# mosure/burn_depth

Measured on AMD Instinct MI355X. Metric: frames/sec Depth Pro @1536^2 bf16, higher is better.
Workload: dtype bf16; 1 GPU; DepthPro::infer [8,3,1536,1536] per GPU, default DepthProConfig; batch_per_gpu=8, streams_per_gpu=1, global_batch=8, parallelism=dp1, attention_form=attn577_gfx950.s (assembly-owned, one persistent workgroup per CU), scatter_inputs_from_rank0=False, gather_depth_to_rank0=False, ranks_seen=1

## Files before the change

### burn_depth_amd/_lib.py

```python
from __future__ import annotations

import ctypes as C
import os

_HERE = os.path.dirname(os.path.abspath(__file__))
LIB_PATH = os.path.join(_HERE, "libmi_depth.so")

MD_OK = 0
MD_ERR_INVALID_ARG, MD_ERR_SHAPE, MD_ERR_IO, MD_ERR_FORMAT, MD_ERR_HIP = -1, -2, -3, -4, -5
MD_ERR_UNSUPPORTED, MD_ERR_NO_FOV, MD_ERR_OOM, MD_ERR_LEVELS = -6, -7, -8, -9
MD_MEM_HOST, MD_MEM_DEVICE = 0, 1
MD_COMM_ID_BYTES = 128
MD_FRAME_U8_GRAY, MD_FRAME_RGBA_F32 = 0, 1
VIT_GEMM_RESID, VIT_GEMM_QKV, VIT_GEMM_FC1, VIT_GEMM_PATCH_EMBED = 0, 1, 2, 3
DECODER_GEMM_CONV3, DECODER_GEMM_CONV3_S2, DECODER_GEMM_PIXSHUF, DECODER_GEMM_HEAD, DECODER_GEMM_HEAD_UP2 = 0, 1, 2, 3, 4
TILE_256x256, TILE_128x128, TILE_256x32, TILE_128x64, TILE_64x64, TILE_AUTO = 0, 1, 2, 3, 4, 99


class MdError(RuntimeError):

    def __init__(self, code: int, message: str):
        super().__init__(f"mi_depth error {code}: {message}")
        self.code = code
        self.message = message
# ... 252 lines not shown
    "md_debug_gemm_direct_store": (_I, [_I]),
    "md_debug_gemm_persistent": (_I, [_I]),
    "md_debug_gemm_stagger": (_I, [_I, _I]),
    "md_debug_gemm_stagger_ticks": (_I, [_I]),
    "md_da3_infer_raw": (_I, [_P, _P, _I, _I, _I, _I, _P, _I, _P]),
    "md_da3_infer_from_tokens": (_I, [_P, C.POINTER(C.c_void_p), _I, _I, _I, _I, _I, _P, _I, _P]),
    "md_da3_param_inventory": (_I, [C.POINTER(MdDa3Cfg), _I, _I, C.POINTER(C.c_char_p), C.POINTER(C.c_size_t), _F, _F]),
    "md_model_query": (_I, [_P, C.c_char_p, C.POINTER(C.c_int64)]),
    "md_model_set_option": (_I, [_P, C.c_char_p, C.c_int64]),
    "md_model_enable_taps": (_I, [_P, _I]),
    "md_model_read_tap": (_I, [_P, C.c_char_p, _P, C.c_size_t, C.POINTER(C.c_int64 * 4)]),
    "md_model_enable_timing": (_I, [_P, _I]),
    "md_model_set_timing_filter": (_I, [_P, C.c_char_p]),
    "md_model_read_timing": (_I, [_P, C.POINTER(C.c_char_p), _F, C.POINTER(_I), _I, C.POINTER(_I)]),
    "md_model_read_launch_order": (_I, [_P, C.POINTER(C.c_char_p), _I, C.POINTER(_I)]),
    "md_op_rgb_to_input": (_I, [_P, _P, C.c_size_t, _I, _I, _P, _P]),
    "md_catmull_rom_taps": (_I, [_I, _I, _I, C.POINTER(_I), C.POINTER(_I), _F]),
    "md_op_resize_catmull_rom": (_I, [_P, _P, _I, _I, _I, _I, _I, _I, _I, _I, _I, _P, _P, _P]),
    "md_op_depth_display": (_I, [_P, _P, _I, _I, _I, _I, _I, _I, _I, _I, _I, _I, _I, _P, _P, _P]),
    "md_op_resize_bilinear": (_I, [_P, _P, _I, _I, _I, _I, _P, _I, _I, _I, _P]),
    "md_op_pyramid_patchify": (_I, [_P, _P, _I, _I, _I, _I, _I, _I, _I, _P, C.POINTER(_I), C.POINTER(_I), _P]),
    "md_op_resize_nhwc": (_I, [_P, _P, _I, _I, _I, _I, _P, _I, _I, _I, _I, _P]),
    "md_op_resize_output_size": (_I, [_I, _I, C.c_float, C.c_float, C.POINTER(_I), C.POINTER(_I)]),
    "md_op_split": (_I, [_P, _P, _I, _I, _I, _I, C.c_float, _P, C.POINTER(_I), _P]),
    "md_op_merge": (_I, [_P, _P, _I, _I, _I, _I, _I, _I, _P, C.POINTER(_I), C.POINTER(_I), _P]),
    "md_op_layernorm": (_I, [_P, _P, _P, _P, _I, _I, C.c_float, _P, _P]),
    "md_op_linear": (_I, [_P, _P, _P, _P, _I, _I, _I, _I, _I, _P, _P]),
    "md_op_linear_tile": (_I, [_P, _P, _P, _P, _I, _I, _I, _I, _I, _I, _P, _P]),
    "md_op_attention": (_I, [_P, _P, _I, _I, _I, _I, _P, _P]),
    "md_op_attention_views": (_I, [_P, _P, _I, _I, _I, _I, _I, _P, _P]),
    "md_op_attention_ex": (_I, [_P, C.POINTER(MdAttentionOp), _P]),
    "md_debug_attention_last_form": (_I, [C.POINTER(_I * 4)]),
    "md_op_conv3x3": (_I, [_P, _P, _P, _P, _I, _I, _I, _I, _I, _I, _I, _P, _P]),
    "md_op_deconv2x2": (_I, [_P, _P, _P, _P, _I, _I, _I, _I, _I, _I, _P, _P]),
    "md_op_conv2d_direct": (_I, [_P, _P, _P, _P, _I, _I, _I, _I, _I, _I, _I, _I, _I, _P, _P]),
    "md_op_qkv_norm_rope": (_I, [_P, _P, _P, _P, _P, _P, _P, _P, _I, _I, _I, _I, _I, _I, _I, C.c_float, C.c_float, _I, _I, _I, _P, _P, _P]),
    "md_op_qk_norm_rope": (_I, [_P, _P, _P, _P, _P, _P, _I, _I, _I, _I, _I, _I, C.c_float, C.c_float, _I, _P, _P]),
    "md_op_hook_cat_ln": (_I, [_P, _P, _P, _I, _I, _I, _I, _P, _P, C.c_float, _P, _P, C.c_float, _I, _P, _P, _P]),
    "md_op_patchify": (_I, [_P, _P, _I, _I, _I, _I, _I, _I, _P, _P, _I, _I, _I, _P, _P, _P]),
    "md_op_set_token0": (_I, [_P, _P, _I, _I, _I, _P, _I, _P]),
    "md_op_border_bias_fix": (_I, [_P, _P, _I, _I, _I, _I, _I, _P, _I, _P]),
    "md_op_layernorm_ex": (_I, [_P, _P, _I, _I, _I, _I, C.POINTER(_I), C.POINTER(_I), C.POINTER(_P), C.POINTER(_P), C.c_float, _I, _I,
                                C.c_float, _P, _I, _P, _P]),
    "md_op_store_rows": (_I, [_P, _P, C.c_int64, _I, _I, _P, _P]),
    "md_op_load_rows": (_I, [_P, _P, C.c_int64, _I, _I, _P, _P]),
    "md_op_f32_to_fp8": (_I, [_P, _P, C.c_int64, C.c_float, _P, _P]),
    "md_op_pack_fp8_rows": (_I, [_P, _P, _I, _I, _I, _P, _P, _P]),
    "md_op_nchw_to_nhwc": (_I, [_P, _P, _I, _I, _I, _I, _I, _I, _I, _P, _P]),
    "md_op_nhwc_to_nchw": (_I, [_P, _P, _I, _I, _I, _I, _I, _I, _I, _P, _P]),
    "md_op_ln_fold_vectors": (_I, [_P, _P, _P, _P, _P, _I, _I, _I, _P, _P, _P]),
    "md_op_ln_finish": (_I, [_P, _P, C.c_int64, C.c_float, C.c_float, _P, _P]),
    "md_op_vit_gemm": (_I, [_P, C.POINTER(MdVitGemm), _P]),
    "md_debug_gemm_last_form": (_I, [C.POINTER(_I * 8)]),
    "md_debug_gemm_last_launch": (_I, [C.POINTER(_I * 4)]),
    "md_op_decoder_gemm": (_I, [_P, C.POINTER(MdDecoderGemm), _P]),
    "md_op_camera_encode": (_I, [_P, C.POINTER(MdCameraEncode), _P]),
    "md_op_camera_decode": (_I, [_P, C.POINTER(MdCameraDecode), _P]),
    "md_op_pose_to_camera": (_I, [_P, _P, _I, _I, _I, _P, _P, _P]),
    "md_op_conv2d_direct_ex": (_I, [_P, _P, _P, _P, _P, _I, _I, _I, _I, _I, _I, _I, _I, _I, _I, _I, _P, _P]),
    "md_op_fov_to_focal": (_I, [C.c_float, _I, _I, _F, _F]),
    "md_op_focal_to_fov": (_I, [C.c_float, _I, _I, _F, _F]),
    "md_bench_gemm": (_I, [_P, _I, _I, _I, _I, _I, _I, _I, _I, _I, _F]),
    "md_gemm_pick_tile": (_I, [_I, _I, _I, _I]),
    "md_bench_attention": (_I, [_P, _I, _I, _I, _I, _F]),
    "md_bench_attention_ex": (_I, [_P, _I, _I, _I, _I, C.c_float, _I, _F]),
    "md_debug_attention_asm": (_I, [_I]),
    "md_debug_attention_asm_launches": (C.c_long, []),
    "md_debug_attention_redo_units": (C.c_long, [_P, _I]),
    "md_bench_attention_qkv": (_I, [_P, _P, _I, _I, _I, _I, _I, _F, C.POINTER(C.c_long)]),
    "md_comm_unique_id": (_I, [_P]),
    "md_comm_init_rank": (_I, [_P, _P, _I, _I, C.POINTER(_P)]),
    "md_comm_rank": (_I, [_P, C.POINTER(_I), C.POINTER(_I)]),
    "md_comm_count": (_I, [_P, C.POINTER(_I)]),
    "md_comm_destroy": (_I, [_P]),
    "md_comm_broadcast_weights": (_I, [_P, _P, _I]),
    "md_comm_scatter_images": (_I, [_P, _P, _P, C.c_size_t, _I, _P]),
    "md_comm_gather_depth": (_I, [_P, _P, _P, C.c_size_t, _I, _P]),
    "md_depth_pro_infer_tiles_loopback": (_I, [C.POINTER(_P), _I, _I, _P, _I, _I, _I, _I, _P, _P, _P, _P, _I, _P]),
    "md_comm_depth_pro_infer_tiles": (_I, [_P, _P, _P, _I, _I, _I, _I, _P, _P, _P, _P, _I, _I, _P]),
    "md_param_inventory": (_I, [C.POINTER(MdDepthProCfg), _I, _I, C.POINTER(C.c_char_p), C.POINTER(C.c_size_t), _F, _F]),
    "md_uniform_stream": (_I, [C.c_char_p, C.c_uint64, C.c_size_t, C.c_float, C.c_float, _P]),
    "md_split_geometry": (_I, [_I, _I, C.c_float, C.POINTER(_I), C.POINTER(_I)]),
    "md_feature_padding": (_I, [_I, _I, _I]),
}


def _infer_points(*parts):
    return _I, [_P, _P, _I, _I, _I, _I, _P, C.POINTER(MdPointsCameras), *(C.POINTER(p) for p in parts), _I, _P]


_POINTS_HEAD = [MdViewFilterOpts, MdPointsOpts, MdPointsOutputs]
_POINTS_PARTS = [("normals", MdPointsNormals), ("voxel", MdPointsVoxel), ("render", MdPointsRender), ("mesh", MdPointsMesh),
                 ("raster", MdPointsRaster), ("outlier", MdPointsOutlier), ("decimate", MdPointsDecimate), ("components", MdPointsComponents),
                 ("smooth", MdPointsSmooth), ("planes", MdPointsPlanes), ("clusters", MdPointsClusters)]
SYMBOLS["md_infer_points"] = _infer_points(*_POINTS_HEAD[1:])
SYMBOLS["md_infer_points_filtered"] = _infer_points(*_POINTS_HEAD)
SYMBOLS.update({f"md_infer_points_{name}": _infer_points(*_POINTS_HEAD, *(p for _, p in _POINTS_PARTS[:i + 1]))
                for i, (name, _) in enumerate(_POINTS_PARTS)})

_lib = None


def load() -> C.CDLL:
    global _lib
    if _lib is not None:
        return _lib
    if not os.path.exists(LIB_PATH):
        raise ImportError(
            f"{LIB_PATH} is missing: build the HIP extension first (python -c 'import __graft_entry__ as g; g.build()'). "
            "burn_depth_amd has no CPU fallback.")
    lib = C.CDLL(LIB_PATH)
    for name, (res, args) in SYMBOLS.items():
        fn = getattr(lib, name)
        fn.restype = res
        fn.argtypes = args
    _lib = lib
    return lib


def check(code: int) -> None:
    if code != MD_OK:
        msg = load().md_last_error()
        raise MdError(code, msg.decode("utf-8", "replace") if msg else "")
```

### burn_depth_amd/csrc/kernels/ops.h

```cpp
#pragma once

#include "../md_common.h"

namespace md {

int launch_rgb_to_input(const uint8_t* rgb, int w, int h, float* out, hipStream_t s);

struct CrAxis {
  const int2* win;
  const float* w;
  int maxc;
};
void catmull_rom_window(int in_len, int out_len, int o, int* left, int* count, float* weights);
int catmull_rom_max_taps(int in_len, int out_len);
void catmull_rom_span(const int* left, const int* count, int cx, int tw, int* xb0, int* nq);
int launch_resize_catmull_rom(const uint8_t* rgb, int B, int h, int w, const CrAxis& ax_v, int cy, int th, const CrAxis& ax_h, int cx,
                              int tw, int xb0, int nq, float* tmp, uint8_t* out_u8, float* out_nchw, hipStream_t s);
struct DisplayGeom {
  int B, h, w, cx, cy, cw, ch, ow, oh, resize;
  float sx, sy;
};
int display_parts(const DisplayGeom& g);
int launch_depth_display(const float* depth, const DisplayGeom& g, int normalize, int format, void* out, float* range, float2* parts,
                         hipStream_t s);
// ... 233 lines not shown
};
constexpr int kRenderMaxRadius = 16;
size_t render_scratch_bytes(int T, int H, int W);
int launch_render_points(const RenderParams& p, void* scratch, hipStream_t s);

struct MeshParams {
  const float* depth = nullptr;
  const int32_t* pixel_index = nullptr;
  int B = 0, H = 0, W = 0, stride = 1;
  long limit = 0;
  float max_rtol = 0.f;
  int32_t* faces = nullptr;
  int32_t* face_count = nullptr;
  long face_capacity = 0;
};
size_t mesh_scratch_bytes(int B, int H, int W, int stride);
int launch_mesh_index(int B, int H, int W, const void* points_scratch, int32_t* pixel_index, hipStream_t s);
int launch_mesh_grid(const MeshParams& p, void* scratch, hipStream_t s);

struct RasterParams {
  const float* xyz = nullptr;
  const uint8_t* rgb = nullptr;
  const int32_t* faces = nullptr;
  const int32_t* count = nullptr;
  int n = 0, nf = 0;
  int T = 0, H = 0, W = 0;
  const float *K = nullptr, *E = nullptr, *focal = nullptr;
  float off = 0.f, znear = 0.f, zfar = 0.f;
  int cull = 0, max_extent = 64;
  float* depth = nullptr;
  int32_t* face = nullptr;
  uint8_t* rgb_out = nullptr;
  int32_t* filled = nullptr;
  int32_t* skipped = nullptr;
};
constexpr int kRasterMaxExtent = 1024;
constexpr int kRasterDefaultExtent = 64;
int raster_inline_pixels();
int raster_queue_capacity(int capacity);
int raster_queue_entries();
size_t raster_scratch_bytes(int T, int H, int W, int queue_entries);
int launch_render_mesh(const RasterParams& p, void* scratch, int queue_entries, hipStream_t s);

int launch_resize_bilinear(const float* in, int planes, int H, int W, float* out, int OH, int OW, int method,
                           int post, hipStream_t s);

struct PyramidGeom {
  int B, S, win, ps;
  int steps0, stride0;
  int steps1, stride1;
  int method;
};
int launch_pyramid_patchify(const float* x, const PyramidGeom& g, void* patches, int prec, hipStream_t s, bool force_generic = false);

int launch_patchify(const float* x, int B, int H, int W, int ps, int Kp, void* out, int prec, hipStream_t s, float* cls_x = nullptr,
                    int S = 0, int n_tokens = 0, int D = 0, const float* cls = nullptr, const float* pos0 = nullptr);

int launch_resize_nhwc(const void* in, int B, int H, int W, int C, long ld_in, void* out, int OH, int OW, long ld_out,
                       int method, const float* addend, int prec, hipStream_t s);

int launch_border_bias_fix(void* map, int B, int H, int W, int C, long ld, const float* bias9, int prec, hipStream_t s);

int launch_split(const float* x, int B, int C, int S, int win, int stride, int steps, float* out, hipStream_t s);
int launch_merge(const float* tiles, int B, int C, int h, int w, int steps, int pad, float* out, int OH, int OW,
                 hipStream_t s);

struct SeqGroups {
  int ngroups;
  int seq0[4];
  int nseq[4];
  const float* a[4];
  const float* b[4];
};
int launch_cls_init(float* x, int nseq_total, int S, int n_tokens, int D, const SeqGroups& g, hipStream_t s);

int launch_layernorm(const float* x, void* out, long rows, int D, float eps, int S, const SeqGroups& g, int prec,
                     int out_f32, hipStream_t s, float fp8_inv_scale = 1.f, const float* tok0 = nullptr, int tok0_stride = 0,
                     float* x_rw = nullptr);
int launch_ln_fold_vectors(const float* W, const float* gamma, const float* beta, const float* bias, int N, int K, int prec, float* c,
                           float* d, hipStream_t s);
int launch_fill_pairs(float* ab, long rows, float a, float b, hipStream_t s);
int launch_ln_finish(const float* parts, float* ab, long rows, float inv_n, float eps, hipStream_t s);
int launch_convert_rows(const float* x, void* out, long count, int prec, hipStream_t s, int width = 0);

int launch_nchw_to_nhwc(const float* in, int B, int C, int H, int W, void* out, int prec, int relu, hipStream_t s, long ld = 0);
int launch_head_tail_debug(const void* relu_map, long ld, long pixels, int C, const float* w, const float* bias, float* pre_out,
                           float* canonical, int prec, hipStream_t s);
int launch_nhwc_to_nchw(const void* in, int B, int C, int H, int W, long ld, int coff, float* out, int prec,
                        hipStream_t s);
int launch_rows_to_f32(const void* in, long count, float* out, int prec, hipStream_t s, int width = 0);
int launch_f32_to_rows(const float* in, long count, void* out, int prec, hipStream_t s, int width = 0);

int launch_conv_direct(const void* in, int in_prec, const float* add, int B, int H, int W, int Cin, const float* w,
                       const float* bias, int Cout, int k, int stride, int pad, int relu, float* out, hipStream_t s, int out_ld = 0);

int launch_f32_to_fp8(const float* in, long n, float inv_scale, void* out, hipStream_t s);
int launch_pack_fp8_rows(const float* w, int N, int K, int Kp, void* out, float* scale, hipStream_t s);

int launch_qk_norm_rope(void* qk, long rows, int S, int n_tokens, int D, int heads, int pw, const float* q_gamma,
                        const float* q_beta, const float* k_gamma, const float* k_beta, float eps, const float* rope_cos,
                        const float* rope_sin, int global_pos, float q_scale, int prec, hipStream_t s);
int launch_set_token0(float* x, int nseq, int S, int D, const float* src, hipStream_t s, int src_stride = 0);

#define MD_CAM_MAX_VIEWS 16
struct CamEncW {
  static constexpr int kMaxDepth = 8;
  const float *fc1_w, *fc1_b, *fc2_w, *fc2_b;
  const float *tn_g, *tn_b, *on_g, *on_b;
  struct Blk {
    const float *n1g, *n1b, *n2g, *n2b, *qkv_w, *qkv_b, *proj_w, *proj_b, *ls1, *fc1_w, *fc1_b, *fc2_w, *fc2_b, *ls2;
  } blk[kMaxDepth];
  int depth;
};
struct CamDecW {
  const float *w1, *b1, *w2, *b2, *wt, *bt, *wq, *bq, *wf, *bf;
};
int launch_camera_decoder(const float* cam, int B, int din, const CamDecW& w, int H, int W, float* h1, float* h2, float* pose, float* extr,
                          float* intr, hipStream_t s);
size_t camera_encoder_scratch_floats(int B, int V, int D);
int launch_camera_encoder(const float* extr, const float* intr, int B, int V, int D, int heads, int H, int W, float eps_tok, float eps_blk,
                          const CamEncW& w, float* scratch, float* out, hipStream_t s);
int launch_hook_cat_ln(const float* x_local, const float* x, long rows, int S, int n_tokens, int D, const float* norm_g,
                       const float* norm_b, float eps_final, const float* head_g, const float* head_b, float eps_head,
                       void* out, float* cam_out, int prec, hipStream_t s);
int launch_pose_to_camera(const float* pose, int B, int H, int W, float* extrinsics, float* intrinsics, hipStream_t s);

int launch_fov_post(const float* fov_deg, int B, int H, int W, float* focal_px, float* fovy_rad, float* ratio,
                    hipStream_t s);
int launch_focal_post(const float* f_px, int B, int H, int W, float* focal_px, float* fovx_deg, float* fovy_rad, float* ratio,
                      hipStream_t s);
int launch_depth_post(const float* canonical, const float* ratio, int B, long hw, float* out, int post, hipStream_t s);

int launch_softmax_rows(float* s, long rows, int n_valid, int ld, float scale, hipStream_t st);

int launch_qkv_split(const float* qkv, int T, int N, int heads, int SS, int kpad, void* qk, void* vT, float q_scale, int prec,
                     hipStream_t s);
int launch_unpad_rows(const void* in, int T, int N, int SS, int D, float* out, int prec, hipStream_t s);

constexpr float kAttnQScale = 0.125f * 1.4426950408889634f;
inline float attn_qscale(int prec) { return prec == MD_PREC_F32 ? 1.0f : kAttnQScale; }

int launch_attention(const void* qk, const void* vT, void* out, int nseq, int S, int n_tokens, int heads, int D,
                     int kpad, int prec, hipStream_t s, float out_fp8_inv = 0.f, long v_plane = 0, int* redo = nullptr,
                     int redo_units = 0);
int attention_asm_prepare();
int launch_attention_views(const void* qk, const void* vT, void* out, int nseq, int views, int S, int n_tokens, int heads, int D,
                           int kpad, int prec, hipStream_t s, long v_plane = 0, int* redo = nullptr, int redo_units = 0);
int attention_allow_asm(int on);
long attention_asm_launches();
int attention_redo_ints(int nunits);
long attention_asm_redo_units(int reset);
int attention_allow_small(int on);
struct AttnSmallScope {
  explicit AttnSmallScope(int on) : prev_(attention_allow_small(on)) {}
  ~AttnSmallScope() { attention_allow_small(prev_); }
  AttnSmallScope(const AttnSmallScope&) = delete;
  AttnSmallScope& operator=(const AttnSmallScope&) = delete;

 private:
  int prev_;
};
enum { ATTN_FORM_NONE = -1, ATTN_FORM_PLAIN = 0, ATTN_FORM_KEYSPLIT = 1, ATTN_FORM_ASM = 2, ATTN_FORM_VIEWS = 3, ATTN_FORM_FP8OUT = 4, ATTN_FORM_F32 = 5 };
struct AttnForm {
  int form = ATTN_FORM_NONE;
  int grid = 0, qw = 0, ks = 0;
};
// ... 5 lines not shown
```

### burn_depth_amd/csrc/kernels/ops.hip

```cpp
#include "ops.h"
#include "camera_math.h"
#include "elem.h"

namespace md {

static inline int grid_for(long work_items, int block = 256, int cap = 256 * 8) {
  long g = (work_items + block - 1) / block;
  if (g < 1) g = 1;
  if (g > cap) g = cap;
  return (int)g;
}

__global__ void rgb_to_input_kernel(const uint8_t* __restrict__ rgb, long hw, float* __restrict__ out) {
#pragma clang fp contract(off)
  const float mean[3] = {0.485f, 0.456f, 0.406f};
  const float sd[3] = {0.229f, 0.224f, 0.225f};
  for (long i = blockIdx.x * (long)blockDim.x + threadIdx.x; i < hw; i += (long)gridDim.x * blockDim.x) {
#pragma unroll
    for (int c = 0; c < 3; ++c) {
      float v = (float)rgb[i * 3 + c] / 255.0f;
      out[c * hw + i] = (v - mean[c]) / sd[c];
    }
  }
}
// ... 685 lines not shown
  }
}

int launch_f32_to_rows(const float* in, long count, void* out, int prec, hipStream_t s, int width) {
  if (prec == MD_PREC_F16X2 && (width <= 0 || count % width != 0)) MD_FAIL(MD_ERR_INVALID_ARG, "f32_to_rows: split-half rows need the row width");
  MD_BY_PREC(prec, hipLaunchKernelGGL(f32_to_rows_kernel<T>, dim3(grid_for(count)), dim3(256), 0, s, in, count, (T*)out, width));
  MD_HIP(hipGetLastError());
  return MD_OK;
}
__global__ __launch_bounds__(256) void ln_finish_kernel(const float* __restrict__ parts, float* __restrict__ ab, long rows, float inv_n, float eps) {
  const long r = (long)blockIdx.x * 256 + threadIdx.x;
  if (r >= rows) return;
  const f32x4_t p0 = *(const f32x4_t*)(parts + r * 8), p1 = *(const f32x4_t*)(parts + r * 8 + 4);
  const float mu = ((p0[0] + p0[2]) + (p1[0] + p1[2])) * 0.25f;
  const float d0 = p0[0] - mu, d1 = p0[2] - mu, d2 = p1[0] - mu, d3 = p1[2] - mu;
  const float m2 = ((p0[1] + p0[3]) + (p1[1] + p1[3])) + 256.0f * ((d0 * d0 + d1 * d1) + (d2 * d2 + d3 * d3));
  const float rstd = 1.0f / sqrtf(m2 * inv_n + eps);
  ab[r * 2] = rstd;
  ab[r * 2 + 1] = -mu * rstd;
}

__global__ __launch_bounds__(256) void fill_pairs_kernel(float* __restrict__ ab, long rows, float a, float b) {
  const long r = (long)blockIdx.x * 256 + threadIdx.x;
  if (r < rows) { ab[2 * r] = a; ab[2 * r + 1] = b; }
}
int launch_fill_pairs(float* ab, long rows, float a, float b, hipStream_t s) {
  if (!ab || rows <= 0) MD_FAIL(MD_ERR_INVALID_ARG, "fill_pairs: invalid argument");
  hipLaunchKernelGGL(fill_pairs_kernel, dim3((unsigned)((rows + 255) / 256)), dim3(256), 0, s, ab, rows, a, b);
  MD_HIP(hipGetLastError());
  return MD_OK;
}

int launch_ln_finish(const float* parts, float* ab, long rows, float inv_n, float eps, hipStream_t s) {
  if (!parts || !ab || rows <= 0) MD_FAIL(MD_ERR_INVALID_ARG, "ln_finish: invalid argument");
  hipLaunchKernelGGL(ln_finish_kernel, dim3((unsigned)((rows + 255) / 256)), dim3(256), 0, s, parts, ab, rows, inv_n, eps);
  MD_HIP(hipGetLastError());
  return MD_OK;
}

template <typename T>
__global__ __launch_bounds__(256) void ln_fold_vectors_kernel(const float* __restrict__ W, const float* __restrict__ gamma,
                                                              const float* __restrict__ beta, const float* __restrict__ bias, int N, int K,
                                                              float* __restrict__ c, float* __restrict__ d) {
  const int n = blockIdx.x * 4 + (threadIdx.x >> 6), lane = threadIdx.x & 63;
  if (n >= N) return;
  const float* w = W + (long)n * K;
  double sc = 0.0, sd = 0.0;
  for (int k = lane; k < K; k += 64) {
    float wr;
    if constexpr (sizeof(T) == 4) {
      wr = w[k];
    } else {
      const float hi = (float)cvt_elem<T>(w[k]);
      wr = is_split<T>::value ? hi + (float)cvt_elem<T>(w[k] - hi) : hi;
    }
    sc += (double)gamma[k] * (double)wr;
    sd += (double)beta[k] * (double)wr;
  }
#pragma unroll
  for (int o = 32; o > 0; o >>= 1) {
    sc += __shfl_xor(sc, o);
    sd += __shfl_xor(sd, o);
  }
  if (lane == 0) {
    c[n] = (float)sc;
    d[n] = (float)(sd + (bias ? (double)bias[n] : 0.0));
  }
}

int launch_ln_fold_vectors(const float* W, const float* gamma, const float* beta, const float* bias, int N, int K, int prec, float* c,
                           float* d, hipStream_t s) {
  if (!W || !gamma || !beta || !c || !d || N <= 0 || K <= 0) MD_FAIL(MD_ERR_INVALID_ARG, "ln_fold_vectors: invalid argument");
  MD_BY_PREC(prec, hipLaunchKernelGGL(ln_fold_vectors_kernel<T>, dim3((unsigned)((N + 3) / 4)), dim3(256), 0, s, W, gamma, beta, bias, N, K, c, d));
  MD_HIP(hipGetLastError());
  return MD_OK;
}

int launch_convert_rows(const float* x, void* out, long count, int prec, hipStream_t s, int width) {
  return launch_f32_to_rows(x, count, out, prec, s, width);
}
int launch_rows_to_f32(const void* in, long count, float* out, int prec, hipStream_t s, int width) {
  if (prec == MD_PREC_F16X2 && (width <= 0 || count % width != 0)) MD_FAIL(MD_ERR_INVALID_ARG, "rows_to_f32: split-half rows need the row width");
  MD_BY_PREC(prec, hipLaunchKernelGGL(rows_to_f32_kernel<T>, dim3(grid_for(count)), dim3(256), 0, s, (const T*)in, count, out, width));
  MD_HIP(hipGetLastError());
  return MD_OK;
}

template <typename T>
__global__ void nchw_to_nhwc_kernel(const float* __restrict__ in, int B, int C, int H, int W, T* __restrict__ out,
                                    int relu, long ld) {
  const long total = (long)B * C * H * W;
  for (long e = blockIdx.x * (long)blockDim.x + threadIdx.x; e < total; e += (long)gridDim.x * blockDim.x) {
    const int c = (int)(e % C);
    long t = e / C;
    const int xw = (int)(t % W);
    t /= W;
    const int y = (int)(t % H);
    const int b = (int)(t / H);
    float v = in[(((long)b * C + c) * H + y) * W + xw];
    if (relu) v = fmaxf(v, 0.f);
    st1p<T>(out + (e / C) * (ld * kPlanes<T>) + c, ld, v);
  }
}
template <typename T>
__global__ void nhwc_to_nchw_kernel(const T* __restrict__ in, int B, int C, int H, int W, long ld, int coff,
                                    float* __restrict__ out) {
  const long total = (long)B * C * H * W;
  for (long e = blockIdx.x * (long)blockDim.x + threadIdx.x; e < total; e += (long)gridDim.x * blockDim.x) {
    const int xw = (int)(e % W);
    long t = e / W;
    const int y = (int)(t % H);
    t /= H;
    const int c = (int)(t % C);
    const int b = (int)(t / C);
    const long src = (((long)b * H + y) * W + xw) * (ld * kPlanes<T>) + coff + c;
    out[e] = ld1p<T>(in + src, ld);
  }
}

int launch_nchw_to_nhwc(const float* in, int B, int C, int H, int W, void* out, int prec, int relu, hipStream_t s, long ld) {
  const long total = (long)B * C * H * W;
  if (ld != 0 && ld < C) MD_FAIL(MD_ERR_INVALID_ARG, "nchw_to_nhwc: pixel stride %ld below C %d", ld, C);
  MD_BY_PREC(prec, hipLaunchKernelGGL(nchw_to_nhwc_kernel<T>, dim3(grid_for(total)), dim3(256), 0, s, in, B, C, H, W, (T*)out, relu, ld ? ld : (long)C));
  MD_HIP(hipGetLastError());
  return MD_OK;
}

template <typename T>
__global__ void head_tail_debug_kernel(const T* __restrict__ relu_map, long ld, long pixels, int C, const float* __restrict__ w,
                                       const float* __restrict__ bias, float* __restrict__ pre_out, float* __restrict__ canonical) {
  for (long e = blockIdx.x * (long)blockDim.x + threadIdx.x; e < pixels; e += (long)gridDim.x * blockDim.x) {
    const T* px = relu_map + e * (ld * kPlanes<T>);
    float acc = 0.f;
    for (int c = 0; c < C; ++c) acc = fmaf(ld1p<T>(px + c, ld), w[c], acc);
    acc += bias ? bias[0] : 0.f;
    if (pre_out) pre_out[e] = acc;
    if (canonical) canonical[e] = fmaxf(acc, 0.f);
  }
}
int launch_head_tail_debug(const void* relu_map, long ld, long pixels, int C, const float* w, const float* bias, float* pre_out,
                           float* canonical, int prec, hipStream_t s) {
  MD_BY_PREC(prec, hipLaunchKernelGGL(head_tail_debug_kernel<T>, dim3(grid_for(pixels)), dim3(256), 0, s, (const T*)relu_map, ld, pixels, C, w,
                                      bias, pre_out, canonical));
  MD_HIP(hipGetLastError());
  return MD_OK;
}
int launch_nhwc_to_nchw(const void* in, int B, int C, int H, int W, long ld, int coff, float* out, int prec,
                        hipStream_t s) {
  const long total = (long)B * C * H * W;
  MD_BY_PREC(prec, hipLaunchKernelGGL(nhwc_to_nchw_kernel<T>, dim3(grid_for(total)), dim3(256), 0, s, (const T*)in, B, C, H, W, ld, coff, out));
  MD_HIP(hipGetLastError());
  return MD_OK;
}

template <typename TI>
__device__ inline void load4v(const TI* in, long src, long plane, float v[4]) {
  const f32x4_t t = load4p<TI>(in + src, plane);
  v[0] = t[0], v[1] = t[1], v[2] = t[2], v[3] = t[3];
}

template <typename TI, int CO, int VEC>
__global__ __launch_bounds__(256) void conv_direct_kernel(const TI* __restrict__ in, const float* __restrict__ add,
                                                          int B, int H, int W, int Cin, const float* __restrict__ w,
                                                          const float* __restrict__ bias, int Cout, int k, int stride,
                                                          int pad, int relu, float* __restrict__ out, int OH, int OW, int out_ld) {
  const int lane = threadIdx.x & 63;
// ... 466 lines not shown
```

### burn_depth_amd/csrc/md_api.cpp

```cpp
#include <algorithm>
#include <cmath>
#include <cstdio>
#include <cstring>
#include <optional>
#include <vector>

#include "md_engine.h"
#include "md_engine_util.h"

using namespace md;

namespace {
struct DevBuf {
  void* p = nullptr;
  ~DevBuf() {
    if (p) (void)hipFree(p);
  }
  int alloc(size_t bytes, bool raw = false) {
    if (hipMalloc(&p, bytes + 4096) != hipSuccess) {
      set_error("hipMalloc(%zu) failed", bytes);
      return MD_ERR_OOM;
    }
    return raw || hipMemset(p, 0, bytes + 4096) == hipSuccess ? MD_OK : MD_ERR_HIP;
  }
// ... 289 lines not shown
}

int md_depth_pro_decoder_from_features(md_model_t m, const md_nchw_view* features, int levels, int B, int in_kind,
                                       float* out_features, float* out_lowres, float* const* out_fusions, int out_kind,
                                       void* stream) {
  return model_decoder_from_features(m, features, levels, B, in_kind, out_features, out_lowres, out_fusions, out_kind, (hipStream_t)stream);
}

int md_depth_pro_head_debug(md_model_t m, const md_nchw_view* feature, int B, int in_kind, const md_head_debug* out, int out_kind,
                            void* stream) {
  return model_head_debug(m, feature, B, in_kind, out, out_kind, (hipStream_t)stream);
}

int md_depth_pro_infer_windows(md_model_t m, const float* nchw, int B, int H, int W, int in_kind, float* depth,
                               float* focallength_px, float* fovx_deg, float* fovy_rad, int out_kind, int parts,
                               float* window_ms, float* tail_ms, void* stream) {
  if (!nchw) MD_FAIL(MD_ERR_INVALID_ARG, "input pointer is null");
  if (m && m->kind != 0) MD_FAIL(MD_ERR_INVALID_ARG, "not a Depth Pro model");
  if (parts < 1 || parts > 64) MD_FAIL(MD_ERR_INVALID_ARG, "parts = %d (1 .. 64)", parts);
  ShardPlan sp;
  sp.parts = parts;
  sp.part = -1;
  sp.window_ms = window_ms;
  sp.tail_ms = tail_ms;
  return model_infer_sharded(m, nchw, B, H, W, in_kind, depth, focallength_px, fovx_deg, fovy_rad, out_kind, (hipStream_t)stream, sp);
}

int md_infer_from_rgb(md_model_t m, const uint8_t* rgb, size_t rgb_len, int w, int h, int in_kind, float* depth,
                      float* focallength_px, float* fovy_rad, int out_kind, void* stream) {
  if (!rgb) MD_FAIL(MD_ERR_INVALID_ARG, "rgb pointer is null");
  if (w <= 0 || h <= 0) MD_FAIL(MD_ERR_SHAPE, "invalid image size %dx%d", w, h);
  const size_t expected = (size_t)w * (size_t)h * 3;
  if (rgb_len != expected) MD_FAIL(MD_ERR_SHAPE, "expected %zu RGB bytes for %dx%d, got %zu", expected, w, h, rgb_len);
  if (m && m->kind != 0) MD_FAIL(MD_ERR_INVALID_ARG, "not a Depth Pro model");
  return model_infer(m, nullptr, 1, h, w, in_kind, depth, focallength_px, nullptr, fovy_rad, out_kind, (hipStream_t)stream,
                     rgb, rgb_len);
}

int md_infer_from_rgb_with_focal(md_model_t m, const uint8_t* rgb, size_t rgb_len, int w, int h, int in_kind, float f_px,
                                 float* depth, float* focallength_px, float* fovy_rad, int out_kind, void* stream) {
  if (!rgb) MD_FAIL(MD_ERR_INVALID_ARG, "rgb pointer is null");
  if (w <= 0 || h <= 0) MD_FAIL(MD_ERR_SHAPE, "invalid image size %dx%d", w, h);
  const size_t expected = (size_t)w * (size_t)h * 3;
  if (rgb_len != expected) MD_FAIL(MD_ERR_SHAPE, "expected %zu RGB bytes for %dx%d, got %zu", expected, w, h, rgb_len);
  if (m && m->kind != 0) MD_FAIL(MD_ERR_INVALID_ARG, "not a Depth Pro model");
  return model_infer(m, nullptr, 1, h, w, in_kind, depth, focallength_px, nullptr, fovy_rad, out_kind, (hipStream_t)stream,
                     rgb, rgb_len, &f_px, MD_MEM_HOST);
}

int md_model_enable_graph(md_model_t m, int enable) {
  if (!m) MD_FAIL(MD_ERR_INVALID_ARG, "model is null");
  m->graph_enabled = enable != 0;
  return MD_OK;
}

int md_model_query(md_model_t m, const char* key, int64_t* out) {
  if (!m || !key || !out) MD_FAIL(MD_ERR_INVALID_ARG, "null argument");
  const std::string k = key;
  if (k == "img_size") *out = m->S;
  else if (k == "patch_window") *out = m->win;
  else if (k == "interpolation") *out = m->cfg.interpolation;
  else if (k == "precision") *out = m->prec;
  else if (k == "max_batch") *out = m->cfg.max_batch;
  else if (k == "num_params") {
    int64_t n = 0;
    for (auto& p : m->params) n += (int64_t)p.count();
    *out = n;
  } else if (k == "workspace_bytes") *out = (int64_t)m->ws.cap;
  else if (k == "weight_bytes") *out = m->parent ? 0 : (int64_t)(m->w32_bytes + m->wpk_bytes);
  else if (k == "tiles_per_image") *out = m->steps0 * m->steps0 + m->steps1 * m->steps1 + 1;
  else if (k == "seq_stride") *out = m->SS;
  else if (k == "is_fork") *out = m->parent ? 1 : 0;
  else if (k == "forks") *out = m->forks.load();
  else if (k == "weight_terms") *out = model_root(m)->wterms;
  else if (k == "allocs") *out = m->alloc_count;
  else if (k == "voxel_overflow") return points_voxel_overflow(m, out);
  else if (k == "outlier_overflow") return points_outlier_overflow(m, out);
  else if (k == "clusters_overflow") return points_clusters_overflow(m, out);
  else if (k == "decimate_overflow") return points_decimate_overflow(m, out);
  else if (k == "da3_shape_builds") *out = da3_shape_builds(m);
  else if (k == "batch_invariant") *out = m->batch_invariant ? 1 : 0;
  else if (k == "ln_fold") *out = m->ln_fold_opt;
  else if (k == "ln_fold_active") *out = m->ln_fold_on() ? 1 : 0;
  else if (model_decoder_query(m, k, out)) {}
  else MD_FAIL(MD_ERR_INVALID_ARG, "unknown query key `%s`", key);
  return MD_OK;
}

int md_model_set_option(md_model_t m, const char* key, int64_t value) {
  if (!m || !key) MD_FAIL(MD_ERR_INVALID_ARG, "null argument");
  const std::string k = key;
  if (k == "batch_invariant") {
    if (value != 0 && value != 1) MD_FAIL(MD_ERR_INVALID_ARG, "batch_invariant takes 0 or 1");
    if (m->batch_invariant != (value != 0)) {
      m->batch_invariant = value != 0;
      MD_HIP(hipSetDevice(m->dev->ordinal));
      MD_HIP(hipDeviceSynchronize());
      m->graphs.clear();
    }
    return MD_OK;
  }
  if (k == "ln_fold") {
    if (value < 0 || value > 4) MD_FAIL(MD_ERR_INVALID_ARG, "ln_fold takes 0 (off), 1 (automatic), 2 (on whenever the model can), 3 / 4 (bench diagnostics: unfolded schedule through the fold-form consumer kernels on neutral statistics / the fold with the ln_finish launch)");
    if (value >= 2 && !m->ln_fold_can) MD_FAIL(MD_ERR_UNSUPPORTED, "ln_fold: this model cannot fold its LayerNorms (16-bit Depth Pro models of width %% 256 == 0 can)");
    if (m->ln_fold_opt != (int)value) {
      m->ln_fold_opt = (int)value;
      MD_HIP(hipSetDevice(m->dev->ordinal));
      MD_HIP(hipDeviceSynchronize());
      m->graphs.clear();
    }
    return MD_OK;
  }
  MD_FAIL(MD_ERR_INVALID_ARG, "unknown option `%s`", key);
}

int md_model_enable_taps(md_model_t m, int enable) {
  if (!m) MD_FAIL(MD_ERR_INVALID_ARG, "model is null");
  m->taps_enabled = enable != 0;
  return MD_OK;
}

int md_model_read_tap(md_model_t m, const char* name, float* host_data, size_t capacity, int64_t dims[4]) {
  if (!m || !name) MD_FAIL(MD_ERR_INVALID_ARG, "null argument");
  auto it = m->taps.find(name);
  if (it == m->taps.end() || !it->second.dev) MD_FAIL(MD_ERR_INVALID_ARG, "tap `%s` was not captured", name);
  if (dims) memcpy(dims, it->second.dims, sizeof(int64_t) * 4);
  if (!host_data) return MD_OK;
  if (capacity < it->second.count) MD_FAIL(MD_ERR_SHAPE, "tap `%s` needs %zu floats, capacity %zu", name, it->second.count, capacity);
  MD_HIP(hipSetDevice(m->dev->ordinal));
  MD_HIP(hipDeviceSynchronize());
  MD_HIP(hipMemcpy(host_data, it->second.dev, it->second.count * 4, hipMemcpyDeviceToHost));
  return MD_OK;
}

int md_model_enable_timing(md_model_t m, int enable) {
  if (!m) MD_FAIL(MD_ERR_INVALID_ARG, "model is null");
  m->timing_enabled = enable != 0;
  return MD_OK;
}

int md_model_set_timing_filter(md_model_t m, const char* family) {
  if (!m) MD_FAIL(MD_ERR_INVALID_ARG, "model is null");
  m->timing_filter = family ? family : "";
  return MD_OK;
}

int md_model_read_timing(md_model_t m, const char** names, float* ms, int* calls, int cap, int* n) {
  if (!m || !n) MD_FAIL(MD_ERR_INVALID_ARG, "null argument");
  MD_HIP(hipSetDevice(m->dev->ordinal));
  MD_HIP(hipDeviceSynchronize());
  m->timing_names_out.clear();
  std::vector<float> tot;
  std::vector<int> cnt;
  for (auto& t : m->timing) {
    float e = 0.f;
    if (hipEventElapsedTime(&e, t.a, t.b) != hipSuccess) continue;
    size_t i = 0;
    for (; i < m->timing_names_out.size(); ++i)
      if (m->timing_names_out[i] == t.name) break;
    if (i == m->timing_names_out.size()) {
      m->timing_names_out.push_back(t.name);
      tot.push_back(0.f);
      cnt.push_back(0);
    }
    tot[i] += e;
    cnt[i] += 1;
  }
  for (auto& t : m->timing) {
    (void)hipEventDestroy(t.a);
    (void)hipEventDestroy(t.b);
  }
  m->timing.clear();
  *n = (int)m->timing_names_out.size();
  for (int i = 0; i < *n && i < cap; ++i) {
    if (names) names[i] = m->timing_names_out[i].c_str();
    if (ms) ms[i] = tot[i];
    if (calls) calls[i] = cnt[i];
  }
  return MD_OK;
}

int md_model_read_launch_order(md_model_t m, const char** names, int cap, int* n) {
  if (!m || !n) MD_FAIL(MD_ERR_INVALID_ARG, "null argument");
  *n = (int)m->timing.size();
  for (int i = 0; i < *n && i < cap; ++i)
    if (names) names[i] = m->timing[i].name.c_str();
  return MD_OK;
}

// ... 742 lines not shown
  if ((long)next * S < rows) MD_FAIL(MD_ERR_SHAPE, "layernorm_ex: %d sequences of %d rows do not cover %d rows", next, S, rows);
  OpStage s;
  MD_TRY(s.open(dev, stream));
  MD_TRY(launch_layernorm(x, out, rows, D, eps, S, g, precision, out_f32, s.st, fp8_inv_scale, tok0, tok0_stride, tok0 ? x : nullptr));
  return s.finish();
}

int md_op_store_rows(md_device_t dev, const float* in, int64_t count, int width, int precision, void* out, void* stream) {
  if (!dev || !in || !out) MD_FAIL(MD_ERR_INVALID_ARG, "null argument");
  if (!token_op_prec(precision)) MD_FAIL(MD_ERR_INVALID_ARG, "unknown precision %d", precision);
  if (count <= 0 || width < 0) MD_FAIL(MD_ERR_SHAPE, "store_rows: count=%lld width=%d", (long long)count, width);
  OpStage s;
  MD_TRY(s.open(dev, stream));
  MD_TRY(launch_f32_to_rows(in, (long)count, out, precision, s.st, width));
  return s.finish();
}

int md_op_load_rows(md_device_t dev, const void* in, int64_t count, int width, int precision, float* out, void* stream) {
  if (!dev || !in || !out) MD_FAIL(MD_ERR_INVALID_ARG, "null argument");
  if (!token_op_prec(precision)) MD_FAIL(MD_ERR_INVALID_ARG, "unknown precision %d", precision);
  if (count <= 0 || width < 0) MD_FAIL(MD_ERR_SHAPE, "load_rows: count=%lld width=%d", (long long)count, width);
  OpStage s;
  MD_TRY(s.open(dev, stream));
  MD_TRY(launch_rows_to_f32(in, (long)count, out, precision, s.st, width));
  return s.finish();
}

int md_op_f32_to_fp8(md_device_t dev, const float* in, int64_t count, float inv_scale, void* out, void* stream) {
  if (!dev || !in || !out) MD_FAIL(MD_ERR_INVALID_ARG, "null argument");
  if (count <= 0) MD_FAIL(MD_ERR_SHAPE, "f32_to_fp8: count=%lld", (long long)count);
  OpStage s;
  MD_TRY(s.open(dev, stream));
  MD_TRY(launch_f32_to_fp8(in, (long)count, inv_scale, out, s.st));
  return s.finish();
}

int md_op_pack_fp8_rows(md_device_t dev, const float* w, int N, int K, int Kp, void* out, float* scale, void* stream) {
  if (!dev || !w || !out || !scale) MD_FAIL(MD_ERR_INVALID_ARG, "null argument");
  if (N <= 0 || K <= 0) MD_FAIL(MD_ERR_SHAPE, "pack_fp8_rows: N=%d K=%d", N, K);
  OpStage s;
  MD_TRY(s.open(dev, stream));
  MD_TRY(launch_pack_fp8_rows(w, N, K, Kp, out, scale, s.st));
  return s.finish();
}

int md_op_nchw_to_nhwc(md_device_t dev, const float* in, int B, int C, int H, int W, int precision, int relu, int ld, void* out,
                       void* stream) {
  if (!dev || !in || !out) MD_FAIL(MD_ERR_INVALID_ARG, "null argument");
  if (!token_op_prec(precision)) MD_FAIL(MD_ERR_INVALID_ARG, "unknown precision %d", precision);
  if (B <= 0 || C <= 0 || H <= 0 || W <= 0 || ld < 0) MD_FAIL(MD_ERR_SHAPE, "nchw_to_nhwc: [%d,%d,%d,%d] ld=%d", B, C, H, W, ld);
  OpStage s;
  MD_TRY(s.open(dev, stream));
  MD_TRY(launch_nchw_to_nhwc(in, B, C, H, W, out, precision, relu ? 1 : 0, s.st, ld));
  return s.finish();
}

int md_op_nhwc_to_nchw(md_device_t dev, const void* in, int B, int C, int H, int W, int ld, int coff, int precision, float* out,
                       void* stream) {
  if (!dev || !in || !out) MD_FAIL(MD_ERR_INVALID_ARG, "null argument");
  if (!token_op_prec(precision)) MD_FAIL(MD_ERR_INVALID_ARG, "unknown precision %d", precision);
  if (B <= 0 || C <= 0 || H <= 0 || W <= 0) MD_FAIL(MD_ERR_SHAPE, "nhwc_to_nchw: [%d,%d,%d,%d]", B, C, H, W);
  if (coff < 0 || ld < coff + C) MD_FAIL(MD_ERR_INVALID_ARG, "nhwc_to_nchw: channels [%d, %d) outside a pixel of %d", coff, coff + C, ld);
  OpStage s;
  MD_TRY(s.open(dev, stream));
  MD_TRY(launch_nhwc_to_nchw(in, B, C, H, W, ld, coff, out, precision, s.st));
  return s.finish();
}

int md_op_ln_fold_vectors(md_device_t dev, const float* w, const float* gamma, const float* beta, const float* bias, int N, int K,
                          int precision, float* c, float* d, void* stream) {
  if (!dev) MD_FAIL(MD_ERR_INVALID_ARG, "null argument");
  if (!token_op_prec(precision)) MD_FAIL(MD_ERR_INVALID_ARG, "unknown precision %d", precision);
  OpStage s;
  MD_TRY(s.open(dev, stream));
  MD_TRY(launch_ln_fold_vectors(w, gamma, beta, bias, N, K, precision, c, d, s.st));
  return s.finish();
}

int md_op_ln_finish(md_device_t dev, const float* parts, int64_t rows, float inv_n, float eps, float* ab, void* stream) {
  if (!dev) MD_FAIL(MD_ERR_INVALID_ARG, "null argument");
  OpStage s;
  MD_TRY(s.open(dev, stream));
  MD_TRY(launch_ln_finish(parts, ab, (long)rows, inv_n, eps, s.st));
  return s.finish();
}

int md_op_vit_gemm(md_device_t dev, const md_vit_gemm* d, void* stream) {
  if (!dev || !d || !d->a) MD_FAIL(MD_ERR_INVALID_ARG, "null argument");
  const int prec = d->precision, kind = d->kind, N = d->N, K = d->K, G = d->ngroups;
  if (!token_op_prec(prec) && !(prec == MD_PREC_FP8 && kind == MD_VIT_GEMM_RESID)) MD_FAIL(MD_ERR_INVALID_ARG, "vit_gemm: kind %d has no precision %d", kind, prec);
  if (kind < MD_VIT_GEMM_RESID || kind > MD_VIT_GEMM_PATCH_EMBED) MD_FAIL(MD_ERR_INVALID_ARG, "vit_gemm: kind %d", kind);
  if (G < 1 || G > kMaxGroups) MD_FAIL(MD_ERR_INVALID_ARG, "vit_gemm: %d groups (1..%d)", G, kMaxGroups);
  if (N <= 0 || N % 4 != 0 || K <= 0 || K % ke_of(prec) != 0) MD_FAIL(MD_ERR_UNSUPPORTED, "vit_gemm: N=%d (x4), K=%d (x%d)", N, K, ke_of(prec));
  if (d->a_rows <= 0 || d->out_rows <= 0) MD_FAIL(MD_ERR_SHAPE, "vit_gemm: a_rows=%d out_rows=%d", d->a_rows, d->out_rows);
  const bool patch = kind == MD_VIT_GEMM_PATCH_EMBED, resid = kind == MD_VIT_GEMM_RESID, qkv = kind == MD_VIT_GEMM_QKV;
  const bool producer = resid && d->g[0].gamma_next, consumer = (qkv || kind == MD_VIT_GEMM_FC1) && d->g[0].c;
  long row_space = d->out_rows;
  if (patch) {
    if (d->P <= 0 || d->S < 1 + d->P || d->out_rows % d->S != 0 || !d->x) MD_FAIL(MD_ERR_SHAPE, "vit_gemm: patch embed P=%d S=%d rows=%d", d->P, d->S, d->out_rows);
    row_space = (long)(d->out_rows / d->S) * d->P;
  }
  const int row_mult = (consumer || qkv) ? 4 : 1;
  for (int g = 0; g < G; ++g) {
    const md_vit_gemm_group& q = d->g[g];
    if (!q.w || !q.bias) MD_FAIL(MD_ERR_INVALID_ARG, "vit_gemm: group %d has no weight / bias", g);
    if (q.rows <= 0 || q.row0 < 0 || (long)q.row0 + q.rows > row_space || q.arow0 < 0 || (long)q.arow0 + q.rows > d->a_rows)
      MD_FAIL(MD_ERR_SHAPE, "vit_gemm: group %d = rows [%d, +%d) from A row %d outside %ld output / %d A rows", g, q.row0, q.rows, q.arow0, row_space, d->a_rows);
    if (q.rows % row_mult != 0 || q.row0 % row_mult != 0) MD_FAIL(MD_ERR_UNSUPPORTED, "vit_gemm: group %d: rows [%d, +%d) must be multiples of %d here", g, q.row0, q.rows, row_mult);
    if (resid && !q.scale) MD_FAIL(MD_ERR_INVALID_ARG, "vit_gemm: group %d has no LayerScale", g);
    if (patch && !q.pos) MD_FAIL(MD_ERR_INVALID_ARG, "vit_gemm: group %d has no position table", g);
    if ((resid && !q.gamma_next != !producer) || (!resid && !patch && !q.c != !consumer)) MD_FAIL(MD_ERR_INVALID_ARG, "vit_gemm: the LayerNorm fold is for every group or for none");
  }
  if (producer || consumer) {
    if (d->tile != TILE_256x256 || N % 256 != 0 || prec == MD_PREC_F32 || prec == MD_PREC_FP8) MD_FAIL(MD_ERR_UNSUPPORTED, "vit_gemm: the LayerNorm fold runs on the 256 x 256 kernel, 16-bit operands, N %% 256 == 0");
    if (producer && (!d->ln_out || !d->ln_stats_out)) MD_FAIL(MD_ERR_INVALID_ARG, "vit_gemm: fold producer outputs missing");
    if (consumer && (!d->ln_stats || (d->ln_raw && K != 1024))) MD_FAIL(MD_ERR_INVALID_ARG, "vit_gemm: fold consumer statistics missing (raw partials: four per row, K = 1024)");
  }
  const int D = d->D, S = d->S, heads = D / 64, kpad = (S + 63) / 64 * 64;
  size_t vt_elems = 0;
  if (resid && !d->x) MD_FAIL(MD_ERR_INVALID_ARG, "vit_gemm: x missing");
  if (kind == MD_VIT_GEMM_FC1 && !d->out) MD_FAIL(MD_ERR_INVALID_ARG, "vit_gemm: out missing");
  if (qkv) {
    if (!d->qk || !d->vT) MD_FAIL(MD_ERR_INVALID_ARG, "vit_gemm: qk / vT missing");
    if (D <= 0 || D % 64 != 0 || N != 3 * D || S <= 0 || S % 4 != 0 || d->out_rows % S != 0) MD_FAIL(MD_ERR_SHAPE, "vit_gemm: qkv N=%d D=%d S=%d rows=%d", N, D, S, d->out_rows);
    vt_elems = (size_t)(d->out_rows / S) * heads * 64 * kpad;
    if (vt_elems >= ((size_t)1 << 31) || (long)d->out_rows * 2 * D >= (1L << 31)) MD_FAIL(MD_ERR_UNSUPPORTED, "vit_gemm: tensors of this size are not a test");
  }
  const KsplitScope ksplit(1);
  OpStage s;
  MD_TRY(s.open(dev, stream, prec));
  hipStream_t st = s.st;
  const bool split = s.split;
  const int xm = s.geom.xm;

  DevBuf xa, wa[kMaxGroups], ws[kMaxGroups];
  GemmParams p;
  for (int g = 0; g < G; ++g) MD_TRY(s.terms_of(d->g[g].w, (long)N * K));
  MD_TRY(s.dense_a(d->a, d->a_rows, K, xa, &p.ascale));
  for (int g = 0; g < G; ++g) {
    const md_vit_gemm_group& q = d->g[g];
    MD_TRY(wa[g].alloc((size_t)N * K * esz_of(prec) * split_terms(s.geom, 0)));
    MD_TRY(s.dense_w(q.w, N, K, wa[g], ws[g]));
    p.g_row0[g] = q.row0; p.g_rows[g] = q.rows; p.g_arow0[g] = q.arow0;
    p.W[g] = wa[g].p; p.wscale[g] = (const float*)ws[g].p; p.bias[g] = q.bias; p.scale[g] = q.scale; p.pos[g] = q.pos;
    if (producer) p.ln_gamma[g] = q.gamma_next;
    if (consumer) p.ln_c[g] = q.c;
  }
  p.N = N; p.ngroups = G; p.A = xa.p;
  split_dense_a(s.geom, p, K, K, 0);
  if (consumer) {
    p.ln_stats = d->ln_stats; p.ln_raw = d->ln_raw ? 1 : 0; p.ln_parts = K / 256; p.ln_inv_n = d->ln_inv_n; p.ln_eps = d->ln_eps;
  }

  StorageOut o1, o2;
  const long rows = d->out_rows;
  if (resid) {
    p.epi = EPI_RESID_LS;
    split_out(s.geom, p, N, false);
    p.out = d->x_out ? d->x_out : d->x;
    p.resid_src = d->x_out ? d->x : nullptr;
    if (producer) {
      MD_TRY(o1.open(d->ln_out, rows * N, N, prec, st));
      p.ln_out = o1.buf.p; p.ln_ldo = (long)N * xm; p.ln_plane = split ? N : 0;
      p.ln_stats_out = d->ln_stats_out; p.ln_parts = N / 256;
    }
  } else if (qkv) {
// ... 545 lines not shown
  Da3Outputs o;
  o.depth = out->depth; o.depth_confidence = out->depth_confidence; o.aux = out->aux; o.aux_confidence = out->aux_confidence;
  o.pose_encoding = out->pose_encoding; o.extrinsics = out->extrinsics; o.intrinsics = out->intrinsics;
  o.views = V;
  return da3_infer_ex(m, nchw, B * V, H, W, in_kind, o, out_kind, (hipStream_t)stream);
}

int md_da3_infer_with_camera(md_model_t m, const float* nchw, int B, int H, int W, int in_kind, const float* extrinsics,
                             const float* intrinsics, int views, const md_da3_outputs* out, int out_kind, void* stream) {
  if (!out) MD_FAIL(MD_ERR_INVALID_ARG, "outputs struct is null");
  if (!extrinsics || !intrinsics) MD_FAIL(MD_ERR_INVALID_ARG, "extrinsics/intrinsics is null (md_da3_infer_ex is the call without camera inputs)");
  if (views < 1) MD_FAIL(MD_ERR_SHAPE, "camera inputs need at least one view, got %d", views);
  Da3Outputs o;
  o.depth = out->depth; o.depth_confidence = out->depth_confidence; o.aux = out->aux; o.aux_confidence = out->aux_confidence;
  o.pose_encoding = out->pose_encoding; o.extrinsics = out->extrinsics; o.intrinsics = out->intrinsics;
  o.cam_extrinsics = extrinsics; o.cam_intrinsics = intrinsics; o.cam_views = views;
  return da3_infer_ex(m, nchw, B, H, W, in_kind, o, out_kind, (hipStream_t)stream);
}

int md_da3_infer_raw(md_model_t m, const float* nchw, int B, int H, int W, int in_kind, float* logits, int out_kind, void* stream) {
  if (!logits) MD_FAIL(MD_ERR_INVALID_ARG, "logits is null");
  Da3Outputs o;
  o.raw_logits = logits;
  return da3_infer_ex(m, nchw, B, H, W, in_kind, o, out_kind, (hipStream_t)stream);
}

int md_da3_infer_from_tokens(md_model_t m, const float* const* tokens, int tokens_per_image, int B, int H, int W, int in_kind,
                             const md_da3_outputs* out, int out_kind, void* stream) {
  if (!out) MD_FAIL(MD_ERR_INVALID_ARG, "outputs struct is null");
  if (!tokens) MD_FAIL(MD_ERR_INVALID_ARG, "tokens is null");
  Da3Outputs o;
  o.depth = out->depth; o.depth_confidence = out->depth_confidence; o.aux = out->aux; o.aux_confidence = out->aux_confidence;
  o.pose_encoding = out->pose_encoding; o.extrinsics = out->extrinsics; o.intrinsics = out->intrinsics;
  for (int i = 0; i < 4; ++i) o.tokens[i] = tokens[i];
  if (!o.tokens[0]) MD_FAIL(MD_ERR_LEVELS, "Backbone returned fewer hooks (0) than requested (4)");
  o.tokens_per_image = tokens_per_image;
  return da3_infer_ex(m, nullptr, B, H, W, in_kind, o, out_kind, (hipStream_t)stream);
}

int md_da3_param_inventory(const md_da3_cfg* cfg, int init_scheme, int index, const char** name, size_t* count, float* lo,
                           float* hi) {
  Da3Cfg dc;
  MD_TRY(parse_da3_cfg(cfg, &dc));
  static thread_local std::vector<ParamSpec> specs;
  specs = da3_param_specs(dc, init_scheme);
  if (index >= 0 && index < (int)specs.size()) {
    if (name) *name = specs[index].name.c_str();
    if (count) *count = specs[index].count();
    if (lo) *lo = specs[index].lo;
    if (hi) *hi = specs[index].hi;
  }
  return (int)specs.size();
}

int md_param_inventory(const md_depth_pro_cfg* cfg, int init_scheme, int index, const char** name, size_t* count, float* lo,
                       float* hi) {
  ModelCfg mc;
  MD_TRY(parse_cfg(cfg, &mc));
  static thread_local std::vector<ParamSpec> specs;
  specs = depth_pro_param_specs(mc, init_scheme);
  if (index >= 0 && index < (int)specs.size()) {
    if (name) *name = specs[index].name.c_str();
    if (count) *count = specs[index].count();
    if (lo) *lo = specs[index].lo;
    if (hi) *hi = specs[index].hi;
  }
  return (int)specs.size();
}

int md_uniform_stream(const char* name, uint64_t seed, size_t count, float lo, float hi, float* out_host) {
  if (!name || !out_host) MD_FAIL(MD_ERR_INVALID_ARG, "null argument");
  uniform_stream(name, seed, count, lo, hi, out_host);
  return MD_OK;
}

int md_split_geometry(int image_size, int window, float overlap, int* stride, int* steps) {
  if (!stride || !steps || image_size <= 0 || window <= 0) MD_FAIL(MD_ERR_INVALID_ARG, "invalid argument");
  split_geometry(image_size, window, overlap, stride, steps);
  return MD_OK;
}

int md_feature_padding(int window, int stride, int feature_size) { return feature_padding(window, stride, feature_size); }

}
```

### burn_depth_amd/csrc/md_engine.h

```cpp
#pragma once

#include <atomic>
#include <cstdint>
#include <map>
#include <string>
#include <unordered_map>
#include <vector>

#include "kernels/gemm.h"
#include "kernels/ops.h"
#include "md_common.h"
#include "md_weights.h"

struct md_device_s {
  int ordinal = 0;
  hipStream_t stream = nullptr;
};

namespace md {

struct Arena {
  char* base = nullptr;
  size_t cap = 0, off = 0;
  void* take(size_t bytes) {
    size_t o = align_up(off, 256);
    if (o + bytes > cap) return nullptr;
    off = o + bytes;
    return base + o;
  }
};

void split_geometry(int image_size, int patch_size, float overlap, int* stride, int* steps);
int feature_padding(int patch_size, int stride, int feature_patch_size);
void merge_source(int Y, int X, int h, int w, int steps, int pad, int* j, int* i, int* ty, int* tx);
int merged_extent(int h, int steps, int pad);

enum PackKind : int { PACK_NK = 0, PACK_CONV3 = 1, PACK_DECONV = 2, PACK_DIRECT = 3, PACK_HEAD_W = 4, PACK_HEAD_B = 5, PACK_C1C3_W = 6, PACK_C1C3_B = 7 };

struct PackEntry {
  int param = -1;
  int param2 = -1;
  int param3 = -1, param4 = -1;
  int kind = PACK_NK;
  int d0 = 0, d1 = 0, k = 1;
  int kp = 0;
  int terms = 1;
  int f32 = 0;
  void* dst = nullptr;
  size_t bytes = 0;
};

struct VitBlockW {
  const float *n1g, *n1b, *n2g, *n2b, *qkv_b, *proj_b, *ls1, *fc1_b, *fc2_b, *ls2;
  const void *qkv_w, *proj_w, *fc1_w, *fc2_w;
  const float* w32[4] = {nullptr, nullptr, nullptr, nullptr};
  const float *qkv_c = nullptr, *qkv_d = nullptr, *fc1_c = nullptr, *fc1_d = nullptr;
  const float *qkn_g[2] = {nullptr, nullptr}, *qkn_b[2] = {nullptr, nullptr};
  void* w8[4] = {nullptr, nullptr, nullptr, nullptr};
  float* s8[4] = {nullptr, nullptr, nullptr, nullptr};
  bool global = false;
};
struct VitW {
  const void* pe_w;
  const float *pe_b, *cls, *pos, *norm_g, *norm_b;
  std::vector<VitBlockW> blk;
};
struct ConvW { const void* w = nullptr; const float* b = nullptr; };
struct ResUnitW { ConvW c1, c2; };
struct DepthProW {
  const void *enc_proj[5] = {}, *enc_up[5] = {}, *latent0_1x2 = nullptr;
  ConvW lowres, fuse;
  const void* convs[5] = {};
  ResUnitW res[5][2];
  ConvW out[5];
  ConvW conv0, outconv_conv0, deconv, deconv_conv1, conv1, conv_out;
  ConvW down, fov_proj, head[4];
  const void* down_gemm = nullptr;
};

struct Tap {
  float* dev = nullptr;
  int64_t dims[4] = {0, 0, 0, 0};
  size_t count = 0;
};

struct TimingEntry {
  std::string name;
  hipEvent_t a, b;
};

struct GraphCache {
  GraphCache() = default;
  GraphCache(const GraphCache&) = delete;
  GraphCache& operator=(const GraphCache&) = delete;
  ~GraphCache() { clear(); }
  void clear() {
    for (auto& kv : entries)
      if (kv.second.exec) (void)hipGraphExecDestroy(kv.second.exec);
    entries.clear();
  }
  void track_generation(unsigned root_gen) {
    if (gen == root_gen) return;
    clear();
    gen = root_gen;
  }
  template <typename F>
  int run(hipStream_t st, const std::vector<uintptr_t>& key, F&& body) {
    {
      Entry& e = entries[key];
      if (e.exec) {
        MD_HIP(hipGraphLaunch(e.exec, st));
        return MD_OK;
      }
      if (e.seen++ == 0) return body();
    }
    MD_HIP(hipStreamBeginCapture(st, hipStreamCaptureModeRelaxed));
    const int s = body();
    hipGraph_t g = nullptr;
    const hipError_t ce = hipStreamEndCapture(st, &g);
    if (s != MD_OK || ce != hipSuccess || !g) {
      if (g) (void)hipGraphDestroy(g);
      entries.erase(key);
      if (s != MD_OK) return s;
      MD_FAIL(MD_ERR_HIP, "stream capture failed: %s", hipGetErrorString(ce));
    }
    hipGraphExec_t ex = nullptr;
    const hipError_t ie = hipGraphInstantiate(&ex, g, nullptr, nullptr, 0);
    (void)hipGraphDestroy(g);
    if (ie != hipSuccess || !ex) {
      entries.erase(key);
      MD_FAIL(MD_ERR_HIP, "hipGraphInstantiate failed: %s", hipGetErrorString(ie));
    }
    entries[key].exec = ex;
    MD_HIP(hipGraphLaunch(ex, st));
    return MD_OK;
  }

 private:
  struct Entry {
    int seen = 0;
    hipGraphExec_t exec = nullptr;
  };
  std::map<std::vector<uintptr_t>, Entry> entries;
  unsigned gen = 0;
};

template <typename T, bool Pinned = false>
struct GrowBuf {
  T* p = nullptr;
  size_t cap = 0;
  GrowBuf() = default;
  GrowBuf(const GrowBuf&) = delete;
  GrowBuf& operator=(const GrowBuf&) = delete;
  ~GrowBuf() { release(); }
  void release() {
    if (p) (void)(Pinned ? hipHostFree((void*)p) : hipFree((void*)p));
    p = nullptr;
    cap = 0;
  }
};
using PinnedBuf = GrowBuf<void, true>;

}

struct md_model_s {
  md_device_t dev = nullptr;
  md::ModelCfg cfg;
  int prec = MD_PREC_BF16;
  int esz = 2;
  int ke = 64;
  int xm = 1;
  int wterms = 1;
  size_t vt_plane = 0;

  std::vector<md::ParamSpec> params;
  std::unordered_map<std::string, int> pindex;
  std::vector<float*> w32;
  char* w32_base = nullptr;
  size_t w32_bytes = 0;
  std::vector<md::PackEntry> packs;
  std::unordered_map<std::string, int> pack_index;
  char* wpk_base = nullptr;
  size_t wpk_bytes = 0;
  bool committed = false;
  unsigned commit_gen = 0;
  int ngroups = 2;
  md::VitW vit[3];
  md::DepthProW dp;
  float head_b_host = 0.f;

  md::Arena ws;
  struct Buffers;
  Buffers* buf = nullptr;
  void* zero_page = nullptr;
  long alloc_count = 0;
  std::map<int, int*> index_tables;
  struct IndexSet {
    int *hi = nullptr, *mid = nullptr, *x2 = nullptr, *img = nullptr, *fov = nullptr;
  };
  std::map<int, IndexSet> index_sets;

  bool taps_enabled = false;
  std::map<std::string, md::Tap> taps;
  bool timing_enabled = false;
  std::string timing_filter;
  std::vector<md::TimingEntry> timing;
  std::vector<std::string> timing_names_out;

  bool graph_enabled = false;
  bool batch_invariant = false;
  int ln_fold_opt = 1;
  bool ln_fold_can = false;
  float* lnfold_base = nullptr;
  bool ln_fold_on() const { return ln_fold_can && (ln_fold_opt == 2 || ln_fold_opt == 4 || (ln_fold_opt == 1 && NT >= 256)); }
  md::GraphCache graphs;

  md_model_s* parent = nullptr;
  std::atomic<int> forks{0};
  hipStream_t own_stream = nullptr;

  int kind = 0;
  struct Da3State;
  Da3State* da3 = nullptr;
  struct FrameState;
  FrameState* frame = nullptr;
  struct PointsState;
  PointsState* points = nullptr;
  int S = 0, win = 0, g = 0, P = 0, NT = 0, SS = 0, kpad = 0;
  int steps0 = 0, stride0 = 0, steps1 = 0, stride1 = 0, pad_hi = 0, pad_mid = 0;
  int mh_hi = 0, mh_mid = 0;
};

namespace md {

int model_create(md_device_t dev, const ModelCfg& cfg, md_model_t* out);
int model_init_seeded(md_model_t m, uint64_t seed, int scheme);
int model_load_container(md_model_t m, const char* path);
int model_commit(md_model_t m);
int model_round_weights_f16(md_model_t m);
int model_destroy(md_model_t m);
int model_fork(md_model_t src, md_model_t* out);
inline md_model_s* model_root(md_model_s* m) { return m->parent ? m->parent : m; }
inline hipStream_t model_stream(const md_model_s* m, hipStream_t stream) { return stream ? stream : (m->own_stream ? m->own_stream : m->dev->stream); }
template <typename T, bool Pinned>
int grow(md_model_s* m, hipStream_t st, GrowBuf<T, Pinned>& b, size_t bytes, bool* grown = nullptr) {
  if (grown) *grown = false;
  if (b.cap >= bytes) return MD_OK;
  MD_HIP(hipStreamSynchronize(st));
  m->graphs.clear();
  b.release();
  void* p = nullptr;
  const hipError_t e = Pinned ? hipHostMalloc(&p, bytes, hipHostMallocDefault) : hipMalloc(&p, bytes);
  if (e != hipSuccess) MD_FAIL(MD_ERR_OOM, "%s(%zu) of a staging buffer failed: %s", Pinned ? "hipHostMalloc" : "hipMalloc", bytes, hipGetErrorString(e));
  b.p = (T*)p;
  b.cap = bytes;
  m->alloc_count += 1;
  if (grown) *grown = true;
  return MD_OK;
}
int model_infer(md_model_t m, const float* nchw, int B, int H, int W, int in_kind, float* depth, float* focal,
                float* fovx, float* fovy, int out_kind, hipStream_t stream, const uint8_t* rgb, size_t rgb_len,
                const float* f_px = nullptr, int f_kind = 0);
int model_decoder_from_features(md_model_t m, const md_nchw_view* features, int levels, int B, int in_kind, float* out_features,
                                float* out_lowres, float* const* out_fusions, int out_kind, hipStream_t stream);
int model_head_debug(md_model_t m, const md_nchw_view* feature, int B, int in_kind, const md_head_debug* out, int out_kind,
                     hipStream_t stream);
bool model_decoder_query(md_model_t m, const std::string& key, int64_t* out);
struct ShardSegment {
  void* ptr;
  size_t bytes;
};
struct ShardPlan {
  int parts = 1;
  int part = 0;
  int root = 0;
  int (*exchange)(void* ctx, int parts, const ShardSegment (*seg)[3], hipStream_t st) = nullptr;
  void* ctx = nullptr;
  float* window_ms = nullptr;
  float* tail_ms = nullptr;
};
int model_infer_sharded(md_model_t m, const float* nchw, int B, int H, int W, int in_kind, float* depth, float* focal,
                        float* fovx, float* fovy, int out_kind, hipStream_t stream, const ShardPlan& sp);
int model_stage_input(md_model_t m, const float* nchw, size_t elems, int in_kind, hipStream_t stream, float** dev);
// ... 124 lines not shown
```

### burn_depth_amd/csrc/md_engine.hip

```cpp
#include "md_engine.h"
#include "md_engine_util.h"
#include "kernels/elem.h"

#include <algorithm>
#include <cmath>
#include <cstring>

namespace md {

void split_geometry(int image_size, int patch_size, float overlap, int* stride, int* steps) {
  int st = (int)std::floor((float)patch_size * (1.0f - overlap));
  st = std::max(st, 1);
  st = std::min(st, patch_size);
  *stride = st;
  *steps = patch_size >= image_size ? 1 : 1 + (image_size - patch_size + st - 1) / st;
}

int feature_padding(int patch_size, int stride, int fps) {
  if (fps == 0 || patch_size == 0) return 0;
  const int denom = std::max(patch_size, 1);
  const int fstride = (stride * fps + denom / 2) / denom;
  return std::max(fps - fstride, 0) / 2;
}

// ... 515 lines not shown
  md_model_s* m = new md_model_s();
  m->dev = dev;
  m->cfg = cfg;
  m->prec = cfg.precision;
  m->esz = cfg.precision == MD_PREC_F32 ? 4 : 2;
  m->ke = 128 / m->esz;
  m->xm = cfg.precision == MD_PREC_F16X2 ? 2 : 1;
  m->wterms = m->xm == 2 ? 3 : 1;
  m->ngroups = 2 + ((cfg.use_fov_head && cfg.has_fov_vit) ? 1 : 0);
  m->ln_fold_can = (m->prec == MD_PREC_BF16 || m->prec == MD_PREC_F16 || m->prec == MD_PREC_F16X2) && cfg.pv.D == 1024;
  m->S = cfg.img_size();
  m->win = cfg.pv.img;
  m->g = cfg.pv.grid();
  m->P = m->g * m->g;
  m->NT = m->P + 1;
  m->SS = round_up(m->NT, 4);
  m->kpad = round_up(m->NT, 64);
  split_geometry(m->S, m->win, 0.25f, &m->stride0, &m->steps0);
  split_geometry(m->S / 2, m->win, 0.5f, &m->stride1, &m->steps1);
  m->pad_hi = feature_padding(m->win, m->stride0, m->g);
  m->pad_mid = feature_padding(m->win, m->stride1, m->g);
  m->mh_hi = merged_extent(m->g, m->steps0, m->pad_hi);
  m->mh_mid = merged_extent(m->g, m->steps1, m->pad_mid);
  auto fail = [&](int code) {
    model_destroy(m);
    return code;
  };
  if ((m->steps0 - 1) * m->stride0 + m->win != m->S || (m->steps1 - 1) * m->stride1 + m->win != m->S / 2 ||
      m->stride0 % 4 != 0 || m->stride1 % 4 != 0 || m->g - 2 * m->pad_hi <= 0 || m->g - 2 * m->pad_mid <= 0) {
    set_error("split geometry of window %d at image %d is not tile-exact", m->win, m->S);
    return fail(MD_ERR_UNSUPPORTED);
  }
  if (m->mh_mid * 2 != m->mh_hi || m->g * 4 != m->mh_hi) {
    set_error("merged feature maps %d / %d / %d do not nest by 2", m->mh_hi, m->mh_mid, m->g);
    return fail(MD_ERR_UNSUPPORTED);
  }

  int st = alloc_param_arena(m, depth_pro_param_specs(cfg, MD_INIT_REFERENCE));
  if (st != MD_OK) return fail(st);
  const int D = cfg.pv.D;
  const char* vnames[3] = {"encoder.patch_encoder", "encoder.image_encoder", "fov.encoder"};
  for (int gi = 0; gi < m->ngroups; ++gi) vit_add_packs(m, vnames[gi], cfg.pv);
  dp_add_packs(m);
  if ((st = place_packs(m)) != MD_OK) return fail(st);
  for (int gi = 0; gi < m->ngroups; ++gi) vit_bind(m, vnames[gi], cfg.pv.depth, m->vit[gi]);
  if ((st = dp_bind(m)) != MD_OK) return fail(st);
  if (m->ln_fold_can) {
    const size_t per_blk = (size_t)14 * D;
    if (hipMalloc((void**)&m->lnfold_base, ((size_t)m->ngroups * cfg.pv.depth * per_blk + 4 * D) * 4) != hipSuccess ||
        hipMemset(m->lnfold_base + (size_t)m->ngroups * cfg.pv.depth * per_blk, 0, (size_t)4 * D * 4) != hipSuccess) {
      set_error("hipMalloc of the LayerNorm-fold vectors failed");
      return fail(MD_ERR_OOM);
    }
    for (int gi = 0; gi < m->ngroups; ++gi)
      for (int i = 0; i < cfg.pv.depth; ++i) {
        float* q = m->lnfold_base + ((size_t)gi * cfg.pv.depth + i) * per_blk;
        VitBlockW& k = m->vit[gi].blk[i];
        k.qkv_c = q; k.qkv_d = q + 3 * D; k.fc1_c = q + 6 * D; k.fc1_d = q + 10 * D;
      }
  }

  if ((st = alloc_workspace(m)) != MD_OK) return fail(st);
  *out = m;
  return MD_OK;
}

int model_destroy(md_model_t m) {
  if (!m) return MD_OK;
  if (m->forks.load() > 0) MD_FAIL(MD_ERR_INVALID_ARG, "model has %d live fork(s) sharing its weights: destroy them first", m->forks.load());
  if (m->dev) (void)hipSetDevice(m->dev->ordinal);
  (void)hipDeviceSynchronize();
  if (m->parent) {
    m->parent->forks.fetch_sub(1);
    m->w32_base = nullptr;
    m->wpk_base = nullptr;
  }
  if (m->own_stream) (void)hipStreamDestroy(m->own_stream);
  if (m->w32_base) (void)hipFree(m->w32_base);
  if (m->wpk_base) (void)hipFree(m->wpk_base);
  if (m->lnfold_base && !m->parent) (void)hipFree(m->lnfold_base);
  if (m->ws.base) (void)hipFree(m->ws.base);
  if (m->zero_page) (void)hipFree(m->zero_page);
  for (auto& kv : m->index_tables) (void)hipFree(kv.second);
  m->graphs.clear();
  for (auto& kv : m->taps) (void)hipFree(kv.second.dev);
  for (auto& t : m->timing) {
    (void)hipEventDestroy(t.a);
    (void)hipEventDestroy(t.b);
  }
  if (m->da3) da3_destroy_state(m);
  if (m->frame) frame_destroy_state(m);
  if (m->points) points_destroy_state(m);
  delete m->buf;
  delete m;
  return MD_OK;
}

int model_fork(md_model_t src, md_model_t* out) {
  if (!src || !out) MD_FAIL(MD_ERR_INVALID_ARG, "model/out is null");
  if (src->kind != 0)
    MD_FAIL(MD_ERR_UNSUPPORTED, "md_model_fork: Depth-Anything-v3 models keep per-shape tables beside their workspace "
                                "(the reference's CachedDepthAnything3 is not Sync either, depth_anything3/mod.rs:44,67-70)");
  md_model_s* root = model_root(src);
  if (!root->committed) MD_FAIL(MD_ERR_INVALID_ARG, "weights were modified; call md_model_commit_weights before forking");
  MD_HIP(hipSetDevice(root->dev->ordinal));
  md_model_s* m = new md_model_s();
  m->dev = root->dev;
  m->cfg = root->cfg;
  m->prec = root->prec; m->esz = root->esz; m->ke = root->ke; m->xm = root->xm; m->wterms = root->wterms;
  m->params = root->params; m->pindex = root->pindex; m->w32 = root->w32;
  m->w32_base = root->w32_base; m->w32_bytes = root->w32_bytes;
  m->packs = root->packs; m->pack_index = root->pack_index;
  m->wpk_base = root->wpk_base; m->wpk_bytes = root->wpk_bytes;
  m->committed = true;
  m->ngroups = root->ngroups;
  m->ln_fold_can = root->ln_fold_can; m->ln_fold_opt = root->ln_fold_opt; m->lnfold_base = root->lnfold_base;
  for (int g = 0; g < 3; ++g) m->vit[g] = root->vit[g];
  m->dp = root->dp;
  m->head_b_host = root->head_b_host;
  m->S = root->S; m->win = root->win; m->g = root->g; m->P = root->P; m->NT = root->NT; m->SS = root->SS; m->kpad = root->kpad;
  m->steps0 = root->steps0; m->stride0 = root->stride0; m->steps1 = root->steps1; m->stride1 = root->stride1;
  m->pad_hi = root->pad_hi; m->pad_mid = root->pad_mid; m->mh_hi = root->mh_hi; m->mh_mid = root->mh_mid;
  m->parent = root;
  root->forks.fetch_add(1);
  auto fail = [&](int code) {
    model_destroy(m);
    return code;
  };
  if (hipStreamCreateWithFlags(&m->own_stream, hipStreamDefault) != hipSuccess) {
    set_error("hipStreamCreate failed");
    return fail(MD_ERR_HIP);
  }
  const int st = alloc_workspace(m);
  if (st != MD_OK) return fail(st);
  *out = m;
  return MD_OK;
}

int model_init_seeded(md_model_t m, uint64_t seed, int scheme) {
  if (scheme != MD_INIT_REFERENCE && scheme != MD_INIT_PARITY) MD_FAIL(MD_ERR_INVALID_ARG, "unknown init scheme %d", scheme);
  MD_HIP(hipSetDevice(m->dev->ordinal));
  std::vector<ParamSpec> specs = m->kind == 1 ? da3_param_specs(da3_cfg(m), scheme) : depth_pro_param_specs(m->cfg, scheme);
  if (specs.size() != m->params.size()) MD_FAIL(MD_ERR_FORMAT, "internal: inventory mismatch");
  std::vector<float> tmp;
  for (size_t i = 0; i < specs.size(); ++i) {
    const size_t n = specs[i].count();
    tmp.resize(n);
    uniform_stream(specs[i].name, seed, n, specs[i].lo, specs[i].hi, tmp.data());
    MD_HIP(hipMemcpy(m->w32[i], tmp.data(), n * 4, hipMemcpyHostToDevice));
  }
  return model_commit(m);
}

int model_load_params_from_container(md_model_t m, const char* path) {
  Container c;
  MD_TRY(read_container(path, &c));
  MD_HIP(hipSetDevice(m->dev->ordinal));
  std::vector<float> tmp;
  for (size_t i = 0; i < m->params.size(); ++i) {
    const ParamSpec& s = m->params[i];
    auto it = c.tensors.find(s.name);
    if (it == c.tensors.end()) MD_FAIL(MD_ERR_FORMAT, "checkpoint `%s` has no tensor `%s`", path, s.name.c_str());
    size_t n = 1;
    for (auto d : it->second.shape) n *= (size_t)d;
    if (n != s.count()) {
      MD_FAIL(MD_ERR_FORMAT, "tensor `%s` has %zu elements, the model expects %zu", s.name.c_str(), n, s.count());
    }
    bool linear_t = false;
    if (c.burn_record && s.shape.size() == 2 && it->second.shape.size() == 2) {
      if (it->second.shape[0] != s.shape[1] || it->second.shape[1] != s.shape[0])
        MD_FAIL(MD_ERR_FORMAT, "Burn record: linear weight `%s` has shape [%lld, %lld], expected [d_input = %lld, d_output = %lld]", s.name.c_str(),
                (long long)it->second.shape[0], (long long)it->second.shape[1], (long long)s.shape[1], (long long)s.shape[0]);
      linear_t = true;
    }
    bool swap = false;
    if (s.shape.size() == 4 && it->second.shape.size() == 4 && s.shape[2] == 2 && s.shape[3] == 2 &&
        s.shape[0] != s.shape[1] && it->second.shape[0] == s.shape[1] && it->second.shape[1] == s.shape[0])
      swap = true;
    tmp.resize(n);
    MD_TRY(container_tensor_to_f32(c, it->second, tmp.data(), n));
    if (linear_t) {
      std::vector<float> t2(n);
      const size_t no = (size_t)s.shape[0], ni = (size_t)s.shape[1];
      for (size_t ii = 0; ii < ni; ++ii)
        for (size_t o = 0; o < no; ++o) t2[o * ni + ii] = tmp[ii * no + o];
      tmp.swap(t2);
    }
    if (swap) {
      std::vector<float> t2(n);
      const size_t a = (size_t)s.shape[0], b2 = (size_t)s.shape[1];
      for (size_t o = 0; o < b2; ++o)
        for (size_t ii = 0; ii < a; ++ii)
          for (int q = 0; q < 4; ++q) t2[(ii * b2 + o) * 4 + q] = tmp[(o * a + ii) * 4 + q];
      tmp.swap(t2);
    }
    MD_HIP(hipMemcpy(m->w32[i], tmp.data(), n * 4, hipMemcpyHostToDevice));
  }
  return MD_OK;
}
// ... 10 lines not shown
  float* composed = nullptr;
  size_t composed_elems = 0;
  for (auto& e : m->packs) {
    if (e.kind == PACK_HEAD_W) composed_elems = std::max(composed_elems, (size_t)4 * e.d0 * e.d1 * 9);
    else if (e.kind == PACK_C1C3_W) composed_elems = std::max(composed_elems, (size_t)e.d0 * e.d1 * 9);
    else if (e.kind == PACK_HEAD_B || e.kind == PACK_C1C3_B) continue;
    else if (e.param2 >= 0) composed_elems = std::max(composed_elems, (size_t)e.d0 * e.d1 * e.k * e.k);
  }
  if (composed_elems) MD_HIP(hipMalloc((void**)&composed, composed_elems * sizeof(float)));
  if (m->xm == 2) {
    unsigned* d_cnt = nullptr;
    unsigned h_cnt = 0;
    MD_HIP(hipMalloc((void**)&d_cnt, 4));
    MD_HIP(hipMemsetAsync(d_cnt, 0, 4, s));
    for (auto& e : m->packs) {
      if (e.f32 || e.param2 >= 0 || (e.kind != PACK_NK && e.kind != PACK_CONV3 && e.kind != PACK_DECONV)) continue;
      const long n = (long)m->params[e.param].count();
      hipLaunchKernelGGL(count_inexact_f16_kernel, dim3((int)std::min<long>((n + 255) / 256, 2048)), dim3(256), 0, s, m->w32[e.param], n, d_cnt);
    }
    MD_HIP(hipMemcpyAsync(&h_cnt, d_cnt, 4, hipMemcpyDeviceToHost, s));
    MD_HIP(hipStreamSynchronize(s));
    MD_HIP(hipFree(d_cnt));
    m->wterms = h_cnt == 0 ? 2 : 3;
    for (auto& e : m->packs) e.terms = e.f32 ? 1 : ((e.param2 >= 0 || e.kind == PACK_HEAD_W || e.kind == PACK_C1C3_W) ? 3 : m->wterms);
  }
  for (auto& e : m->packs) {
    if (e.kind == PACK_HEAD_W) {
      MD_TRY(compose_head(m->w32[e.param], m->w32[e.param2], e.d1, e.k, e.d0, composed, s));
      PackEntry c3 = e;
      c3.kind = PACK_CONV3; c3.d0 = 4 * e.d0; c3.k = 3;
      MD_TRY(pack_weight(composed, c3, m->prec, s));
    } else if (e.kind == PACK_HEAD_B || e.kind == PACK_C1C3_B) {
      MD_TRY(compose_head_bias(m->w32[e.param2], m->w32[e.param3], m->w32[e.param4], e.k, e.d0, (float*)e.dst, s));
    } else if (e.kind == PACK_C1C3_W) {
      MD_TRY(compose_c1c3(m->w32[e.param], m->w32[e.param2], e.d1, e.k, e.d0, composed, s));
      PackEntry c3 = e;
      c3.kind = PACK_CONV3; c3.k = 3;
      MD_TRY(pack_weight(composed, c3, m->prec, s));
    } else if (e.param2 < 0) {
      MD_TRY(pack_weight(m->w32[e.param], e, m->prec, s));
    } else if (e.k == 4) {
      MD_TRY(compose_deconv_pair(m->w32[e.param], m->w32[e.param2], e.d0, e.param3, e.d1, composed, s));
      MD_TRY(pack_weight(composed, e, m->prec, s));
    } else {
      MD_TRY(compose_deconv_conv(m->w32[e.param], m->w32[e.param2], e.d0, e.d1, e.d1, composed, s));
      MD_TRY(pack_weight(composed, e, m->prec, s));
    }
  }
  if (m->kind == 0 && m->ln_fold_can && m->lnfold_base) {
    const int D = m->cfg.pv.D;
    for (int gi = 0; gi < m->ngroups; ++gi)
      for (const VitBlockW& k : m->vit[gi].blk) {
        MD_TRY(launch_ln_fold_vectors(k.w32[0], k.n1g, k.n1b, k.qkv_b, 3 * D, D, m->prec, (float*)k.qkv_c, (float*)k.qkv_d, s));
        MD_TRY(launch_ln_fold_vectors(k.w32[2], k.n2g, k.n2b, k.fc1_b, 4 * D, D, m->prec, (float*)k.fc1_c, (float*)k.fc1_d, s));
      }
  }
  auto it = m->pindex.find(m->kind == 1 ? "head_mono.scratch.output_conv2.conv2.bias" : "head.conv_out.bias");
  if (it != m->pindex.end()) MD_HIP(hipMemcpyAsync(&m->head_b_host, m->w32[it->second], 4, hipMemcpyDeviceToHost, s));
  MD_HIP(hipStreamSynchronize(s));
  if (composed) MD_HIP(hipFree(composed));
  if (m->kind == 1) MD_TRY(da3_on_commit(m));
  m->graphs.clear();
  m->commit_gen += 1;
  m->committed = true;
  return MD_OK;
}

int model_round_weights_f16(md_model_t m) {
  if (!m) MD_FAIL(MD_ERR_INVALID_ARG, "model is null");
  if (m->parent) MD_FAIL(MD_ERR_INVALID_ARG, "a fork shares its root's weights: round them on the root model");
  if (m->forks.load() > 0) MD_FAIL(MD_ERR_INVALID_ARG, "model has %d live fork(s) sharing its weights", m->forks.load());
  MD_HIP(hipSetDevice(m->dev->ordinal));
  hipStream_t s = m->dev->stream;
  for (size_t i = 0; i < m->params.size(); ++i) {
    const long n = (long)m->params[i].count();
    hipLaunchKernelGGL(round_f16_kernel, dim3((int)std::min<long>((n + 255) / 256, 2048)), dim3(256), 0, s, m->w32[i], n);
  }
  MD_HIP(hipGetLastError());
  MD_HIP(hipStreamSynchronize(s));
  m->committed = false;
  return model_commit(m);
}

static int get_index_set(md_model_s* m, int B, md_model_s::IndexSet* out) {
  auto it = m->index_sets.find(B);
  if (it != m->index_sets.end()) {
    *out = it->second;
    return MD_OK;
  }
  const int g = m->g, SS = m->SS, P = m->P;
  const int n0 = m->steps0 * m->steps0 * B, n1 = m->steps1 * m->steps1 * B;
  const int nseq_p = n0 + n1 + B;
  const size_t nhi = (size_t)B * m->mh_hi * m->mh_hi, nmid = (size_t)B * m->mh_mid * m->mh_mid, nlo = (size_t)B * P;
  std::vector<int> h(nhi + nmid + 3 * nlo);
  size_t o = 0;
  for (int b = 0; b < B; ++b)
    for (int Y = 0; Y < m->mh_hi; ++Y)
      for (int X = 0; X < m->mh_hi; ++X) {
        int j, i, ty, tx;
        merge_source(Y, X, g, g, m->steps0, m->pad_hi, &j, &i, &ty, &tx);
        h[o++] = ((j * m->steps0 + i) * B + b) * SS + 1 + ty * g + tx;
      }
  for (int b = 0; b < B; ++b)
    for (int Y = 0; Y < m->mh_mid; ++Y)
      for (int X = 0; X < m->mh_mid; ++X) {
        int j, i, ty, tx;
        merge_source(Y, X, g, g, m->steps1, m->pad_mid, &j, &i, &ty, &tx);
        h[o++] = (n0 + (j * m->steps1 + i) * B + b) * SS + 1 + ty * g + tx;
      }
  for (int which = 0; which < 3; ++which)
    for (int b = 0; b < B; ++b)
      for (int p = 0; p < P; ++p) {
        const int seq = which == 0 ? n0 + n1 + b : which == 1 ? nseq_p + b : nseq_p + B + b;
        h[o++] = seq * SS + 1 + p;
      }
  int* d = nullptr;
  MD_HIP(hipMalloc((void**)&d, h.size() * 4));
  m->alloc_count += 1;
  MD_HIP(hipMemcpy(d, h.data(), h.size() * 4, hipMemcpyHostToDevice));
  m->index_tables[B] = d;
  md_model_s::IndexSet s;
  s.hi = d;
  s.mid = d + nhi;
  s.x2 = s.mid + nmid;
  s.img = s.x2 + nlo;
  s.fov = s.img + nlo;
  m->index_sets[B] = s;
  *out = s;
  return MD_OK;
}

int attention_f32(Run* r, hipStream_t st, const void* qk, const void* vT, void* out, float* scores, int nseq, int S, int n_tokens,
                  int heads, int kpad) {
  const int D = heads * 64;
  GemmParams p;
  p.N = S; p.K = 64; p.ngroups = 1; p.g_rows[0] = n_tokens;
  p.batch = nseq * heads; p.batch_inner = heads;
  p.A = qk; p.lda = 2 * D; p.a_bs[0] = (long)S * 2 * D; p.a_bs[1] = 64;
  p.W[0] = (const float*)qk + D; p.ldw = 2 * D; p.w_bs[0] = (long)S * 2 * D; p.w_bs[1] = 64;
  p.epi = EPI_STORE; p.out_f32 = 1; p.out = scores; p.ldo = kpad;
  p.o_bs[0] = (long)heads * S * kpad; p.o_bs[1] = (long)S * kpad;
  if (r) r->begin("attn_scores_f32");
  MD_TRY(launch_gemm(p, A_DENSE, MD_PREC_F32, TILE_128x128, st));
  if (r) r->end();
  if (r) r->begin("attn_softmax_f32");
  MD_TRY(launch_softmax_rows(scores, (long)nseq * heads * S, n_tokens, kpad, 0.125f, st));
  if (r) r->end();
  GemmParams q;
  q.N = 64; q.K = kpad; q.ngroups = 1; q.g_rows[0] = n_tokens;
  q.batch = nseq * heads; q.batch_inner = heads;
  q.A = scores; q.lda = kpad; q.a_bs[0] = (long)heads * S * kpad; q.a_bs[1] = (long)S * kpad;
  q.W[0] = vT; q.ldw = kpad; q.w_bs[0] = (long)heads * 64 * kpad; q.w_bs[1] = 64L * kpad;
  q.epi = EPI_STORE; q.out = out; q.ldo = D; q.o_bs[0] = (long)S * D; q.o_bs[1] = 64;
  if (r) r->begin("attn_pv_f32");
  MD_TRY(launch_gemm(q, A_DENSE, MD_PREC_F32, TILE_128x128, st));
  if (r) r->end();
  attention_note_form(ATTN_FORM_F32, (long)nseq * heads, 0, 0);
  return MD_OK;
}

void vit_add_packs(md_model_s* m, const std::string& prefix, const ViTDims& v) {
  const int D = v.D;
  add_pack(m, prefix + ".patch_embed.proj.weight", PACK_NK, D, 3 * v.ps * v.ps, 1);
  for (int i = 0; i < v.depth; ++i) {
    const std::string b = prefix + ".blocks." + std::to_string(i);
    add_pack(m, b + ".attn.qkv.weight", PACK_NK, 3 * D, D, 1);
    add_pack(m, b + ".attn.proj.weight", PACK_NK, D, D, 1);
    add_pack(m, b + ".mlp.fc1.weight", PACK_NK, 4 * D, D, 1);
    add_pack(m, b + ".mlp.fc2.weight", PACK_NK, D, 4 * D, 1);
  }
}

void vit_bind(md_model_s* m, const std::string& prefix, int depth, VitW& w) {
  w.pe_w = PK(m, prefix + ".patch_embed.proj.weight");
  w.pe_b = P32(m, prefix + ".patch_embed.proj.bias");
  w.cls = P32(m, prefix + ".cls_token");
  w.pos = P32(m, prefix + ".pos_embed");
  w.norm_g = P32(m, prefix + ".norm.gamma");
  w.norm_b = P32(m, prefix + ".norm.beta");
  for (int i = 0; i < depth; ++i) {
    const std::string b = prefix + ".blocks." + std::to_string(i);
    VitBlockW k;
    k.n1g = P32(m, b + ".norm1.gamma"); k.n1b = P32(m, b + ".norm1.beta");
    k.n2g = P32(m, b + ".norm2.gamma"); k.n2b = P32(m, b + ".norm2.beta");
    k.qkv_w = PK(m, b + ".attn.qkv.weight"); k.qkv_b = P32(m, b + ".attn.qkv.bias");
    k.proj_w = PK(m, b + ".attn.proj.weight"); k.proj_b = P32(m, b + ".attn.proj.bias");
    k.ls1 = P32(m, b + ".ls1.gamma"); k.ls2 = P32(m, b + ".ls2.gamma");
    k.fc1_w = PK(m, b + ".mlp.fc1.weight"); k.fc1_b = P32(m, b + ".mlp.fc1.bias");
    k.fc2_w = PK(m, b + ".mlp.fc2.weight"); k.fc2_b = P32(m, b + ".mlp.fc2.bias");
    k.w32[0] = P32(m, b + ".attn.qkv.weight"); k.w32[1] = P32(m, b + ".attn.proj.weight");
    k.w32[2] = P32(m, b + ".mlp.fc1.weight"); k.w32[3] = P32(m, b + ".mlp.fc2.weight");
    k.qkn_g[0] = P32(m, b + ".attn.q_norm.gamma"); k.qkn_b[0] = P32(m, b + ".attn.q_norm.beta");
    k.qkn_g[1] = P32(m, b + ".attn.k_norm.gamma"); k.qkn_b[1] = P32(m, b + ".attn.k_norm.beta");
    w.blk.push_back(k);
  }
}

int run_vit_block(Run& r, VitPlan& v, int i) {
  md_model_s* m = r.m;
  const int G = v.G, D = v.D, heads = v.heads, SS = v.SS, NT = v.NT;
  const size_t esz = (size_t)m->esz * m->xm;
  auto trow = [&](void* base, int width) { return (void*)((char*)base + (size_t)v.s_lo * SS * width * esz); };
  const long rows = (long)v.WS * SS;
  const VitBlockW& k0 = v.vit[0]->blk[i];
  const int depth = (int)v.vit[0]->blk.size();
  const bool f8 = v.lin_prec == MD_PREC_FP8;
  const float a_inv = f8 ? 1.0f / v.a_scale : 1.f;
  auto dense_a = [&](GemmParams& p, int K) {
    if (f8) { p.K = K; p.lda = K; } else split_dense_a(m, p, K, K, 0);
  };
  auto group_rows = [&](GemmParams& p) {
    p.ngroups = G;
    for (int g = 0; g < G; ++g) {
      p.g_row0[g] = v.glo[g] * SS;
      p.g_arow0[g] = v.glo[g] * SS;
      p.g_rows[g] = v.gcnt[g] * SS;
    }
  };
  SeqGroups sg;
  memset(&sg, 0, sizeof(sg));
  sg.ngroups = G;
  for (int g = 0; g < G; ++g) { sg.seq0[g] = v.glo[g] - v.s_lo; sg.nseq[g] = v.gcnt[g]; }
  auto layernorm = [&](bool norm2, const float* tok0) -> int {
    for (int g = 0; g < G; ++g) {
      const VitBlockW& k = v.vit[g]->blk[i];
      sg.a[g] = norm2 ? k.n2g : k.n1g; sg.b[g] = norm2 ? k.n2b : k.n1b;
    }
    float* x = v.x + (size_t)v.s_lo * SS * D;
    r.begin("layernorm");
    const int st_ = launch_layernorm(x, trow(v.xn, D), rows, D, v.ln_eps, SS, sg, v.lin_prec, 0, r.st, a_inv, tok0,
                                     tok0 ? v.tok0_stride : 0, tok0 ? x : nullptr);
    r.end();
    return st_;
  };
  const bool fold = v.fold, neutral = v.neutral;
  const bool fold1 = fold && i > 0;
  auto fold_producer = [&](GemmParams& p, int blk, bool norm2) {
    p.ln_out = v.xn; p.ln_ldo = (long)D * m->xm; p.ln_plane = m->xm == 2 ? D : 0;
    p.ln_stats_out = v.ln_stats; p.ln_parts = D / 256;
    for (int g = 0; g < G; ++g) p.ln_gamma[g] = norm2 ? v.vit[g]->blk[blk].n2g : v.vit[g]->blk[blk].n1g;
  };
  auto fold_consumer = [&](GemmParams& p) {
    p.ln_stats = v.finish_launch ? v.ln_ab : v.ln_stats; p.ln_raw = v.finish_launch ? 0 : 1;
    p.ln_parts = D / 256; p.ln_inv_n = 1.0f / (float)D; p.ln_eps = v.ln_eps;
  };
  auto fold_finish = [&]() -> int {
    if (!v.finish_launch) return MD_OK;
    r.begin("ln_finish");
    const int st_ = launch_ln_finish(v.ln_stats + (size_t)v.s_lo * SS * (D / 256) * 2, v.ln_ab + (size_t)v.s_lo * SS * 2, rows,
                                     1.0f / (float)D, v.ln_eps, r.st);
    r.end();
    return st_;
  };

  if (!fold1) MD_TRY(layernorm(false, i == v.tok0_block ? v.tok0 : nullptr));
  {
    GemmParams p;
    p.N = 3 * D; group_rows(p);
    for (int g = 0; g < G; ++g) {
      const VitBlockW& k = v.vit[g]->blk[i];
      p.W[g] = f8 ? k.w8[0] : k.qkv_w;
      p.wscale[g] = k.s8[0];
      p.bias[g] = fold1 ? k.qkv_d : k.qkv_b;
      if (fold1) p.ln_c[g] = k.qkv_c;
      if (neutral) p.ln_c[g] = v.zero_c;
    }
    if (fold1 || neutral) fold_consumer(p);
    p.A = v.xn;
    dense_a(p, D);
    p.v_plane = (long)m->vt_plane;
    p.epi = EPI_QKV; p.out = v.qk; p.vT = v.vT; p.seq_stride = SS; p.embed = D; p.heads = heads; p.kpad = v.kpad; p.qscale = attn_qscale(m->prec);
    if (f8) p.ascale = v.a_scale;
    if (k0.qkn_g[0] && !f8) {
      p.qkn_g[0] = k0.qkn_g[0]; p.qkn_b[0] = k0.qkn_b[0]; p.qkn_g[1] = k0.qkn_g[1]; p.qkn_b[1] = k0.qkn_b[1];
      p.qkn_eps = v.qk_norm_eps; p.rope_cos = v.rope_cos; p.rope_sin = v.rope_sin;
      p.rope_pw = v.rope_pw; p.rope_global = k0.global ? 1 : 0; p.rope_ntok = NT;
    }
    r.begin("qkv_gemm");
    MD_TRY(launch_gemm(p, A_DENSE, v.lin_prec, (fold1 || neutral) ? TILE_256x256 : TILE_AUTO, r.st));
    r.end();
  }
  if (k0.qkn_g[0] && f8) {
    r.begin("qk_norm_rope");
    MD_TRY(launch_qk_norm_rope(trow(v.qk, 2 * D), rows, SS, NT, D, heads, v.rope_pw, k0.qkn_g[0], k0.qkn_b[0], k0.qkn_g[1], k0.qkn_b[1],
                               v.qk_norm_eps, v.rope_cos, v.rope_sin, k0.global ? 1 : 0, attn_qscale(m->prec), m->prec, r.st));
    r.end();
  }
  void* vT_w = (char*)v.vT + (size_t)v.s_lo * heads * 64 * v.kpad * m->esz;
  if (v.views > 1 && k0.global) {
    if (m->prec == MD_PREC_F32 || f8) MD_FAIL(MD_ERR_UNSUPPORTED, "cross-view attention runs in the bf16, f16 and f16x2 modes");
    r.begin("attention_views");
    MD_TRY(launch_attention_views(trow(v.qk, 2 * D), vT_w, trow(v.ao, D), v.WS, v.views, SS, NT, heads, D, v.kpad, m->prec, r.st, (long)m->vt_plane));
    r.end();
  } else if (m->prec != MD_PREC_F32) {
    r.begin("attention");
    MD_TRY(launch_attention(trow(v.qk, 2 * D), vT_w, trow(v.ao, D), v.WS, SS, NT, heads, D, v.kpad, m->prec, r.st, f8 ? a_inv : 0.f,
                            (long)m->vt_plane, v.redo, v.redo_units));
    r.end();
  } else {
    MD_TRY(attention_f32(&r, r.st, trow(v.qk, 2 * D), vT_w, trow(v.ao, D), v.scores, v.WS, SS, NT, heads, v.kpad));
  }
  {
    GemmParams p;
    p.N = D; group_rows(p);
    for (int g = 0; g < G; ++g) {
      const VitBlockW& k = v.vit[g]->blk[i];
      p.W[g] = f8 ? k.w8[1] : k.proj_w; p.wscale[g] = k.s8[1]; p.bias[g] = k.proj_b; p.scale[g] = k.ls1;
    }
    p.A = v.ao;
    dense_a(p, D);
    p.epi = EPI_RESID_LS; p.out = v.x; p.ldo = D;
    if (k0.global) {
      p.resid_src = v.x; p.out = v.xalt;
      std::swap(v.x, v.xalt);
    }
    if (f8) p.ascale = v.a_scale;
    if (fold) fold_producer(p, i, true);
    r.begin("proj_gemm");
    MD_TRY(launch_gemm(p, A_DENSE, v.lin_prec, fold ? TILE_256x256 : TILE_AUTO, r.st));
    r.end();
    if (fold) MD_TRY(fold_finish());
  }
  if (!fold) MD_TRY(layernorm(true, nullptr));
  {
    GemmParams p;
    p.N = 4 * D; group_rows(p);
    for (int g = 0; g < G; ++g) {
      const VitBlockW& k = v.vit[g]->blk[i];
      p.W[g] = f8 ? k.w8[2] : k.fc1_w;
      p.wscale[g] = k.s8[2];
      p.bias[g] = fold ? k.fc1_d : k.fc1_b;
      if (fold) p.ln_c[g] = k.fc1_c;
      if (neutral) p.ln_c[g] = v.zero_c;
    }
    if (fold || neutral) fold_consumer(p);
    p.A = v.xn;
    dense_a(p, D);
    p.epi = EPI_STORE; p.act = ACT_GELU; p.out = v.hbuf;
    split_out(m, p, 4 * D, true);
    if (f8) { p.ascale = v.a_scale; p.out_fp8 = 1; p.out_inv_scale = 1.0f / v.h_scale; }
    r.begin("fc1_gemm");
    MD_TRY(launch_gemm(p, A_DENSE, v.lin_prec, (fold || neutral || f8) ? TILE_256x256 : TILE_AUTO, r.st));
    r.end();
  }
  {
    const bool fold_next = fold && i + 1 < depth;
    GemmParams p;
    p.N = D; group_rows(p);
    for (int g = 0; g < G; ++g) {
      const VitBlockW& k = v.vit[g]->blk[i];
      p.W[g] = f8 ? k.w8[3] : k.fc2_w; p.wscale[g] = k.s8[3]; p.bias[g] = k.fc2_b; p.scale[g] = k.ls2;
    }
    p.A = v.hbuf;
    dense_a(p, 4 * D);
    p.epi = EPI_RESID_LS; p.out = v.x; p.ldo = D;
    if (f8) p.ascale = v.h_scale;
    if (fold_next) fold_producer(p, i + 1, false);
    r.begin("fc2_gemm");
    MD_TRY(launch_gemm(p, A_DENSE, v.lin_prec, fold ? TILE_256x256 : TILE_AUTO, r.st));
    r.end();
    if (fold_next) MD_TRY(fold_finish());
  }
  return MD_OK;
}

static int run_vit(Run& r, int nseq_p, int nseq, int s_lo, int s_hi) {
  md_model_s* m = r.m;
  md_model_s::Buffers* b = m->buf;
  const ModelCfg& c = m->cfg;
  const int B = r.B, D = c.pv.D, P = m->P, SS = m->SS, NT = m->NT, heads = c.pv.heads;
  const int n0 = m->steps0 * m->steps0 * B, n1 = m->steps1 * m->steps1 * B;
  const int Kpe = 3 * c.pv.ps * c.pv.ps;
  const int gseq0[3] = {0, nseq_p, nseq_p + B};
  const int gnseq[3] = {nseq_p, B, B};
  if (s_lo < 0 || s_hi > nseq || s_lo > s_hi) MD_FAIL(MD_ERR_INVALID_ARG, "sequence window [%d, %d) of %d", s_lo, s_hi, nseq);
  const int WS = s_hi - s_lo;
  if (WS == 0) return MD_OK;
  int G = 0, gi[3], glo[3], gcnt[3];
  for (int g = 0; g < m->ngroups; ++g) {
    const int lo = std::max(gseq0[g], s_lo), hi = std::min(gseq0[g] + gnseq[g], s_hi);
    if (hi > lo) { gi[G] = g; glo[G] = lo; gcnt[G] = hi - lo; ++G; }
  }
  const size_t esz = (size_t)m->esz * m->xm;
  auto trow = [&](void* base, int width) { return (void*)((char*)base + (size_t)s_lo * SS * width * esz); };
  float* xres_w = b->xres + (size_t)s_lo * SS * D;

  SeqGroups sg;
  sg.ngroups = G;
  for (int g = 0; g < 4; ++g) { sg.seq0[g] = 0; sg.nseq[g] = 0; sg.a[g] = nullptr; sg.b[g] = nullptr; }
  for (int g = 0; g < G; ++g) { sg.seq0[g] = glo[g] - s_lo; sg.nseq[g] = gcnt[g]; }

  for (int g = 0; g < G; ++g) { sg.a[g] = m->vit[gi[g]].cls; sg.b[g] = m->vit[gi[g]].pos; }
  r.begin("cls_init");
  MD_TRY(launch_cls_init(xres_w, WS, SS, NT, D, sg, r.st));
  r.end();

  {
    GemmParams p;
    p.N = D; p.K = Kpe; p.ngroups = G;
    for (int g = 0; g < G; ++g) {
      p.g_row0[g] = glo[g] * P;
      p.g_rows[g] = gcnt[g] * P;
      p.g_arow0[g] = gi[g] == 0 ? glo[g] * P : (n0 + n1 + (glo[g] - gseq0[gi[g]])) * P;
      p.W[g] = m->vit[gi[g]].pe_w;
      p.bias[g] = m->vit[gi[g]].pe_b;
      p.pos[g] = m->vit[gi[g]].pos;
    }
    p.A = b->patches;
    split_dense_a(m, p, Kpe, Kpe, 0);
    p.epi = EPI_PATCH_EMBED; p.out = b->xres; p.ldo = D; p.seq_stride = SS; p.seq_patches = P; p.embed = D;
    r.begin("patch_embed");
    MD_TRY(launch_gemm(p, A_DENSE, m->prec, TILE_AUTO, r.st));
    r.end();
  }
  const long rows = (long)WS * SS;
  VitPlan v;
  v.G = G;
  for (int g = 0; g < G; ++g) { v.vit[g] = &m->vit[gi[g]]; v.glo[g] = glo[g]; v.gcnt[g] = gcnt[g]; }
  v.s_lo = s_lo; v.WS = WS;
  v.D = D; v.heads = heads; v.SS = SS; v.NT = NT; v.kpad = m->kpad; v.ln_eps = c.ln_eps;
  v.x = b->xres; v.xn = b->xn; v.qk = b->qk; v.vT = b->vT; v.ao = b->ao; v.hbuf = b->hbuf; v.scores = b->scores;
  v.redo = b->attn_redo; v.redo_units = b->attn_redo_units;
  v.lin_prec = m->prec;
  v.fold = m->ln_fold_on();
  v.neutral = !v.fold && m->ln_fold_can && m->ln_fold_opt == 3;
  v.finish_launch = v.neutral || m->ln_fold_opt == 4;
  v.ln_stats = b->ln_stats; v.ln_ab = b->ln_ab;
  v.zero_c = m->lnfold_base ? m->lnfold_base + (size_t)m->ngroups * c.pv.depth * 14 * D : nullptr;
  if (v.neutral) MD_TRY(launch_fill_pairs(b->ln_ab + (size_t)s_lo * SS * 2, rows, 1.0f, 0.0f, r.st));
  for (int i = 0; i < c.pv.depth; ++i) {
    MD_TRY(run_vit_block(r, v, i));
    for (int hk = 0; hk < 2; ++hk)
      if (c.pv.hook_ids[hk] == i) {
        const int h_lo = std::min(s_lo, n0), h_hi = std::min(s_hi, n0);
        if (h_hi > h_lo) {
          r.begin("hook_copy");
          MD_TRY(launch_convert_rows(b->xres + (size_t)h_lo * SS * D, (char*)b->hook[hk] + (size_t)h_lo * SS * D * esz,
                                     (long)(h_hi - h_lo) * SS * D, m->prec, r.st, D));
          r.end();
        }
      }
  }
  for (int g = 0; g < G; ++g) { sg.a[g] = m->vit[gi[g]].norm_g; sg.b[g] = m->vit[gi[g]].norm_b; }
  r.begin("layernorm");
  MD_TRY(launch_layernorm(xres_w, trow(b->tok, D), rows, D, c.ln_eps, SS, sg, m->prec, 0, r.st));
  r.end();
  return MD_OK;
}

static int run_encoder_tail(Run& r, const md_model_s::IndexSet& ix) {
  md_model_s* m = r.m;
  md_model_s::Buffers* b = m->buf;
  const ModelCfg& c = m->cfg;
  const int B = r.B, D = c.pv.D, F = c.F, g = m->g;
  const int* dims = c.pv.feat_dims;
  const int hi = m->mh_hi, mid = m->mh_mid;
  const long Mhi = (long)B * hi * hi, Mmid = (long)B * mid * mid, Mlo = (long)B * g * g;
  const DepthProW& w = m->dp;
  MD_TRY(gemm_rows(r, "enc_proj", b->hook[0], D, ix.hi, Mhi, w.enc_proj[0], dims[0], D,
                   nullptr, b->l0p, cpad(m, dims[0])));
  MD_TRY(deconv2(r, "enc_deconv", b->l0p, cpad(m, dims[0]), nullptr, hi, hi, w.enc_up[0],
                 cpad(m, dims[0]), F, nullptr, b->l0a, cpad(m, F), 0));
  MD_TRY(deconv2(r, "enc_deconv", b->l0a, cpad(m, F), nullptr, 2 * hi, 2 * hi, w.latent0_1x2,
                 cpad(m, F), F, nullptr, b->enc0, cpad(m, F), 0, b->enc0r, 4, 3));
  MD_TRY(gemm_rows(r, "enc_proj", b->hook[1], D, ix.hi, Mhi, w.enc_proj[1], dims[0], D,
                   nullptr, b->l1p, cpad(m, dims[0])));
  MD_TRY(deconv2(r, "enc_deconv", b->l1p, cpad(m, dims[0]), nullptr, hi, hi, w.enc_up[1],
                 cpad(m, dims[0]), dims[0], nullptr, b->enc1, cpad(m, dims[0]), 0, nullptr, 4, 3));
  MD_TRY(gemm_rows(r, "enc_proj", b->tok, D, ix.hi, Mhi, w.enc_proj[2], dims[1], D, nullptr,
                   b->x0p, cpad(m, dims[1])));
  MD_TRY(deconv2(r, "enc_deconv", b->x0p, cpad(m, dims[1]), nullptr, hi, hi, w.enc_up[2],
                 cpad(m, dims[1]), dims[1], nullptr, b->enc2, cpad(m, dims[1]), 0));
  MD_TRY(gemm_rows(r, "enc_proj", b->tok, D, ix.mid, Mmid, w.enc_proj[3], dims[2], D, nullptr,
                   b->x1p, cpad(m, dims[2])));
  MD_TRY(deconv2(r, "enc_deconv", b->x1p, cpad(m, dims[2]), nullptr, mid, mid, w.enc_up[3],
                 cpad(m, dims[2]), dims[2], nullptr, b->enc3, cpad(m, dims[2]), 0));
  const int catld = 2 * cpad(m, dims[3]);
  MD_TRY(gemm_rows(r, "enc_proj", b->tok, D, ix.x2, Mlo, w.enc_proj[4], dims[3], D, nullptr,
                   b->x2p, cpad(m, dims[3])));
  MD_TRY(deconv2(r, "enc_deconv", b->x2p, cpad(m, dims[3]), nullptr, g, g, w.enc_up[4],
                 cpad(m, dims[3]), dims[3], nullptr, b->cat, catld, 0));
  MD_TRY(deconv2(r, "enc_deconv", b->tok, D, ix.img, g, g, w.lowres.w, D, dims[3], w.lowres.b, b->cat, catld, cpad(m, dims[3])));
  MD_TRY(gemm_rows(r, "enc_fuse", b->cat, catld, nullptr, Mlo * 4, w.fuse.w, dims[3], catld, w.fuse.b, b->enc4, cpad(m, dims[3])));
  if (m->taps_enabled) {
    MD_TRY(r.tap_nhwc("encoder_feature_0", b->enc0, F, 8 * hi, 8 * hi, cpad(m, F)));
    MD_TRY(r.tap_nhwc("encoder_feature_1", b->enc1, dims[0], 4 * hi, 4 * hi, cpad(m, dims[0])));
    MD_TRY(r.tap_nhwc("encoder_feature_2", b->enc2, dims[1], 2 * hi, 2 * hi, cpad(m, dims[1])));
    MD_TRY(r.tap_nhwc("encoder_feature_3", b->enc3, dims[2], 2 * mid, 2 * mid, cpad(m, dims[2])));
    MD_TRY(r.tap_nhwc("encoder_feature_4", b->enc4, dims[3], 2 * g, 2 * g, cpad(m, dims[3])));
  }
  return MD_OK;
}

static int run_decoder_head(Run& r, bool decoder_only = false) {
  md_model_s* m = r.m;
  md_model_s::Buffers* b = m->buf;
  const ModelCfg& c = m->cfg;
  const int F = c.F, Fp = cpad(m, F);
  const int* dims = c.pv.feat_dims;
  int hw[5];
  level_sizes(m, hw);
  const int ddims[5] = {F, dims[0], dims[1], dims[2], dims[3]};
  const void* enc[5] = {b->enc0, b->enc1, b->enc2, b->enc3, b->enc4};
  const DepthProW& w = m->dp;
  const bool fused_c0 = w.outconv_conv0.w != nullptr && hw[0] >= 2;
  const void* feats = nullptr;
  for (int l = 4; l >= 0; --l) {
    const void *pj, *pjr;
    if (l == 0) {
      pj = b->enc0;
      pjr = b->enc0r;
    } else {
      const ConvW cv{w.convs[l], nullptr};
      MD_TRY(conv3(r, "dec_conv3x3", enc[l], hw[l], hw[l], cpad(m, ddims[l]), &cv, F, b->proj[l], Fp, ACT_NONE, nullptr, nullptr, b->projr[l]));
      pj = b->proj[l];
      pjr = b->projr[l];
    }
    const void *x, *xr;
    if (l == 4) {
      if (m->taps_enabled) MD_TRY(r.tap_nhwc("decoder_lowres_feature", pj, F, hw[4], hw[4], Fp));
      x = pj;
      xr = pjr;
    } else {
      MD_TRY(residual_unit(r, "dec_conv3x3", &w.res[l][0], 1, hw[l], hw[l], Fp, F, pj, pjr, false, feats, b->dt[l], b->dx[l], b->dxr[l]));
      x = b->dx[l];
      xr = b->dxr[l];
    }
    MD_TRY(residual_unit(r, "dec_conv3x3", &w.res[l][1], 1, hw[l], hw[l], Fp, F, x, xr, false, nullptr, b->dt[l], b->dy[l], nullptr));
    int ohw = hw[l];
    if (l != 0) {
      MD_TRY(deconv2(r, "dec_deconv_out", b->dy[l], Fp, nullptr, hw[l], hw[l], w.out[l].w, Fp, F, w.out[l].b, b->df[l], Fp, 0, nullptr, 2, 3));
      ohw = 2 * hw[l];
    } else if (!fused_c0 || m->taps_enabled) {
      MD_TRY(gemm_rows(r, "dec_out_conv", b->dy[l], Fp, nullptr, (long)r.B * ohw * ohw, w.out[l].w, F, Fp, w.out[l].b, b->df[l],
                       Fp));
    }
    feats = b->df[l];
    if (m->taps_enabled) {
      const std::string tn = "decoder_fusion_" + std::to_string(l);
      MD_TRY(r.tap_nhwc(tn.c_str(), feats, F, ohw, ohw, Fp));
    }
  }
  if (m->taps_enabled) MD_TRY(r.tap_nhwc("decoder_feature", feats, F, hw[0], hw[0], Fp));
  if (decoder_only) return MD_OK;
  const int F2 = F / 2, F2p = cpad(m, F2);
  if (fused_c0) {
    const float* bias9 = w.outconv_conv0.b;
    const ConvW c0{w.outconv_conv0.w, bias9 + 4 * F2};
    MD_TRY(conv3(r, "head_conv0", b->dy[0], hw[0], hw[0], Fp, &c0, F2, b->h0, F2p, ACT_NONE, nullptr, nullptr, nullptr, 3));
    r.begin("head_conv0");
    MD_TRY(launch_border_bias_fix(b->h0, r.B, hw[0], hw[0], F2, F2p, bias9, m->prec, r.st));
    r.end();
  } else {
    MD_TRY(conv3(r, "head_conv0", feats, hw[0], hw[0], Fp, &w.conv0, F2, b->h0, F2p, ACT_NONE, nullptr, nullptr, nullptr));
  }
  if (m->taps_enabled) {
    MD_TRY(deconv2(r, "head_deconv_tap", b->h0, F2p, nullptr, hw[0], hw[0], w.deconv.w, F2p, F2, w.deconv.b, b->h1, F2p, 0));
    MD_TRY(r.tap_nhwc("head_conv0", b->h0, F2, hw[0], hw[0], F2p));
    MD_TRY(r.tap_nhwc("head_deconv", b->h1, F2, 2 * hw[0], 2 * hw[0], F2p));
  }
  {
    GemmParams p;
    p.N = 4 * 32; p.ngroups = 1; p.g_rows[0] = r.B * hw[0] * hw[0]; p.W[0] = w.deconv_conv1.w;
    p.A = b->h0; p.cH = hw[0]; p.cW = hw[0]; p.zero_page = m->zero_page;
    split_conv_a(m, p, F2p, 3);
// ... 351 lines not shown
  return model_infer_eager(m, nchw, B, H, W, in_kind, depth, focal, fovx, fovy, out_kind, stream, nullptr, 0, nullptr, 0, &sp);
}

static int model_infer_eager(md_model_t m, const float* nchw, int B, int H, int W, int in_kind, float* depth, float* focal,
                             float* fovx, float* fovy, int out_kind, hipStream_t stream, const uint8_t* rgb, size_t rgb_len,
                             const float* f_px, int f_kind, const ShardPlan* sp) {
  if (!m) MD_FAIL(MD_ERR_INVALID_ARG, "model is null");
  if (!model_root(m)->committed) MD_FAIL(MD_ERR_INVALID_ARG, "weights were modified; call md_model_commit_weights first");
  if (!nchw && !rgb) MD_FAIL(MD_ERR_INVALID_ARG, "input pointer is null");
  if (B <= 0 || H <= 0 || W <= 0) MD_FAIL(MD_ERR_SHAPE, "invalid input shape [%d,3,%d,%d]", B, H, W);
  if (B > m->cfg.max_batch) MD_FAIL(MD_ERR_SHAPE, "batch %d exceeds max_batch %d", B, m->cfg.max_batch);
  const bool known_focal = f_px != nullptr;
  if (known_focal && sp) MD_FAIL(MD_ERR_INVALID_ARG, "the tile-parallel mode takes no focal length");
  if (!known_focal && !m->cfg.use_fov_head) MD_FAIL(MD_ERR_NO_FOV, "FOV head required for focal length");
  if (known_focal && f_kind == MD_MEM_HOST)
    for (int i = 0; i < B; ++i)
      if (!std::isfinite(f_px[i]) || !(f_px[i] > 0.f)) MD_FAIL(MD_ERR_INVALID_ARG, "f_px[%d] = %g: a focal length must be finite and > 0", i, (double)f_px[i]);
  MD_HIP(hipSetDevice(m->dev->ordinal));
  hipStream_t st = model_stream(m, stream);
  md_model_s::Buffers* b = m->buf;
  Run r{m, st, B};
  const float* fpx_dev = f_px;
  if (known_focal && f_kind == MD_MEM_HOST) {
    MD_TRY(grow(m, st, b->fpx, (size_t)B * 4));
    MD_TRY(stage_host_to_device(m, b->fpx.p, f_px, (size_t)B * 4, st, &b->pin_fpx));
    fpx_dev = b->fpx.p;
  }
  const int S = m->S;
  const size_t in_elems = (size_t)B * 3 * H * W;
  const bool resize_needed = H != S || W != S;
  const float* x_dev = nullptr;
  if (rgb) {
    if (rgb_len != (size_t)W * H * 3) MD_FAIL(MD_ERR_SHAPE, "expected %zu RGB bytes for %dx%d, got %zu", (size_t)W * H * 3, W, H, rgb_len);
    const uint8_t* rgb_dev = rgb;
    if (in_kind == MD_MEM_HOST) {
      MD_TRY(grow(m, st, b->rgb, rgb_len));
      MD_TRY(stage_host_to_device(m, b->rgb.p, rgb, rgb_len, st));
      rgb_dev = b->rgb.p;
    }
    float* dst = b->xin;
    if (resize_needed) {
      MD_TRY(grow(m, st, b->xraw, in_elems * 4));
      dst = b->xraw.p;
    }
    r.begin("rgb_to_input");
    MD_TRY(launch_rgb_to_input(rgb_dev, W, H, dst, st));
    r.end();
    x_dev = dst;
  } else if (in_kind == MD_MEM_HOST) {
    float* dst = b->xin;
    if (resize_needed) {
      MD_TRY(grow(m, st, b->xraw, in_elems * 4));
      dst = b->xraw.p;
    }
    MD_TRY(stage_host_to_device(m, dst, nchw, in_elems * 4, st));
    x_dev = dst;
  } else {
    x_dev = nchw;
  }
  if (resize_needed) {
    r.begin("resize_in");
    MD_TRY(launch_resize_bilinear(x_dev, B * 3, H, W, b->xin, S, S, m->cfg.interpolation, 0, st));
    r.end();
    x_dev = b->xin;
  }
  const int n0 = m->steps0 * m->steps0 * B, n1 = m->steps1 * m->steps1 * B;
  const int nseq_p = n0 + n1 + B;
  const int nseq = nseq_p + B * (m->ngroups - 1);
  PyramidGeom pg{B, S, m->win, m->cfg.pv.ps, m->steps0, m->stride0, m->steps1, m->stride1, m->cfg.interpolation};
  r.begin("pyramid_patchify");
  MD_TRY(launch_pyramid_patchify(x_dev, pg, b->patches, m->prec, st));
  r.end();
  md_model_s::IndexSet ix;
  MD_TRY(get_index_set(m, B, &ix));
  struct EventSet {
    hipEvent_t e[66] = {};
    ~EventSet() {
      for (hipEvent_t x : e)
        if (x) (void)hipEventDestroy(x);
    }
  } ev_set;
  hipEvent_t* ev_w = ev_set.e;
  const bool time_windows = sp && sp->part < 0 && (sp->window_ms || sp->tail_ms) && sp->parts <= 64;
  if (!sp) {
    MD_TRY(run_vit(r, nseq_p, nseq, 0, known_focal ? nseq_p + B : nseq));
  } else {
    auto lo_of = [&](int p) { return (int)((long)nseq * p / sp->parts); };
    if (sp->part < 0) {
      for (int p = 0; p < sp->parts; ++p) {
        if (time_windows) { MD_HIP(hipEventCreate(&ev_w[p])); MD_HIP(hipEventRecord(ev_w[p], st)); }
        MD_TRY(run_vit(r, nseq_p, nseq, lo_of(p), lo_of(p + 1)));
      }
      if (time_windows) { MD_HIP(hipEventCreate(&ev_w[sp->parts])); MD_HIP(hipEventRecord(ev_w[sp->parts], st)); }
    } else {
      MD_TRY(run_vit(r, nseq_p, nseq, lo_of(sp->part), lo_of(sp->part + 1)));
      if (sp->parts > 1) {
        const size_t rowb = (size_t)m->SS * m->cfg.pv.D * m->esz * m->xm;
        std::vector<ShardSegment> segs((size_t)sp->parts * 3);
        for (int p = 0; p < sp->parts; ++p) {
          const int lo = lo_of(p), hi = lo_of(p + 1), hlo = std::min(lo, n0), hhi = std::min(hi, n0);
          segs[3 * p + 0] = {(char*)b->tok + (size_t)lo * rowb, (size_t)(hi - lo) * rowb};
          segs[3 * p + 1] = {(char*)b->hook[0] + (size_t)hlo * rowb, (size_t)(hhi - hlo) * rowb};
          segs[3 * p + 2] = {(char*)b->hook[1] + (size_t)hlo * rowb, (size_t)(hhi - hlo) * rowb};
        }
        MD_TRY(sp->exchange(sp->ctx, sp->parts, (const ShardSegment(*)[3])segs.data(), st));
      }
      if (sp->part != sp->root) return MD_OK;
    }
  }
  auto finish_timing = [&]() -> int {
    if (!time_windows) return MD_OK;
    const int np = sp->parts;
    MD_HIP(hipEventCreate(&ev_w[np + 1]));
    MD_HIP(hipEventRecord(ev_w[np + 1], st));
    MD_HIP(hipEventSynchronize(ev_w[np + 1]));
    for (int p = 0; p < np; ++p)
      if (sp->window_ms) MD_HIP(hipEventElapsedTime(&sp->window_ms[p], ev_w[p], ev_w[p + 1]));
    if (sp->tail_ms) MD_HIP(hipEventElapsedTime(sp->tail_ms, ev_w[np], ev_w[np + 1]));
    return MD_OK;
  };
  MD_TRY(run_encoder_tail(r, ix));
  MD_TRY(run_decoder_head(r));
  if (!known_focal) {
    MD_TRY(run_fov(r, ix));
    r.begin("fov_post");
    MD_TRY(launch_fov_post(b->fov_deg, B, H, W, b->focal, b->fovy, b->ratio, st));
    r.end();
  } else {
    auto tp = m->taps.find("fov_deg");
    hipStreamCaptureStatus cs = hipStreamCaptureStatusNone;
    if (tp != m->taps.end() && hipStreamIsCapturing(st, &cs) == hipSuccess && cs == hipStreamCaptureStatusNone) {
      if (tp->second.dev) MD_HIP(hipFree(tp->second.dev));
      m->taps.erase(tp);
    }
    r.begin("focal_post");
    MD_TRY(launch_focal_post(fpx_dev, B, H, W, b->focal, b->fov_deg, b->fovy, b->ratio, st));
    r.end();
  }
  const size_t out_elems = (size_t)B * H * W;
  float* depth_dev = nullptr;
  if (depth) {
    if (out_kind == MD_MEM_DEVICE) {
      depth_dev = depth;
    } else {
      MD_TRY(grow(m, st, b->depth_stage, out_elems * 4));
      depth_dev = b->depth_stage.p;
    }
    r.begin("depth_post");
    if (!resize_needed) {
      MD_TRY(launch_depth_post(b->canonical, b->ratio, B, (long)S * S, depth_dev, 1, st));
      r.end();
    } else {
      MD_TRY(launch_depth_post(b->canonical, b->ratio, B, (long)S * S, b->inv, 0, st));
      r.end();
      r.begin("resize_out");
      MD_TRY(launch_resize_bilinear(b->inv, B, S, S, depth_dev, H, W, m->cfg.interpolation, 1, st));
      r.end();
    }
  }
  if (out_kind == MD_MEM_HOST) {
    const size_t dbytes = depth ? out_elems * 4 : 0, need = dbytes + 3 * (size_t)B * 4;
    MD_TRY(grow(m, st, b->pin_out, need));
    char* ph = (char*)b->pin_out.p;
    if (depth) MD_HIP(hipMemcpyAsync(ph, depth_dev, dbytes, hipMemcpyDeviceToHost, st));
    const float* srcs[3] = {b->focal, b->fov_deg, b->fovy};
    float* dsts[3] = {focal, fovx, fovy};
    for (int i = 0; i < 3; ++i)
      if (dsts[i]) MD_HIP(hipMemcpyAsync(ph + dbytes + (size_t)i * B * 4, srcs[i], (size_t)B * 4, hipMemcpyDeviceToHost, st));
    MD_HIP(hipStreamSynchronize(st));
    if (depth) memcpy(depth, ph, dbytes);
    for (int i = 0; i < 3; ++i)
      if (dsts[i]) memcpy(dsts[i], ph + dbytes + (size_t)i * B * 4, (size_t)B * 4);
    return finish_timing();
  }
  auto copy_out = [&](float* dst, const float* src, size_t n) -> int {
    if (!dst) return MD_OK;
    MD_HIP(hipMemcpyAsync(dst, src, n * 4, hipMemcpyDeviceToDevice, st));
    return MD_OK;
  };
  MD_TRY(copy_out(focal, b->focal, B));
  MD_TRY(copy_out(fovx, b->fov_deg, B));
  MD_TRY(copy_out(fovy, b->fovy, B));
  return finish_timing();
}

}
```

### burn_depth_amd/csrc/md_engine_util.h

```cpp
#pragma once

#include <algorithm>
#include <string>

#include "md_engine.h"

namespace md {

inline int round_up(int v, int a) { return (v + a - 1) / a * a; }

inline size_t pack_elems(const PackEntry& e, int terms = 1) {
  const size_t kpt = (size_t)e.kp * terms;
  switch (e.kind) {
    case PACK_NK: return (size_t)e.d0 * kpt;
    case PACK_CONV3: return (size_t)e.d0 * 9 * kpt;
    case PACK_DECONV: return (size_t)e.k * e.k * e.d1 * kpt;
    case PACK_HEAD_W: return (size_t)4 * e.d0 * 9 * kpt;
    case PACK_HEAD_B: return (size_t)9 * e.d0;
    case PACK_C1C3_W: return (size_t)e.d0 * 9 * kpt;
    case PACK_C1C3_B: return (size_t)9 * e.d0;
    default: return (size_t)e.d0 * e.d1 * e.k * e.k;
  }
}
inline size_t pack_bytes(const md_model_s* m, const PackEntry& e) {
// ... 202 lines not shown
  p.N = f * f * Cout; p.ngroups = 1; p.g_rows[0] = B * h * w; p.W[0] = W; p.ps_f = f;
  p.A = A; p.a_index = idx;
  split_dense_a(m, p, Cin_p, lda, terms);
  p.epi = EPI_PIXSHUF; p.bias[0] = bias; p.out = out; p.out2 = out2;
  split_out(m, p, ldo, true);
  p.psH = h; p.psW = w; p.psC = Cout; p.ps_coff = coff;
  return p;
}
inline int deconv2(Run& r, const char* name, const void* A, long lda, const int* idx, int h, int w, const void* W, int Cin_p,
            int Cout, const float* bias, void* out, long ldo, int coff, void* out2 = nullptr, int f = 2, int terms = 0) {
  const GemmParams p = deconv2_params(geom_of(r.m), r.B, A, lda, idx, h, w, W, Cin_p, Cout, bias, out, ldo, coff, out2, f, terms);
  r.begin(name);
  int s = launch_gemm(p, idx ? A_INDEXED : A_DENSE, r.m->prec, TILE_AUTO, r.st);
  r.end();
  return s;
}

inline GemmParams conv3_params(const OperandGeom& m, int B, const void* in, int H, int W, int Cin_p, const ConvW* w, int Cout, void* out,
                                long ldo, int act, const void* res1, const void* res2, void* out2, int terms = 0, int G = 1,
                                bool in_shared = false, bool res1_shared = false) {
  GemmParams p;
  const int M = B * H * W;
  p.N = Cout; p.ngroups = G;
  for (int g = 0; g < G; ++g) {
    p.g_rows[g] = M; p.g_row0[g] = g * M; p.g_arow0[g] = in_shared ? 0 : g * M;
    p.W[g] = w[g].w; p.bias[g] = w[g].b;
  }
  p.A = in; p.cH = H; p.cW = W; p.zero_page = m.zero_page;
  split_conv_a(m, p, Cin_p, terms);
  p.epi = EPI_STORE; p.act = act; p.out = out; p.out2 = out2;
  split_out(m, p, ldo, true);
  p.res1 = res1; p.res2 = res2; p.ldr = p.ldo; p.r_plane = (res1 || res2) ? p.o_plane : 0;
  if (res1 && res1_shared && G > 1) p.res_mod = M;
  return p;
}
inline int conv3(Run& r, const char* name, const void* in, int H, int W, int Cin_p, const ConvW* w, int Cout, void* out, long ldo,
                 int act, const void* res1, const void* res2, void* out2, int terms = 0, int G = 1, bool in_shared = false,
                 bool res1_shared = false) {
  const GemmParams p = conv3_params(geom_of(r.m), r.B, in, H, W, Cin_p, w, Cout, out, ldo, act, res1, res2, out2, terms, G, in_shared, res1_shared);
  r.begin(name);
  int s = launch_gemm(p, A_CONV3, r.m->prec, TILE_AUTO, r.st);
  r.end();
  return s;
}

inline int residual_unit(Run& r, const char* name, const ResUnitW* u, int G, int H, int W, int Cp, int C, const void* x,
                         const void* xr, bool x_shared, const void* extra, void* t, void* out, void* out_relu) {
  const ConvW c1[2] = {u[0].c1, u[G - 1].c1}, c2[2] = {u[0].c2, u[G - 1].c2};
  MD_TRY(conv3(r, name, xr, H, W, Cp, c1, C, t, Cp, ACT_RELU, nullptr, nullptr, nullptr, 0, G, x_shared));
  return conv3(r, name, t, H, W, Cp, c2, C, out, Cp, ACT_NONE, x, extra, out_relu, 0, G, false, x_shared);
}

int attention_f32(Run* r, hipStream_t st, const void* qk, const void* vT, void* out, float* scores, int nseq, int S, int n_tokens,
                  int heads, int kpad);

void vit_add_packs(md_model_s* m, const std::string& prefix, const ViTDims& v);
void vit_bind(md_model_s* m, const std::string& prefix, int depth, VitW& w);

struct VitPlan {
  int G = 1;
  const VitW* vit[3] = {nullptr, nullptr, nullptr};
  int glo[3] = {0, 0, 0}, gcnt[3] = {0, 0, 0};
  int s_lo = 0, WS = 0;
  int views = 1;
  int D = 0, heads = 0, SS = 0, NT = 0, kpad = 0;
  float ln_eps = 0.f;
  float* x = nullptr;
  float* xalt = nullptr;
  void *xn = nullptr, *qk = nullptr, *vT = nullptr, *ao = nullptr, *hbuf = nullptr;
  float* scores = nullptr;
  int* redo = nullptr;
  int redo_units = 0;
  bool fold = false, neutral = false, finish_launch = false;
  float *ln_stats = nullptr, *ln_ab = nullptr;
  const float* zero_c = nullptr;
  int lin_prec = MD_PREC_BF16;
  float a_scale = 0.f, h_scale = 0.f;
  float qk_norm_eps = 0.f;
  const float *rope_cos = nullptr, *rope_sin = nullptr;
  int rope_pw = 0;
  int tok0_block = -1;
  const float* tok0 = nullptr;
  int tok0_stride = 0;
};
int run_vit_block(Run& r, VitPlan& v, int i);


}
```

### burn_depth_amd/ops.py

```python
from __future__ import annotations

import ctypes as C
from typing import Optional, Tuple

import torch

from . import _lib
from .depth_pro import Device, _stream_ptr
from .points import (FittedPlanes, PointCloud, RasterisedMesh, RenderedPoints, SmoothedMesh, _cluster_mode_of, _clusters_struct, _f32, _i32, _lattice,
                     _new_clusters, _plane_mode, _planes_struct, _points_cameras, _points_request, _ptr,
                     _raster_request, _render_request, _u8, _view_filter_opts)


def _p(t: Optional[torch.Tensor]) -> C.c_void_p:
    return C.c_void_p(t.data_ptr()) if t is not None else C.c_void_p(0)


def _f32c(t: torch.Tensor) -> torch.Tensor:
    assert t.is_cuda, "operators take device tensors"
    return t.contiguous().to(torch.float32)


def resize_bilinear(dev: Device, x: torch.Tensor, out_hw: Tuple[int, int], method: int = 0) -> torch.Tensor:
    x = _f32c(x)
# ... 257 lines not shown
def layernorm_ex(dev: Device, x: torch.Tensor, S: int, groups, eps: float, precision: int, out_f32: bool = False,
                 fp8_inv_scale: float = 1.0, tok0: Optional[torch.Tensor] = None, tok0_stride: int = 0):
    x = _f32c(x).clone()
    rows, D = x.shape
    n = len(groups)
    keep = [(None if g is None else _f32c(g), None if b is None else _f32c(b)) for _, _, g, b in groups]
    seq0, nseq = (C.c_int * n)(*[int(g[0]) for g in groups]), (C.c_int * n)(*[int(g[1]) for g in groups])
    ga = (C.c_void_p * n)(*[t[0].data_ptr() if t[0] is not None else None for t in keep])
    be = (C.c_void_p * n)(*[t[1].data_ptr() if t[1] is not None else None for t in keep])
    if tok0 is not None:
        tok0 = _f32c(tok0)
        assert tok0.numel() >= ((rows + S - 1) // S - 1) * tok0_stride + D, "tok0 is shorter than the sequences read from it"
    out = torch.empty((rows, D), dtype=torch.float32, device=x.device) if out_f32 else _raw_empty((rows,), D, precision, x.device)
    _lib.check(_lib.load().md_op_layernorm_ex(dev.handle, _p(x), rows, D, S, n, seq0, nseq, ga, be, C.c_float(eps), precision, int(out_f32),
                                              C.c_float(fp8_inv_scale), _p(tok0), tok0_stride, _p(out), _stream_ptr(dev.ordinal)))
    del keep
    return out, (x if tok0 is not None else None)


def store_rows(dev: Device, x: torch.Tensor, width: int, precision: int) -> torch.Tensor:
    x = _f32c(x).reshape(-1)
    out = _raw_empty((x.numel() // max(width, 1),), width, precision, x.device) if width else _raw_empty((), x.numel(), precision, x.device)
    _lib.check(_lib.load().md_op_store_rows(dev.handle, _p(x), x.numel(), width, precision, _p(out), _stream_ptr(dev.ordinal)))
    return out


def load_rows(dev: Device, raw: torch.Tensor, count: int, width: int, precision: int) -> torch.Tensor:
    assert raw.is_cuda and raw.is_contiguous() and raw.dtype == _RAW_DTYPE[precision] and raw.numel() == count * (2 if precision == 4 else 1)
    out = torch.empty(count, dtype=torch.float32, device=raw.device)
    _lib.check(_lib.load().md_op_load_rows(dev.handle, _p(raw), count, width, precision, _p(out), _stream_ptr(dev.ordinal)))
    return out


def f32_to_fp8(dev: Device, x: torch.Tensor, inv_scale: float) -> torch.Tensor:
    x = _f32c(x)
    out = torch.empty(x.shape, dtype=torch.uint8, device=x.device)
    _lib.check(_lib.load().md_op_f32_to_fp8(dev.handle, _p(x), x.numel(), C.c_float(inv_scale), _p(out), _stream_ptr(dev.ordinal)))
    return out


def pack_fp8_rows(dev: Device, w: torch.Tensor, Kp: int) -> Tuple[torch.Tensor, torch.Tensor]:
    w = _f32c(w)
    N, K = w.shape
    out = torch.full((N, max(Kp, 0)), 0x55, dtype=torch.uint8, device=w.device)
    scale = torch.empty(N, dtype=torch.float32, device=w.device)
    _lib.check(_lib.load().md_op_pack_fp8_rows(dev.handle, _p(w), N, K, Kp, _p(out), _p(scale), _stream_ptr(dev.ordinal)))
    return out, scale


def nchw_to_nhwc(dev: Device, x: torch.Tensor, precision: int, relu: bool, ld: int, out: torch.Tensor) -> torch.Tensor:
    x, out = _f32c(x), out.contiguous().clone()
    B, Cn, H, W = x.shape
    assert out.is_cuda and out.dtype == _RAW_DTYPE[precision] and out.numel() == B * H * W * (ld or Cn) * (2 if precision == 4 else 1)
    _lib.check(_lib.load().md_op_nchw_to_nhwc(dev.handle, _p(x), B, Cn, H, W, precision, int(relu), ld, _p(out), _stream_ptr(dev.ordinal)))
    return out


def nhwc_to_nchw(dev: Device, raw: torch.Tensor, Cn: int, ld: int, coff: int, precision: int) -> torch.Tensor:
    assert raw.is_cuda and raw.is_contiguous() and raw.dtype == _RAW_DTYPE[precision] and raw.shape[3] == ld * (2 if precision == 4 else 1)
    B, H, W, _ = raw.shape
    out = torch.empty((B, Cn, H, W), dtype=torch.float32, device=raw.device)
    _lib.check(_lib.load().md_op_nhwc_to_nchw(dev.handle, _p(raw), B, Cn, H, W, ld, coff, precision, _p(out), _stream_ptr(dev.ordinal)))
    return out


def ln_fold_vectors(dev: Device, w: torch.Tensor, gamma: torch.Tensor, beta: torch.Tensor, bias: Optional[torch.Tensor],
                    precision: int) -> Tuple[torch.Tensor, torch.Tensor]:
    w, gamma, beta = _f32c(w), _f32c(gamma), _f32c(beta)
    bias = _f32c(bias) if bias is not None else None
    N, K = w.shape
    c, d = torch.empty(N, dtype=torch.float32, device=w.device), torch.empty(N, dtype=torch.float32, device=w.device)
    _lib.check(_lib.load().md_op_ln_fold_vectors(dev.handle, _p(w), _p(gamma), _p(beta), _p(bias), N, K, precision, _p(c), _p(d),
                                                 _stream_ptr(dev.ordinal)))
    return c, d


def ln_finish(dev: Device, parts: torch.Tensor, inv_n: float, eps: float) -> torch.Tensor:
    parts = _f32c(parts)
    rows = parts.shape[0]
    assert parts.shape == (rows, 4, 2)
    ab = torch.empty((rows, 2), dtype=torch.float32, device=parts.device)
    _lib.check(_lib.load().md_op_ln_finish(dev.handle, _p(parts), rows, C.c_float(inv_n), C.c_float(eps), _p(ab), _stream_ptr(dev.ordinal)))
    return ab


def vit_gemm(dev: Device, kind: int, a: torch.Tensor, groups, precision: int, tile: int = _lib.TILE_AUTO, *, x: Optional[torch.Tensor] = None,
             x_out: Optional[torch.Tensor] = None, ln_out: Optional[torch.Tensor] = None, ln_stats_out: Optional[torch.Tensor] = None,
             ln_stats: Optional[torch.Tensor] = None, ln_raw: bool = False, ln_eps: float = 0.0, ln_inv_n: float = 0.0, S: int = 0, D: int = 0,
             P: int = 0, qk: Optional[torch.Tensor] = None, vT: Optional[torch.Tensor] = None, out: Optional[torch.Tensor] = None) -> None:
    tensors = [a, x, x_out, ln_out, ln_stats_out, ln_stats, qk, vT, out] + [g.get(k) for g in groups for k in ("w", "bias", "scale", "gamma_next", "c", "pos")]
    for t in tensors:
        assert t is None or (t.is_cuda and t.is_contiguous() and t.dtype == torch.float32), "vit_gemm takes contiguous fp32 device tensors"
    d = _lib.MdVitGemm()
    d.kind, d.precision, d.tile = kind, precision, tile
    d.N, d.K = groups[0]["w"].shape
    d.a_rows, d.a, d.ngroups = a.shape[0], a.data_ptr(), len(groups)
    assert a.shape[1] == d.K and 1 <= len(groups) <= 4
    for i, g in enumerate(groups):
        assert g["w"].shape == (d.N, d.K) and g["bias"].shape == (d.N,)
        d.g[i].row0, d.g[i].rows, d.g[i].arow0 = g["row0"], g["rows"], g.get("arow0", g["row0"])
        for k in ("w", "bias", "scale", "gamma_next", "c", "pos"):
            setattr(d.g[i], k, g[k].data_ptr() if g.get(k) is not None else None)
    first = next(t for t in (x, qk, out) if t is not None)
    d.out_rows = first.shape[0]
    for name, t, cols in (("x", x, d.N), ("x_out", x_out, d.N), ("ln_out", ln_out, d.N), ("out", out, d.N), ("qk", qk, 2 * D)):
        assert t is None or t.shape == (d.out_rows, cols), name
        setattr(d, name, t.data_ptr() if t is not None else None)
    assert ln_stats_out is None or ln_stats_out.shape == (d.out_rows, d.N // 256, 2)
    assert ln_stats is None or ln_stats.shape == ((d.out_rows, 4, 2) if ln_raw else (d.out_rows, 2))
    assert vT is None or vT.shape == (d.out_rows // S, D // 64, 64, (S + 63) // 64 * 64)
    d.ln_stats_out = ln_stats_out.data_ptr() if ln_stats_out is not None else None
    d.ln_stats = ln_stats.data_ptr() if ln_stats is not None else None
    d.vT = vT.data_ptr() if vT is not None else None
    d.ln_raw, d.ln_eps, d.ln_inv_n, d.S, d.D, d.P = int(ln_raw), ln_eps, ln_inv_n, S, D, P
    _lib.check(_lib.load().md_op_vit_gemm(dev.handle, C.byref(d), _stream_ptr(dev.ordinal)))


def gemm_last_form() -> dict:
    v, n = (C.c_int * 8)(), (C.c_int * 4)()
    _lib.check(_lib.load().md_debug_gemm_last_form(C.byref(v)))
    _lib.check(_lib.load().md_debug_gemm_last_launch(C.byref(n)))
    return dict(zip(("family", "ek", "fold", "qkv", "conv", "diag", "blocks", "grid", "tile", "ps_fast"), list(v) + list(n)[:2]))


def decoder_gemm(dev: Device, kind: int, x: torch.Tensor, w, bias, precision: int, tile: int = _lib.TILE_AUTO, *, B: int, H: int, W: int, Cin: int,
                 Cin_p: int, Cout: int, out: Optional[torch.Tensor] = None, ldo: int = 0, act: int = 0, res1: Optional[torch.Tensor] = None,
                 res2: Optional[torch.Tensor] = None, res_mod: int = 0, out2: Optional[torch.Tensor] = None, in_shared: bool = False,
                 res1_shared: bool = False, out_f32: bool = False, ps_f: int = 2, ps_coff: int = 0, head=None, head_w: Optional[torch.Tensor] = None,
                 head_b: float = 0.0, head_act: int = 0, Cmid: int = 0, w2: Optional[torch.Tensor] = None, bias2: Optional[torch.Tensor] = None) -> None:
    ws = list(w) if isinstance(w, (list, tuple)) else [w]
    bs = list(bias) if isinstance(bias, (list, tuple)) else [bias] * len(ws)
    G, xm, raw = len(ws), (2 if precision == 4 else 1), _RAW_DTYPE.get(precision)
    conv, s2, ps, hd, up2 = (kind == k for k in range(5))
    assert 1 <= G <= 2 and len(bs) == G and (G == 1 or conv)
    OH, OW = ((H - 1) // 2 + 1, (W - 1) // 2 + 1) if s2 else ((ps_f * H, ps_f * W) if ps else (H, W))
    f32s = [t for t in ws + bs + [head_w, w2, bias2] if t is not None]
    for t in f32s:
        assert t.is_cuda and t.is_contiguous() and t.dtype == torch.float32, "weights and biases are contiguous fp32 device tensors"
    taps = ps_f * ps_f if ps else (4 if up2 else 9)
    for t in ws:
        assert t.numel() == Cin * (Cmid if up2 else Cout) * taps, "weight shape"
    for t in bs:
        assert t is None or t.numel() == (Cmid if up2 else Cout), "bias shape"

    def holds(t, elems, dtype, what):
        ok = t.numel() >= elems if what.startswith("out") else t.numel() == elems
        assert t.is_cuda and t.is_contiguous() and t.dtype == dtype and ok, f"{what}: {tuple(t.shape)} {t.dtype}, expected {elems} of {dtype}"

    holds(x, (1 if in_shared else G) * B * H * W * Cin_p * xm, raw, "x")
    d = _lib.MdDecoderGemm()
    d.kind, d.precision, d.tile, d.B, d.H, d.W, d.Cin, d.Cin_p, d.Cout, d.ngroups = kind, precision, tile, B, H, W, Cin, Cin_p, Cout, G
    d.in_shared, d.res1_shared, d.act, d.res_mod, d.ldo, d.out_f32, d.ps_f, d.ps_coff = int(in_shared), int(res1_shared), act, res_mod, ldo, int(out_f32), ps_f, ps_coff
    for g in range(G):
        d.w[g], d.bias[g] = ws[g].data_ptr(), (bs[g].data_ptr() if bs[g] is not None else None)
    d.in_ = x.data_ptr()
    if conv or s2 or ps:
        if out_f32:
            holds(out, B * OH * OW * Cout, torch.float32, "out")
        else:
            assert ldo >= (ps_coff if ps else 0) + Cout
            holds(out, G * B * OH * OW * ldo * xm, raw, "out")
        if out2 is not None:
            holds(out2, G * B * OH * OW * ldo * xm, raw, "out2")
        if res1 is not None:
            holds(res1, (res_mod if res_mod else (1 if res1_shared else G) * B * OH * OW) * ldo * xm, raw, "res1")
        if res2 is not None:
# ... 321 lines not shown
```

### include/mi_depth.h

```cpp
#ifndef MI_DEPTH_H
#define MI_DEPTH_H

#include <stddef.h>
#include <stdint.h>

#ifdef __cplusplus
extern "C" {
#endif

typedef struct md_device_s* md_device_t;
typedef struct md_model_s* md_model_t;

typedef enum md_status {
  MD_OK = 0,
  MD_ERR_INVALID_ARG = -1,
  MD_ERR_SHAPE = -2,
  MD_ERR_IO = -3,
  MD_ERR_FORMAT = -4,
  MD_ERR_HIP = -5,
  MD_ERR_UNSUPPORTED = -6,
  MD_ERR_NO_FOV = -7,
  MD_ERR_OOM = -8,
  MD_ERR_LEVELS = -9
} md_status;
// ... 447 lines not shown
int md_model_read_tap(md_model_t m, const char* name, float* host_data, size_t capacity, int64_t dims[4]);

int md_op_rgb_to_input(md_device_t dev, const uint8_t* rgb_dev, size_t rgb_len, int w, int h, float* out_dev,
                       void* stream);
int md_op_resize_bilinear(md_device_t dev, const float* in_dev, int B, int C, int H, int W, float* out_dev,
                          int OH, int OW, int method, void* stream);
int md_op_pyramid_patchify(md_device_t dev, const float* x_dev, int B, int S, int window, int patch, int method, int precision,
                           int force_generic, void* out_dev, int* rows_out, int* cols_out, void* stream);
int md_op_resize_nhwc(md_device_t dev, const void* in_dev, int B, int H, int W, int C, void* out_dev, int OH, int OW,
                      int method, int precision, void* stream);
int md_catmull_rom_taps(int in_len, int out_len, int index, int* left, int* count, float* weights);
int md_op_resize_catmull_rom(md_device_t dev, const uint8_t* rgb_dev, int B, int h, int w, int sw, int sh, int cx, int cy,
                             int tw, int th, uint8_t* out_u8, float* out_nchw, void* stream);
int md_op_depth_display(md_device_t dev, const float* depth_dev, int B, int h, int w, int crop_x, int crop_y, int crop_w,
                        int crop_h, int ow, int oh, int normalize, int format, void* out, float* range, void* stream);
int md_op_resize_output_size(int H, int W, float scale_h, float scale_w, int* oh, int* ow);
int md_op_split(md_device_t dev, const float* in_dev, int B, int C, int S, int window, float overlap,
                float* out_dev, int* steps_out, void* stream);
int md_op_merge(md_device_t dev, const float* in_dev, int tiles, int C, int h, int w, int batch, int padding,
                float* out_dev, int* out_h, int* out_w, void* stream);
int md_op_layernorm(md_device_t dev, const float* x_dev, const float* gamma_dev, const float* beta_dev, int rows,
                    int D, float eps, float* out_dev, void* stream);
int md_op_linear(md_device_t dev, const float* x_dev, const float* w_dev, const float* bias_dev, int M, int N,
                 int K, int act, int precision, float* out_dev, void* stream);
int md_op_linear_tile(md_device_t dev, const float* x_dev, const float* w_dev, const float* bias_dev, int M, int N,
                      int K, int act, int precision, int tile, float* out_dev, void* stream);
int md_op_attention(md_device_t dev, const float* qkv_dev, int T, int N, int heads, int precision, float* out_dev,
                    void* stream);
int md_op_attention_views(md_device_t dev, const float* qkv_dev, int T, int V, int N, int heads, int precision, float* out_dev,
                          void* stream);
typedef struct md_attention_op {
  int T, V, N, heads;
  int precision;
  int seq_stride;
  int kpad;
  float out_fp8_inv;
  int small;
  int poison_pad;
  const float* qkv;
  void* out;
} md_attention_op;
int md_op_attention_ex(md_device_t dev, const md_attention_op* desc, void* stream);
typedef enum md_attention_form {
  MD_ATTN_FORM_NONE = -1, MD_ATTN_FORM_PLAIN = 0, MD_ATTN_FORM_KEY_SPLIT = 1, MD_ATTN_FORM_ASSEMBLY = 2, MD_ATTN_FORM_VIEWS = 3,
  MD_ATTN_FORM_FP8_OUT = 4, MD_ATTN_FORM_F32_PATH = 5
} md_attention_form;
int md_debug_attention_last_form(int out[4]);
int md_op_conv3x3(md_device_t dev, const float* x_dev, const float* w_dev, const float* bias_dev, int B, int Cin,
                  int H, int W, int Cout, int pre_relu, int precision, float* out_dev, void* stream);
int md_op_deconv2x2(md_device_t dev, const float* x_dev, const float* w_dev, const float* bias_dev, int B, int Cin,
                    int H, int W, int Cout, int precision, float* out_dev, void* stream);
int md_op_conv2d_direct(md_device_t dev, const float* x_dev, const float* w_dev, const float* bias_dev, int B,
                        int Cin, int H, int W, int Cout, int k, int stride, int pad, int relu, float* out_dev,
                        void* stream);
int md_op_qkv_norm_rope(md_device_t dev, const float* x_dev, const float* w_dev, const float* bias_dev, const float* q_gamma,
                        const float* q_beta, const float* k_gamma, const float* k_beta, int T, int S, int n_tokens, int K, int D,
                        int pw, int global_pos, float rope_frequency, float eps, int precision, int tile, int form,
                        float* qk_out, float* vt_out, void* stream);
int md_op_qk_norm_rope(md_device_t dev, const float* qk_in, const float* q_gamma, const float* q_beta, const float* k_gamma,
                       const float* k_beta, int T, int S, int n_tokens, int D, int pw, int global_pos, float rope_frequency,
                       float eps, int precision, float* qk_out, void* stream);
int md_op_hook_cat_ln(md_device_t dev, const float* x_local, const float* x, int T, int S, int n_tokens, int D,
                      const float* norm_g, const float* norm_b, float eps_final, const float* head_g, const float* head_b,
                      float eps_head, int precision, float* out, float* cam_out, void* stream);
int md_op_patchify(md_device_t dev, const float* x_dev, int B, int H, int W, int ps, int Kp, int precision, float* out,
                   float* cls_x, int S, int n_tokens, int D, const float* cls, const float* pos0, void* stream);
int md_op_set_token0(md_device_t dev, float* x, int nseq, int S, int D, const float* src, int src_stride, void* stream);
int md_op_border_bias_fix(md_device_t dev, float* map, int B, int H, int W, int C, int ld, const float* bias9, int precision,
                          void* stream);
int md_op_layernorm_ex(md_device_t dev, float* x, int rows, int D, int S, int ngroups, const int* seq0, const int* nseq,
                       const float* const* gamma, const float* const* beta, float eps, int precision, int out_f32, float fp8_inv_scale,
                       const float* tok0, int tok0_stride, void* out, void* stream);
int md_op_store_rows(md_device_t dev, const float* in, int64_t count, int width, int precision, void* out, void* stream);
int md_op_load_rows(md_device_t dev, const void* in, int64_t count, int width, int precision, float* out, void* stream);
int md_op_f32_to_fp8(md_device_t dev, const float* in, int64_t count, float inv_scale, void* out, void* stream);
int md_op_pack_fp8_rows(md_device_t dev, const float* w, int N, int K, int Kp, void* out, float* scale, void* stream);
int md_op_nchw_to_nhwc(md_device_t dev, const float* in, int B, int C, int H, int W, int precision, int relu, int ld, void* out,
                       void* stream);
int md_op_nhwc_to_nchw(md_device_t dev, const void* in, int B, int C, int H, int W, int ld, int coff, int precision, float* out,
                       void* stream);
int md_op_ln_fold_vectors(md_device_t dev, const float* w, const float* gamma, const float* beta, const float* bias, int N, int K,
                          int precision, float* c, float* d, void* stream);
int md_op_ln_finish(md_device_t dev, const float* parts, int64_t rows, float inv_n, float eps, float* ab, void* stream);
typedef enum md_vit_gemm_kind { MD_VIT_GEMM_RESID = 0, MD_VIT_GEMM_QKV = 1, MD_VIT_GEMM_FC1 = 2, MD_VIT_GEMM_PATCH_EMBED = 3 } md_vit_gemm_kind;
typedef struct md_vit_gemm_group {
  int row0, rows, arow0;
  const float* w;
  const float* bias;
  const float* scale;
  const float* gamma_next;
  const float* c;
  const float* pos;
} md_vit_gemm_group;
typedef struct md_vit_gemm {
  int kind, precision, tile;
  int N, K;
  int a_rows;
  const float* a;
  int ngroups;
  md_vit_gemm_group g[4];
  int out_rows;
  float* x;
  float* x_out;
  float* ln_out;
  float* ln_stats_out;
  const float* ln_stats;
  int ln_raw;
  float ln_eps, ln_inv_n;
  int S, D;
  int P;
  float* qk;
  float* vT;
  float* out;
} md_vit_gemm;
int md_op_vit_gemm(md_device_t dev, const md_vit_gemm* desc, void* stream);
int md_debug_gemm_last_form(int out[8]);
int md_debug_gemm_last_launch(int out[4]);
typedef enum md_decoder_gemm_kind {
  MD_DECODER_GEMM_CONV3 = 0,
  MD_DECODER_GEMM_CONV3_S2 = 1,
  MD_DECODER_GEMM_PIXSHUF = 2,
  MD_DECODER_GEMM_HEAD = 3,
  MD_DECODER_GEMM_HEAD_UP2 = 4
} md_decoder_gemm_kind;
typedef struct md_decoder_gemm_head_ch {
  const float* w;
  float b;
  int act;
  float* out;
  int64_t bstride;
} md_decoder_gemm_head_ch;
typedef struct md_decoder_gemm {
  int kind, precision, tile;
  int B, H, W;
  int Cin, Cin_p;
  int Cout;
  int ngroups;
  int in_shared, res1_shared;
  const float* w[2];
  const float* bias[2];
  const void* in;
  int act;
  const void* res1;
  const void* res2;
  int res_mod;
  void* out;
  void* out2;
  int ldo;
  int out_f32;
  int ps_f, ps_coff;
  int head_nch;
  md_decoder_gemm_head_ch ch[8];
  const float* head_w;
  float head_b;
  int head_act;
  int Cmid;
  const float* w2;
  const float* bias2;
} md_decoder_gemm;
int md_op_decoder_gemm(md_device_t dev, const md_decoder_gemm* desc, void* stream);
typedef struct md_camera_encode {
  int B, V, D, heads, depth;
  int H, W;
  float eps_tok, eps_blk;
  const float* w[8];
  const float* blk[8][14];
  const float* extr;
  const float* intr;
  float* out;
  float* pose_out;
} md_camera_encode;
int md_op_camera_encode(md_device_t dev, const md_camera_encode* desc, void* stream);
typedef struct md_camera_decode {
  int B, din, H, W;
  const float* cam;
  const float* w[10];
  float* pose;
  float* extr;
  float* intr;
} md_camera_decode;
int md_op_camera_decode(md_device_t dev, const md_camera_decode* desc, void* stream);
int md_op_pose_to_camera(md_device_t dev, const float* pose, int B, int H, int W, float* extr, float* intr, void* stream);
int md_op_conv2d_direct_ex(md_device_t dev, const float* x_dev, const float* w_dev, const float* bias_dev, const float* add_dev, int B,
                           int Cin, int H, int W, int Cout, int k, int stride, int pad, int relu, int in_precision, int out_ld,
                           float* out_dev, void* stream);
int md_op_fov_to_focal(float fovx_deg, int H, int W, float* focal_px, float* fovy_rad);
int md_op_focal_to_fov(float f_px, int H, int W, float* fovx_deg, float* fovy_rad);

int md_bench_gemm(md_device_t dev, int mode, int M, int N, int K, int aux0, int aux1, int precision, int tile, int iters,
                  float* avg_ms);
int md_gemm_pick_tile(int M, int N, int K, int precision);
int md_gemm_ksplit_launches(void);
int md_debug_gemm_direct_store(int on);
int md_debug_gemm_persistent(int mask);
int md_debug_gemm_stagger(int which, int ticks);
int md_debug_gemm_stagger_ticks(int which);
int md_bench_attention(md_device_t dev, int T, int n_tokens, int heads, int iters, float* avg_ms);
int md_bench_attention_ex(md_device_t dev, int T, int n_tokens, int heads, int precision, float qk_scale, int iters,
                          float* avg_ms);
int md_bench_attention_qkv(md_device_t dev, const float* qkv_dev, int T, int n_tokens, int heads, int precision, int iters,
                           float* avg_ms, long* redo_units_per_launch);
int md_debug_attention_asm(int on);
long md_debug_attention_asm_launches(void);
long md_debug_attention_redo_units(md_device_t dev, int reset);

typedef struct md_comm_s* md_comm_t;
#define MD_COMM_ID_BYTES 128
int md_comm_unique_id(uint8_t id[MD_COMM_ID_BYTES]);
int md_comm_init_rank(md_device_t dev, const uint8_t id[MD_COMM_ID_BYTES], int world_size, int rank, md_comm_t* out);
int md_comm_rank(md_comm_t c, int* rank, int* world_size);
int md_comm_count(md_comm_t c, int* ranks_seen);
int md_comm_destroy(md_comm_t c);
int md_comm_broadcast_weights(md_comm_t c, md_model_t m, int root);
int md_comm_scatter_images(md_comm_t c, const float* all_dev, float* shard_dev, size_t elems_per_rank, int root, void* stream);
int md_comm_gather_depth(md_comm_t c, const float* shard_dev, float* all_dev, size_t elems_per_rank, int root, void* stream);

int md_comm_depth_pro_infer_tiles(md_comm_t comm, md_model_t model, const float* nchw, int B, int H, int W, int in_kind,
                                  float* depth, float* focallength_px, float* fovx_deg, float* fovy_rad, int out_kind,
                                  int root, void* stream);
int md_depth_pro_infer_tiles_loopback(const md_model_t* models, int parts, int root, const float* nchw, int B, int H, int W,
                                      int in_kind, float* depth, float* focallength_px, float* fovx_deg, float* fovy_rad,
                                      int out_kind, void* stream);

int md_param_inventory(const md_depth_pro_cfg* cfg, int init_scheme, int index, const char** name, size_t* count,
                       float* lo, float* hi);
int md_uniform_stream(const char* name, uint64_t seed, size_t count, float lo, float hi, float* out_host);
int md_split_geometry(int image_size, int window, float overlap, int* stride, int* steps);
int md_feature_padding(int window, int stride, int feature_size);

int md_model_enable_timing(md_model_t m, int enable);
int md_model_set_timing_filter(md_model_t m, const char* family);
int md_model_read_timing(md_model_t m, const char** names, float* ms, int* calls, int cap, int* n);
int md_model_read_launch_order(md_model_t m, const char** names, int cap, int* n);

#ifdef __cplusplus
}
#endif
#endif
```

Before: 55.45 frames/s.

## Compute last ViT block's post-attention work only on token rows the merge keeps

```diff
diff --git a/burn_depth_amd/_lib.py b/burn_depth_amd/_lib.py
--- a/burn_depth_amd/_lib.py
+++ b/burn_depth_amd/_lib.py
@@ -358,6 +358,8 @@
     "md_uniform_stream": (_I, [C.c_char_p, C.c_uint64, C.c_size_t, C.c_float, C.c_float, _P]),
     "md_split_geometry": (_I, [_I, _I, C.c_float, C.POINTER(_I), C.POINTER(_I)]),
     "md_feature_padding": (_I, [_I, _I, _I]),
+    "md_debug_last_block_rows": (_I, [_I, _I, _I, _I, C.POINTER(C.c_int64 * 12), _P, _P, _P]),
+    "md_op_compact_rows": (_I, [_P, _P, _I, _P, _I, _P, C.c_int64, C.c_int64, _P, _P, _P]),
 }
 
 
diff --git a/burn_depth_amd/csrc/kernels/ops.h b/burn_depth_amd/csrc/kernels/ops.h
--- a/burn_depth_amd/csrc/kernels/ops.h
+++ b/burn_depth_amd/csrc/kernels/ops.h
@@ -339,6 +339,8 @@
 int launch_fill_pairs(float* ab, long rows, float a, float b, hipStream_t s);
 int launch_ln_finish(const float* parts, float* ab, long rows, float inv_n, float eps, hipStream_t s);
 int launch_convert_rows(const float* x, void* out, long count, int prec, hipStream_t s, int width = 0);
+int launch_compact_rows(const void* a, void* a_c, int a_bytes, const void* x, void* x_c, int x_bytes, const int* list, long n,
+                        hipStream_t s);
 
 int launch_nchw_to_nhwc(const float* in, int B, int C, int H, int W, void* out, int prec, int relu, hipStream_t s, long ld = 0);
 int launch_head_tail_debug(const void* relu_map, long ld, long pixels, int C, const float* w, const float* bias, float* pre_out,
diff --git a/burn_depth_amd/csrc/kernels/ops.hip b/burn_depth_amd/csrc/kernels/ops.hip
--- a/burn_depth_amd/csrc/kernels/ops.hip
+++ b/burn_depth_amd/csrc/kernels/ops.hip
@@ -791,6 +791,41 @@
 int launch_rows_to_f32(const void* in, long count, float* out, int prec, hipStream_t s, int width) {
   if (prec == MD_PREC_F16X2 && (width <= 0 || count % width != 0)) MD_FAIL(MD_ERR_INVALID_ARG, "rows_to_f32: split-half rows need the row width");
   MD_BY_PREC(prec, hipLaunchKernelGGL(rows_to_f32_kernel<T>, dim3(grid_for(count)), dim3(256), 0, s, (const T*)in, count, out, width));
+  MD_HIP(hipGetLastError());
+  return MD_OK;
+}
+
+__global__ __launch_bounds__(256) void compact_rows_kernel(const char* __restrict__ a, char* __restrict__ a_c, int a_bytes,
+                                                           const char* __restrict__ x, char* __restrict__ x_c, int x_bytes,
+                                                           const int* __restrict__ list, long n) {
+  const int o0 = (threadIdx.x & 63) * 16;
+  const long wave_id = (blockIdx.x * (long)blockDim.x + threadIdx.x) >> 6;
+  const long nwaves = ((long)gridDim.x * blockDim.x) >> 6;
+  for (long i = wave_id; i < n; i += nwaves) {
+    const long src = list[i];
+    i32x4_t va[4], vx[4];
+#pragma unroll
+    for (int k = 0; k < 4; ++k) {
+      const int o = o0 + k * 1024;
+      if (o < a_bytes) va[k] = *(const i32x4_t*)(a + src * a_bytes + o);
+      if (o < x_bytes) vx[k] = *(const i32x4_t*)(x + src * x_bytes + o);
+    }
+#pragma unroll
+    for (int k = 0; k < 4; ++k) {
+      const int o = o0 + k * 1024;
+      if (o < a_bytes) *(i32x4_t*)(a_c + i * a_bytes + o) = va[k];
+      if (o < x_bytes) *(i32x4_t*)(x_c + i * x_bytes + o) = vx[k];
+    }
+  }
+}
+
+int launch_compact_rows(const void* a, void* a_c, int a_bytes, const void* x, void* x_c, int x_bytes, const int* list, long n,
+                        hipStream_t s) {
+  if (!a || !a_c || !x || !x_c || !list || n <= 0) MD_FAIL(MD_ERR_INVALID_ARG, "compact_rows: invalid argument");
+  if (a_bytes <= 0 || x_bytes <= 0 || a_bytes % 16 != 0 || x_bytes % 16 != 0 || a_bytes > 4096 || x_bytes > 4096)
+    MD_FAIL(MD_ERR_UNSUPPORTED, "compact_rows: rows of %d / %d bytes (multiples of 16 up to 4096)", a_bytes, x_bytes);
+  hipLaunchKernelGGL(compact_rows_kernel, dim3(grid_for(n * 64)), dim3(256), 0, s, (const char*)a, (char*)a_c, a_bytes, (const char*)x,
+                     (char*)x_c, x_bytes, list, n);
   MD_HIP(hipGetLastError());
   return MD_OK;
 }
diff --git a/burn_depth_amd/csrc/md_api.cpp b/burn_depth_amd/csrc/md_api.cpp
--- a/burn_depth_amd/csrc/md_api.cpp
+++ b/burn_depth_amd/csrc/md_api.cpp
@@ -395,6 +395,9 @@
   else if (k == "batch_invariant") *out = m->batch_invariant ? 1 : 0;
   else if (k == "ln_fold") *out = m->ln_fold_opt;
   else if (k == "ln_fold_active") *out = m->ln_fold_on() ? 1 : 0;
+  else if (k == "last_block_rows") *out = m->last_block_rows_opt ? 1 : 0;
+  else if (k == "last_block_rows_active") *out = m->last_block_rows_off == 0 ? 1 : 0;
+  else if (k == "last_block_rows_off") *out = m->last_block_rows_off;
   else if (model_decoder_query(m, k, out)) {}
   else MD_FAIL(MD_ERR_INVALID_ARG, "unknown query key `%s`", key);
   return MD_OK;
@@ -418,6 +421,17 @@
     if (value >= 2 && !m->ln_fold_can) MD_FAIL(MD_ERR_UNSUPPORTED, "ln_fold: this model cannot fold its LayerNorms (16-bit Depth Pro models of width %% 256 == 0 can)");
     if (m->ln_fold_opt != (int)value) {
       m->ln_fold_opt = (int)value;
+      MD_HIP(hipSetDevice(m->dev->ordinal));
+      MD_HIP(hipDeviceSynchronize());
+      m->graphs.clear();
+    }
+    return MD_OK;
+  }
+  if (k == "last_block_rows") {
+    if (value != 0 && value != 1) MD_FAIL(MD_ERR_INVALID_ARG, "last_block_rows takes 0 or 1");
+    if (m->kind != 0) MD_FAIL(MD_ERR_UNSUPPORTED, "last_block_rows: a Depth Pro option (its encoder's merge drops token rows)");
+    if (m->last_block_rows_opt != (value != 0)) {
+      m->last_block_rows_opt = value != 0;
       MD_HIP(hipSetDevice(m->dev->ordinal));
       MD_HIP(hipDeviceSynchronize());
       m->graphs.clear();
@@ -1326,6 +1340,23 @@
   OpStage s;
   MD_TRY(s.open(dev, stream));
   MD_TRY(launch_ln_finish(parts, ab, (long)rows, inv_n, eps, s.st));
+  return s.finish();
+}
+
+int md_op_compact_rows(md_device_t dev, const void* a, int a_bytes, const void* x, int x_bytes, const int32_t* list, int64_t n,
+                       int64_t src_rows, void* a_c, void* x_c, void* stream) {
+  if (!dev) MD_FAIL(MD_ERR_INVALID_ARG, "null argument");
+  if (n <= 0 || src_rows <= 0) MD_FAIL(MD_ERR_SHAPE, "compact_rows: n=%lld of %lld rows", (long long)n, (long long)src_rows);
+  OpStage s;
+  MD_TRY(s.open(dev, stream));
+  {
+    std::vector<int32_t> h((size_t)n);
+    MD_HIP(hipMemcpyAsync(h.data(), list, (size_t)n * 4, hipMemcpyDeviceToHost, s.st));
+    MD_HIP(hipStreamSynchronize(s.st));
+    for (int64_t i = 0; i < n; ++i)
+      if (h[(size_t)i] < 0 || h[(size_t)i] >= src_rows) MD_FAIL(MD_ERR_INVALID_ARG, "compact_rows: list[%lld] = %d outside %lld rows", (long long)i, h[(size_t)i], (long long)src_rows);
+  }
+  MD_TRY(launch_compact_rows(a, a_c, a_bytes, x, x_c, x_bytes, list, (long)n, s.st));
   return s.finish();
 }
 
@@ -2037,4 +2068,30 @@
 
 int md_feature_padding(int window, int stride, int feature_size) { return feature_padding(window, stride, feature_size); }
 
-}
+int md_debug_last_block_rows(int window, int patch, int B, int with_fov, int64_t* counts, int32_t* tables, int32_t* kept, int32_t* remapped) {
+  if (!counts || window <= 0 || patch <= 0 || window % patch != 0 || B <= 0) MD_FAIL(MD_ERR_INVALID_ARG, "invalid argument");
+  TokenGeom t;
+  int stride0 = 0, stride1 = 0;
+  t.g = window / patch;
+  t.SS = (t.g * t.g + 1 + 3) / 4 * 4;
+  split_geometry(4 * window, window, 0.25f, &stride0, &t.steps0);
+  split_geometry(2 * window, window, 0.5f, &stride1, &t.steps1);
+  t.pad_hi = feature_padding(window, stride0, t.g);
+  t.pad_mid = feature_padding(window, stride1, t.g);
+  t.mh_hi = merged_extent(t.g, t.steps0, t.pad_hi);
+  t.mh_mid = merged_extent(t.g, t.steps1, t.pad_mid);
+  std::vector<int> blob;
+  size_t off[6];
+  build_index_tables(t, B, &blob, off);
+  KeptRows k;
+  build_kept_rows(t, B, blob, off, with_fov ? 5 : 4, &k);
+  for (int i = 0; i < 5; ++i) counts[i] = (int64_t)(off[i + 1] - off[i]);
+  counts[5] = (int64_t)k.rows.size();
+  for (int g = 0; g < 3; ++g) { counts[6 + g] = k.grow0[g]; counts[9 + g] = k.grows[g]; }
+  if (tables) memcpy(tables, blob.data(), blob.size() * 4);
+  if (kept) memcpy(kept, k.rows.data(), k.rows.size() * 4);
+  if (remapped) memcpy(remapped, k.remap.data(), k.remap.size() * 4);
+  return MD_OK;
+}
+
+}
diff --git a/burn_depth_amd/csrc/md_engine.h b/burn_depth_amd/csrc/md_engine.h
--- a/burn_depth_amd/csrc/md_engine.h
+++ b/burn_depth_amd/csrc/md_engine.h
@@ -34,6 +34,17 @@
 int feature_padding(int patch_size, int stride, int feature_patch_size);
 void merge_source(int Y, int X, int h, int w, int steps, int pad, int* j, int* i, int* ty, int* tx);
 int merged_extent(int h, int steps, int pad);
+
+struct TokenGeom {
+  int g = 0, SS = 0, steps0 = 0, steps1 = 0, pad_hi = 0, pad_mid = 0, mh_hi = 0, mh_mid = 0;
+};
+void build_index_tables(const TokenGeom& t, int B, std::vector<int>* blob, size_t off[6]);
+struct KeptRows {
+  std::vector<int> rows;
+  std::vector<int> remap;
+  int grow0[3] = {0, 0, 0}, grows[3] = {0, 0, 0};
+};
+void build_kept_rows(const TokenGeom& t, int B, const std::vector<int>& blob, const size_t off[6], int ntables, KeptRows* out);
 
 enum PackKind : int { PACK_NK = 0, PACK_CONV3 = 1, PACK_DECONV = 2, PACK_DIRECT = 3, PACK_HEAD_W = 4, PACK_HEAD_B = 5, PACK_C1C3_W = 6, PACK_C1C3_B = 7 };
 
@@ -199,6 +210,16 @@
     int *hi = nullptr, *mid = nullptr, *x2 = nullptr, *img = nullptr, *fov = nullptr;
   };
   std::map<int, IndexSet> index_sets;
+  struct LastRows {
+    int* blob = nullptr;
+    int* list = nullptr;
+    int n = 0;
+    IndexSet ix;
+    int grow0[3] = {0, 0, 0}, grows[3] = {0, 0, 0};
+  };
+  std::map<std::pair<int, int>, LastRows> last_rows;
+  bool last_block_rows_opt = true;
+  int last_block_rows_off = 1;
 
   bool taps_enabled = false;
   std::map<std::string, md::Tap> taps;
diff --git a/burn_depth_amd/csrc/md_engine.hip b/burn_depth_amd/csrc/md_engine.hip
--- a/burn_depth_amd/csrc/md_engine.hip
+++ b/burn_depth_amd/csrc/md_engine.hip
@@ -621,6 +621,7 @@
   if (m->ws.base) (void)hipFree(m->ws.base);
   if (m->zero_page) (void)hipFree(m->zero_page);
   for (auto& kv : m->index_tables) (void)hipFree(kv.second);
+  for (auto& kv : m->last_rows) (void)hipFree(kv.second.blob);
   m->graphs.clear();
   for (auto& kv : m->taps) (void)hipFree(kv.second.dev);
   for (auto& t : m->timing) {
@@ -654,6 +655,7 @@
   m->committed = true;
   m->ngroups = root->ngroups;
   m->ln_fold_can = root->ln_fold_can; m->ln_fold_opt = root->ln_fold_opt; m->lnfold_base = root->lnfold_base;
+  m->last_block_rows_opt = root->last_block_rows_opt;
   for (int g = 0; g < 3; ++g) m->vit[g] = root->vit[g];
   m->dp = root->dp;
   m->head_b_host = root->head_b_host;
@@ -830,31 +832,29 @@
   return model_commit(m);
 }
 
-static int get_index_set(md_model_s* m, int B, md_model_s::IndexSet* out) {
-  auto it = m->index_sets.find(B);
-  if (it != m->index_sets.end()) {
-    *out = it->second;
-    return MD_OK;
-  }
-  const int g = m->g, SS = m->SS, P = m->P;
-  const int n0 = m->steps0 * m->steps0 * B, n1 = m->steps1 * m->steps1 * B;
+void build_index_tables(const TokenGeom& t, int B, std::vector<int>* blob, size_t off[6]) {
+  const int g = t.g, SS = t.SS, P = g * g;
+  const int n0 = t.steps0 * t.steps0 * B, n1 = t.steps1 * t.steps1 * B;
   const int nseq_p = n0 + n1 + B;
-  const size_t nhi = (size_t)B * m->mh_hi * m->mh_hi, nmid = (size_t)B * m->mh_mid * m->mh_mid, nlo = (size_t)B * P;
-  std::vector<int> h(nhi + nmid + 3 * nlo);
+  const size_t nhi = (size_t)B * t.mh_hi * t.mh_hi, nmid = (size_t)B * t.mh_mid * t.mh_mid, nlo = (size_t)B * P;
+  off[0] = 0; off[1] = nhi; off[2] = nhi + nmid;
+  for (int i = 3; i < 6; ++i) off[i] = off[i - 1] + nlo;
+  std::vector<int>& h = *blob;
+  h.resize(off[5]);
   size_t o = 0;
   for (int b = 0; b < B; ++b)
-    for (int Y = 0; Y < m->mh_hi; ++Y)
-      for (int X = 0; X < m->mh_hi; ++X) {
+    for (int Y = 0; Y < t.mh_hi; ++Y)
+      for (int X = 0; X < t.mh_hi; ++X) {
         int j, i, ty, tx;
-        merge_source(Y, X, g, g, m->steps0, m->pad_hi, &j, &i, &ty, &tx);
-        h[o++] = ((j * m->steps0 + i) * B + b) * SS + 1 + ty * g + tx;
+        merge_source(Y, X, g, g, t.steps0, t.pad_hi, &j, &i, &ty, &tx);
+        h[o++] = ((j * t.steps0 + i) * B + b) * SS + 1 + ty * g + tx;
       }
   for (int b = 0; b < B; ++b)
-    for (int Y = 0; Y < m->mh_mid; ++Y)
-      for (int X = 0; X < m->mh_mid; ++X) {
+    for (int Y = 0; Y < t.mh_mid; ++Y)
+      for (int X = 0; X < t.mh_mid; ++X) {
         int j, i, ty, tx;
-        merge_source(Y, X, g, g, m->steps1, m->pad_mid, &j, &i, &ty, &tx);
-        h[o++] = (n0 + (j * m->steps1 + i) * B + b) * SS + 1 + ty * g + tx;
+        merge_source(Y, X, g, g, t.steps1, t.pad_mid, &j, &i, &ty, &tx);
+        h[o++] = (n0 + (j * t.steps1 + i) * B + b) * SS + 1 + ty * g + tx;
       }
   for (int which = 0; which < 3; ++which)
     for (int b = 0; b < B; ++b)
@@ -862,19 +862,86 @@
         const int seq = which == 0 ? n0 + n1 + b : which == 1 ? nseq_p + b : nseq_p + B + b;
         h[o++] = seq * SS + 1 + p;
       }
+}
+
+void build_kept_rows(const TokenGeom& t, int B, const std::vector<int>& blob, const size_t off[6], int ntables, KeptRows* out) {
+  const size_t used = off[ntables];
+  out->rows.assign(blob.begin(), blob.begin() + used);
+  std::sort(out->rows.begin(), out->rows.end());
+  out->rows.erase(std::unique(out->rows.begin(), out->rows.end()), out->rows.end());
+  out->remap.assign(blob.size(), -1);
+  for (size_t e = 0; e < used; ++e)
+    out->remap[e] = (int)(std::lower_bound(out->rows.begin(), out->rows.end(), blob[e]) - out->rows.begin());
+  const int nseq_p = (t.steps0 * t.steps0 + t.steps1 * t.steps1 + 1) * B;
+  const int seq_end[3] = {nseq_p, nseq_p + B, nseq_p + 2 * B};
+  int lo = 0;
+  for (int g = 0; g < 3; ++g) {
+    const int hi = (int)(std::lower_bound(out->rows.begin(), out->rows.end(), seq_end[g] * t.SS) - out->rows.begin());
+    out->grow0[g] = lo;
+    out->grows[g] = hi - lo;
+    lo = hi;
+  }
+}
+
+static TokenGeom token_geom(const md_model_s* m) {
+  TokenGeom t;
+  t.g = m->g; t.SS = m->SS; t.steps0 = m->steps0; t.steps1 = m->steps1;
+  t.pad_hi = m->pad_hi; t.pad_mid = m->pad_mid; t.mh_hi = m->mh_hi; t.mh_mid = m->mh_mid;
+  return t;
+}
+
+static md_model_s::IndexSet index_set_at(int* d, const size_t off[6], bool with_fov = true) {
+  md_model_s::IndexSet s;
+  s.hi = d + off[0];
+  s.mid = d + off[1];
+  s.x2 = d + off[2];
+  s.img = d + off[3];
+  s.fov = with_fov ? d + off[4] : nullptr;
+  return s;
+}
+
+static int get_index_set(md_model_s* m, int B, md_model_s::IndexSet* out) {
+  auto it = m->index_sets.find(B);
+  if (it != m->index_sets.end()) {
+    *out = it->second;
+    return MD_OK;
+  }
+  std::vector<int> h;
+  size_t off[6];
+  build_index_tables(token_geom(m), B, &h, off);
   int* d = nullptr;
   MD_HIP(hipMalloc((void**)&d, h.size() * 4));
   m->alloc_count += 1;
   MD_HIP(hipMemcpy(d, h.data(), h.size() * 4, hipMemcpyHostToDevice));
   m->index_tables[B] = d;
-  md_model_s::IndexSet s;
-  s.hi = d;
-  s.mid = d + nhi;
-  s.x2 = s.mid + nmid;
-  s.img = s.x2 + nlo;
-  s.fov = s.img + nlo;
+  const md_model_s::IndexSet s = index_set_at(d, off);
   m->index_sets[B] = s;
   *out = s;
+  return MD_OK;
+}
+
+static int get_last_rows(md_model_s* m, int B, bool with_fov, const md_model_s::LastRows** out) {
+  const std::pair<int, int> key(B, with_fov ? 1 : 0);
+  auto it = m->last_rows.find(key);
+  if (it == m->last_rows.end()) {
+    std::vector<int> h;
+    size_t off[6];
+    const TokenGeom t = token_geom(m);
+    build_index_tables(t, B, &h, off);
+    KeptRows k;
+    build_kept_rows(t, B, h, off, with_fov ? 5 : 4, &k);
+    md_model_s::LastRows lr;
+    lr.n = (int)k.rows.size();
+    MD_HIP(hipMalloc((void**)&lr.blob, (k.rows.size() + k.remap.size()) * 4));
+    m->alloc_count += 1;
+    MD_HIP(hipMemcpy(lr.blob, k.rows.data(), k.rows.size() * 4, hipMemcpyHostToDevice));
+    MD_HIP(hipMemcpy(lr.blob + k.rows.size(), k.remap.data(), k.remap.size() * 4, hipMemcpyHostToDevice));
+    lr.list = lr.blob;
+    lr.ix = index_set_at(lr.blob + k.rows.size(), off, with_fov);
+    for (int g = 0; g < 3; ++g) { lr.grow0[g] = k.grow0[g]; lr.grows[g] = k.grows[g]; }
+    it = m->last_rows.emplace(key, lr).first;
+  }
+  *out = &it->second;
   return MD_OK;
 }
 
@@ -957,12 +1024,13 @@
   auto dense_a = [&](GemmParams& p, int K) {
     if (f8) { p.K = K; p.lda = K; } else split_dense_a(m, p, K, K, 0);
   };
-  auto group_rows = [&](GemmParams& p) {
+  const VitPlan::TailRows* tr = (v.tail && i == depth - 1) ? v.tail : nullptr;
+  auto group_rows = [&](GemmParams& p, bool compact = false) {
     p.ngroups = G;
     for (int g = 0; g < G; ++g) {
-      p.g_row0[g] = v.glo[g] * SS;
-      p.g_arow0[g] = v.glo[g] * SS;
-      p.g_rows[g] = v.gcnt[g] * SS;
+      p.g_row0[g] = compact ? tr->grow0[g] : v.glo[g] * SS;
+      p.g_arow0[g] = p.g_row0[g];
+      p.g_rows[g] = compact ? tr->grows[g] : v.gcnt[g] * SS;
     }
   };
   SeqGroups sg;
@@ -976,8 +1044,15 @@
     }
     float* x = v.x + (size_t)v.s_lo * SS * D;
     r.begin("layernorm");
-    const int st_ = launch_layernorm(x, trow(v.xn, D), rows, D, v.ln_eps, SS, sg, v.lin_prec, 0, r.st, a_inv, tok0,
-                                     tok0 ? v.tok0_stride : 0, tok0 ? x : nullptr);
+    int st_;
+    if (norm2 && tr) {
+      SeqGroups cg = sg;
+      for (int g = 0; g < G; ++g) { cg.seq0[g] = tr->grow0[g]; cg.nseq[g] = tr->grows[g]; }
+      st_ = launch_layernorm(tr->x_c, v.xn, tr->n, D, v.ln_eps, 1, cg, v.lin_prec, 0, r.st, a_inv);
+    } else {
+      st_ = launch_layernorm(x, trow(v.xn, D), rows, D, v.ln_eps, SS, sg, v.lin_prec, 0, r.st, a_inv, tok0, tok0 ? v.tok0_stride : 0,
+                             tok0 ? x : nullptr);
+    }
     r.end();
     return st_;
   };
@@ -995,8 +1070,9 @@
   auto fold_finish = [&]() -> int {
     if (!v.finish_launch) return MD_OK;
     r.begin("ln_finish");
-    const int st_ = launch_ln_finish(v.ln_stats + (size_t)v.s_lo * SS * (D / 256) * 2, v.ln_ab + (size_t)v.s_lo * SS * 2, rows,
-                                     1.0f / (float)D, v.ln_eps, r.st);
+    const size_t row0 = tr ? 0 : (size_t)v.s_lo * SS;
+    const int st_ = launch_ln_finish(v.ln_stats + row0 * (D / 256) * 2, v.ln_ab + row0 * 2, tr ? (long)tr->n : rows, 1.0f / (float)D,
+                                     v.ln_eps, r.st);
     r.end();
     return st_;
   };
@@ -1048,16 +1124,22 @@
   } else {
     MD_TRY(attention_f32(&r, r.st, trow(v.qk, 2 * D), vT_w, trow(v.ao, D), v.scores, v.WS, SS, NT, heads, v.kpad));
   }
+  if (tr) {
+    if (k0.global || v.s_lo != 0) MD_FAIL(MD_ERR_INVALID_ARG, "internal: the kept-row form of the last block takes a whole call of local blocks");
+    r.begin("compact_rows");
+    MD_TRY(launch_compact_rows(v.ao, tr->ao_c, (int)(D * esz), v.x, tr->x_c, D * 4, tr->list, tr->n, r.st));
+    r.end();
+  }
   {
     GemmParams p;
-    p.N = D; group_rows(p);
+    p.N = D; group_rows(p, tr != nullptr);
     for (int g = 0; g < G; ++g) {
       const VitBlockW& k = v.vit[g]->blk[i];
       p.W[g] = f8 ? k.w8[1] : k.proj_w; p.wscale[g] = k.s8[1]; p.bias[g] = k.proj_b; p.scale[g] = k.ls1;
     }
-    p.A = v.ao;
+    p.A = tr ? tr->ao_c : v.ao;
     dense_a(p, D);
-    p.epi = EPI_RESID_LS; p.out = v.x; p.ldo = D;
+    p.epi = EPI_RESID_LS; p.out = tr ? tr->x_c : v.x; p.ldo = D;
     if (k0.global) {
       p.resid_src = v.x; p.out = v.xalt;
       std::swap(v.x, v.xalt);
@@ -1072,7 +1154,7 @@
   if (!fold) MD_TRY(layernorm(true, nullptr));
   {
     GemmParams p;
-    p.N = 4 * D; group_rows(p);
+    p.N = 4 * D; group_rows(p, tr != nullptr);
     for (int g = 0; g < G; ++g) {
       const VitBlockW& k = v.vit[g]->blk[i];
       p.W[g] = f8 ? k.w8[2] : k.fc1_w;
@@ -1094,14 +1176,14 @@
   {
     const bool fold_next = fold && i + 1 < depth;
     GemmParams p;
-    p.N = D; group_rows(p);
+    p.N = D; group_rows(p, tr != nullptr);
     for (int g = 0; g < G; ++g) {
       const VitBlockW& k = v.vit[g]->blk[i];
       p.W[g] = f8 ? k.w8[3] : k.fc2_w; p.wscale[g] = k.s8[3]; p.bias[g] = k.fc2_b; p.scale[g] = k.ls2;
     }
     p.A = v.hbuf;
     dense_a(p, 4 * D);
-    p.epi = EPI_RESID_LS; p.out = v.x; p.ldo = D;
+    p.epi = EPI_RESID_LS; p.out = tr ? tr->x_c : v.x; p.ldo = D;
     if (f8) p.ascale = v.h_scale;
     if (fold_next) fold_producer(p, i + 1, false);
     r.begin("fc2_gemm");
@@ -1112,7 +1194,7 @@
   return MD_OK;
 }
 
-static int run_vit(Run& r, int nseq_p, int nseq, int s_lo, int s_hi) {
+static int run_vit(Run& r, int nseq_p, int nseq, int s_lo, int s_hi, const md_model_s::LastRows* lr = nullptr) {
   md_model_s* m = r.m;
   md_model_s::Buffers* b = m->buf;
   const ModelCfg& c = m->cfg;
@@ -1176,6 +1258,14 @@
   v.ln_stats = b->ln_stats; v.ln_ab = b->ln_ab;
   v.zero_c = m->lnfold_base ? m->lnfold_base + (size_t)m->ngroups * c.pv.depth * 14 * D : nullptr;
   if (v.neutral) MD_TRY(launch_fill_pairs(b->ln_ab + (size_t)s_lo * SS * 2, rows, 1.0f, 0.0f, r.st));
+  VitPlan::TailRows tail;
+  if (lr) {
+    if (s_lo != 0) MD_FAIL(MD_ERR_INVALID_ARG, "internal: kept rows with a sequence window");
+    tail.list = lr->list; tail.n = lr->n;
+    for (int g = 0; g < G; ++g) { tail.grow0[g] = lr->grow0[gi[g]]; tail.grows[g] = lr->grows[gi[g]]; }
+    tail.ao_c = b->tok; tail.x_c = (float*)b->qk;
+    v.tail = &tail;
+  }
   for (int i = 0; i < c.pv.depth; ++i) {
     MD_TRY(run_vit_block(r, v, i));
     for (int hk = 0; hk < 2; ++hk)
@@ -1191,12 +1281,17 @@
   }
   for (int g = 0; g < G; ++g) { sg.a[g] = m->vit[gi[g]].norm_g; sg.b[g] = m->vit[gi[g]].norm_b; }
   r.begin("layernorm");
-  MD_TRY(launch_layernorm(xres_w, trow(b->tok, D), rows, D, c.ln_eps, SS, sg, m->prec, 0, r.st));
+  if (lr) {
+    for (int g = 0; g < G; ++g) { sg.seq0[g] = tail.grow0[g]; sg.nseq[g] = tail.grows[g]; }
+    MD_TRY(launch_layernorm(tail.x_c, b->tok, tail.n, D, c.ln_eps, 1, sg, m->prec, 0, r.st));
+  } else {
+    MD_TRY(launch_layernorm(xres_w, trow(b->tok, D), rows, D, c.ln_eps, SS, sg, m->prec, 0, r.st));
+  }
   r.end();
   return MD_OK;
 }
 
-static int run_encoder_tail(Run& r, const md_model_s::IndexSet& ix) {
+static int run_encoder_tail(Run& r, const md_model_s::IndexSet& ix, const md_model_s::IndexSet& tx) {
   md_model_s* m = r.m;
   md_model_s::Buffers* b = m->buf;
   const ModelCfg& c = m->cfg;
@@ -1215,20 +1310,20 @@
                    nullptr, b->l1p, cpad(m, dims[0])));
   MD_TRY(deconv2(r, "enc_deconv", b->l1p, cpad(m, dims[0]), nullptr, hi, hi, w.enc_up[1],
                  cpad(m, dims[0]), dims[0], nullptr, b->enc1, cpad(m, dims[0]), 0, nullptr, 4, 3));
-  MD_TRY(gemm_rows(r, "enc_proj", b->tok, D, ix.hi, Mhi, w.enc_proj[2], dims[1], D, nullptr,
+  MD_TRY(gemm_rows(r, "enc_proj", b->tok, D, tx.hi, Mhi, w.enc_proj[2], dims[1], D, nullptr,
                    b->x0p, cpad(m, dims[1])));
   MD_TRY(deconv2(r, "enc_deconv", b->x0p, cpad(m, dims[1]), nullptr, hi, hi, w.enc_up[2],
                  cpad(m, dims[1]), dims[1], nullptr, b->enc2, cpad(m, dims[1]), 0));
-  MD_TRY(gemm_rows(r, "enc_proj", b->tok, D, ix.mid, Mmid, w.enc_proj[3], dims[2], D, nullptr,
+  MD_TRY(gemm_rows(r, "enc_proj", b->tok, D, tx.mid, Mmid, w.enc_proj[3], dims[2], D, nullptr,
                    b->x1p, cpad(m, dims[2])));
   MD_TRY(deconv2(r, "enc_deconv", b->x1p, cpad(m, dims[2]), nullptr, mid, mid, w.enc_up[3],
                  cpad(m, dims[2]), dims[2], nullptr, b->enc3, cpad(m, dims[2]), 0));
   const int catld = 2 * cpad(m, dims[3]);
-  MD_TRY(gemm_rows(r, "enc_proj", b->tok, D, ix.x2, Mlo, w.enc_proj[4], dims[3], D, nullptr,
+  MD_TRY(gemm_rows(r, "enc_proj", b->tok, D, tx.x2, Mlo, w.enc_proj[4], dims[3], D, nullptr,
                    b->x2p, cpad(m, dims[3])));
   MD_TRY(deconv2(r, "enc_deconv", b->x2p, cpad(m, dims[3]), nullptr, g, g, w.enc_up[4],
                  cpad(m, dims[3]), dims[3], nullptr, b->cat, catld, 0));
-  MD_TRY(deconv2(r, "enc_deconv", b->tok, D, ix.img, g, g, w.lowres.w, D, dims[3], w.lowres.b, b->cat, catld, cpad(m, dims[3])));
+  MD_TRY(deconv2(r, "enc_deconv", b->tok, D, tx.img, g, g, w.lowres.w, D, dims[3], w.lowres.b, b->cat, catld, cpad(m, dims[3])));
   MD_TRY(gemm_rows(r, "enc_fuse", b->cat, catld, nullptr, Mlo * 4, w.fuse.w, dims[3], catld, w.fuse.b, b->enc4, cpad(m, dims[3])));
   if (m->taps_enabled) {
     MD_TRY(r.tap_nhwc("encoder_feature_0", b->enc0, F, 8 * hi, 8 * hi, cpad(m, F)));
@@ -1746,8 +1841,17 @@
   } ev_set;
   hipEvent_t* ev_w = ev_set.e;
   const bool time_windows = sp && sp->part < 0 && (sp->window_ms || sp->tail_ms) && sp->parts <= 64;
+  const bool fov_group = !known_focal && m->ngroups == 3;
+  const int off_why = !m->last_block_rows_opt ? 1 : m->taps_enabled ? 2 : sp ? 3 : (m->P % 4 != 0) ? 4 : 0;
+  m->last_block_rows_off = off_why;
+  const md_model_s::LastRows* lr = nullptr;
+  md_model_s::IndexSet tx = ix;
+  if (!off_why) {
+    MD_TRY(get_last_rows(m, B, fov_group, &lr));
+    tx = lr->ix;
+  }
   if (!sp) {
-    MD_TRY(run_vit(r, nseq_p, nseq, 0, known_focal ? nseq_p + B : nseq));
+    MD_TRY(run_vit(r, nseq_p, nseq, 0, known_focal ? nseq_p + B : nseq, lr));
   } else {
     auto lo_of = [&](int p) { return (int)((long)nseq * p / sp->parts); };
     if (sp->part < 0) {
@@ -1783,10 +1887,10 @@
     if (sp->tail_ms) MD_HIP(hipEventElapsedTime(sp->tail_ms, ev_w[np], ev_w[np + 1]));
     return MD_OK;
   };
-  MD_TRY(run_encoder_tail(r, ix));
+  MD_TRY(run_encoder_tail(r, ix, tx));
   MD_TRY(run_decoder_head(r));
   if (!known_focal) {
-    MD_TRY(run_fov(r, ix));
+    MD_TRY(run_fov(r, tx));
     r.begin("fov_post");
     MD_TRY(launch_fov_post(b->fov_deg, B, H, W, b->focal, b->fovy, b->ratio, st));
     r.end();
diff --git a/burn_depth_amd/csrc/md_engine_util.h b/burn_depth_amd/csrc/md_engine_util.h
--- a/burn_depth_amd/csrc/md_engine_util.h
+++ b/burn_depth_amd/csrc/md_engine_util.h
@@ -308,6 +308,14 @@
   int tok0_block = -1;
   const float* tok0 = nullptr;
   int tok0_stride = 0;
+  struct TailRows {
+    const int* list = nullptr;
+    int n = 0;
+    int grow0[3] = {0, 0, 0}, grows[3] = {0, 0, 0};
+    void* ao_c = nullptr;
+    float* x_c = nullptr;
+  };
+  const TailRows* tail = nullptr;
 };
 int run_vit_block(Run& r, VitPlan& v, int i);
 
diff --git a/burn_depth_amd/ops.py b/burn_depth_amd/ops.py
--- a/burn_depth_amd/ops.py
+++ b/burn_depth_amd/ops.py
@@ -363,6 +363,35 @@
     ab = torch.empty((rows, 2), dtype=torch.float32, device=parts.device)
     _lib.check(_lib.load().md_op_ln_finish(dev.handle, _p(parts), rows, C.c_float(inv_n), C.c_float(eps), _p(ab), _stream_ptr(dev.ordinal)))
     return ab
+
+
+def compact_rows(dev: Device, a: torch.Tensor, x: torch.Tensor, rows: torch.Tensor) -> Tuple[torch.Tensor, torch.Tensor]:
+    assert a.is_cuda and x.is_cuda and a.is_contiguous() and x.is_contiguous() and a.dim() == 2 and x.dim() == 2 and a.shape[0] == x.shape[0]
+    rows = rows.to(device=a.device, dtype=torch.int32).contiguous()
+    n = rows.numel()
+    a_c = torch.empty((n, a.shape[1]), dtype=a.dtype, device=a.device)
+    x_c = torch.empty((n, x.shape[1]), dtype=x.dtype, device=x.device)
+    _lib.check(_lib.load().md_op_compact_rows(dev.handle, _p(a), a.shape[1] * a.element_size(), _p(x), x.shape[1] * x.element_size(), _p(rows), n,
+                                              a.shape[0], _p(a_c), _p(x_c), _stream_ptr(dev.ordinal)))
+    return a_c, x_c
+
+
+def last_block_rows(window: int, patch: int, B: int, with_fov: bool = True) -> dict:
+    import numpy as np
+    lib = _lib.load()
+    counts = (C.c_int64 * 12)()
+    _lib.check(lib.md_debug_last_block_rows(window, patch, B, int(with_fov), C.byref(counts), None, None, None))
+    sizes = [int(c) for c in counts[:5]]
+    tables, remapped = np.empty(sum(sizes), dtype=np.int32), np.empty(sum(sizes), dtype=np.int32)
+    kept = np.empty(int(counts[5]), dtype=np.int32)
+    _lib.check(lib.md_debug_last_block_rows(window, patch, B, int(with_fov), C.byref(counts), tables.ctypes.data_as(C.c_void_p),
+                                            kept.ctypes.data_as(C.c_void_p), remapped.ctypes.data_as(C.c_void_p)))
+    names, o, res = ("hi", "mid", "x2", "img", "fov"), 0, {"kept": kept, "tables": {}, "remapped": {}}
+    for name, sz in zip(names, sizes):
+        res["tables"][name], res["remapped"][name] = tables[o:o + sz], remapped[o:o + sz]
+        o += sz
+    res["group_row0"], res["group_rows"] = [int(c) for c in counts[6:9]], [int(c) for c in counts[9:12]]
+    return res
 
 
 def vit_gemm(dev: Device, kind: int, a: torch.Tensor, groups, precision: int, tile: int = _lib.TILE_AUTO, *, x: Optional[torch.Tensor] = None,
diff --git a/include/mi_depth.h b/include/mi_depth.h
--- a/include/mi_depth.h
+++ b/include/mi_depth.h
@@ -553,6 +553,8 @@
 int md_op_ln_fold_vectors(md_device_t dev, const float* w, const float* gamma, const float* beta, const float* bias, int N, int K,
                           int precision, float* c, float* d, void* stream);
 int md_op_ln_finish(md_device_t dev, const float* parts, int64_t rows, float inv_n, float eps, float* ab, void* stream);
+int md_op_compact_rows(md_device_t dev, const void* a, int a_bytes, const void* x, int x_bytes, const int32_t* list, int64_t n,
+                       int64_t src_rows, void* a_c, void* x_c, void* stream);
 typedef enum md_vit_gemm_kind { MD_VIT_GEMM_RESID = 0, MD_VIT_GEMM_QKV = 1, MD_VIT_GEMM_FC1 = 2, MD_VIT_GEMM_PATCH_EMBED = 3 } md_vit_gemm_kind;
 typedef struct md_vit_gemm_group {
   int row0, rows, arow0;
@@ -698,6 +700,7 @@
 int md_uniform_stream(const char* name, uint64_t seed, size_t count, float lo, float hi, float* out_host);
 int md_split_geometry(int image_size, int window, float overlap, int* stride, int* steps);
 int md_feature_padding(int window, int stride, int feature_size);
+int md_debug_last_block_rows(int window, int patch, int B, int with_fov, int64_t* counts, int32_t* tables, int32_t* kept, int32_t* remapped);
 
 int md_model_enable_timing(md_model_t m, int enable);
 int md_model_set_timing_filter(md_model_t m, const char* family);
```

Result: no change. 55.87 frames/s (median of 6 runs) (+0.8%).
